# FelixBronnhuber/RenderBaby

Hardware: AMD Instinct MI355X
Metric: Msamples/s (ray-segments/s) (higher is better)
Workload: dtype f32; 1 GPU; C2 Cornell box (12 tris, 8 spheres, 1 area light), 1920x1080, 1024 spp, 8 bounces; width=1920, height=1080, spp=1024, max_depth=8, parallelism=single GPU, stripe_rows=8, walk=library default, tree_builder=, device=AMD Radeon Graphics (gfx950:sramecc+:xnack-, 256 CUs)

## Files before the change

### include/rb_abi.h

```cpp
#ifndef RB_ABI_H
#define RB_ABI_H

#include <stddef.h>
#include <stdint.h>

#ifdef __cplusplus
extern "C" {
#endif


typedef struct rb_camera {
    float pane_distance;
    float pane_width;
    float _pad0[2];
    float pos[3];
    float _pad1;
    float dir[3];
    float _pad2;
} rb_camera;

typedef struct rb_uniforms {
    uint32_t width;
    uint32_t height;
    uint32_t total_samples;
// ... 249 lines not shown
int rb_reset_stats(rb_engine* e);
int rb_last_dispatch_ms(rb_engine* e, float* ms);

int rb_bvh_build(const rb_gpu_triangle* tris, size_t n_tris,
                 rb_bvh_node* nodes_out, size_t nodes_capacity, size_t* n_nodes,
                 uint32_t* indices_out);

int rb_bvh_build_canonical(const rb_gpu_triangle* tris, size_t n_tris,
                           rb_bvh_node* nodes_out, size_t nodes_capacity, size_t* n_nodes,
                           uint32_t* indices_out);
int rb_bvh_build_device(int32_t device, const rb_gpu_triangle* tris, size_t n_tris,
                        rb_bvh_node* nodes_out, size_t nodes_capacity, size_t* n_nodes,
                        uint32_t* indices_out);
int rb_engine_tree(rb_engine* e, rb_bvh_node* nodes_out, size_t nodes_capacity, size_t* n_nodes,
                   uint32_t* indices_out, size_t indices_capacity, size_t* n_indices);
const char* rb_tree_builder(const rb_engine* e, float* build_ms);

int rb_debug_chunk_tree(const rb_gpu_triangle* tris, size_t n_tris, const rb_bvh_node* nodes, size_t n_nodes, const uint32_t* indices,
                        size_t n_indices, uint64_t out6[6]);
int rb_debug_engine_chunk_tree(rb_engine* e, uint64_t out6[6]);
typedef struct rb_debug_own_node {
    float lmin[3];
    uint32_t left;
    float lmax[3];
    uint32_t right;
    float rmin[3];
    float left_fa;
    float rmax[3];
    float right_fa;
} rb_debug_own_node;
typedef struct rb_debug_sphere_node {
    float cx[4], cy[4], cz[4], hx[4], hy[4], hz[4];
    uint32_t ref[4];
    uint32_t axes;
    uint32_t _pad[3];
} rb_debug_sphere_node;
int rb_debug_own_tree(const rb_gpu_triangle* tris, size_t n_tris, const rb_bvh_node* nodes, size_t n_nodes, const uint32_t* indices,
                      size_t n_indices, rb_debug_own_node* nodes_out, size_t nodes_capacity, uint32_t* slots_out, size_t slots_capacity,
                      uint32_t* slot_meta_out, size_t slot_meta_capacity, uint64_t counts3[3], uint32_t root_depth[2], float bounds6[6]);
int rb_debug_engine_own_tree(rb_engine* e, rb_debug_own_node* nodes_out, size_t nodes_capacity, uint32_t* slots_out, size_t slots_capacity,
                             uint32_t* slot_meta_out, size_t slot_meta_capacity, uint64_t counts3[3], uint32_t root_depth[2], float bounds6[6]);
int rb_debug_sphere_tree(const rb_sphere* spheres, size_t n, rb_debug_sphere_node* nodes_out, size_t nodes_capacity, float* leaf_out,
                         uint32_t* id_out, size_t spheres_capacity, uint64_t counts2[2], uint32_t root_depth[2]);
int rb_debug_engine_sphere_tree(rb_engine* e, rb_debug_sphere_node* nodes_out, size_t nodes_capacity, float* leaf_out, uint32_t* id_out,
                                size_t spheres_capacity, uint64_t counts2[2], uint32_t root_depth[2]);
const char* rb_chunk_tree_builder(const rb_engine* e, float* build_ms);
int rb_measure_l1_gather(int32_t device, uint64_t table_bytes, double* accesses_per_s);
int rb_debug_math(const float* a, const float* b, float* out8n, uint32_t n);
int rb_debug_walk_profile(uint64_t out64[64], int reset);
int rb_debug_rcp_exhaustive(uint32_t biased_exponent, uint32_t* out16);
int rb_debug_rcp_det_exhaustive(uint32_t biased_exponent, uint32_t* out16);
int rb_debug_triangle_trip(uint32_t n, uint32_t seed, uint32_t* out32);
int rb_debug_triangle_trip_flat(uint32_t n, uint32_t seed, uint32_t* out32);
int rb_debug_root_box(const float* rays, uint32_t n, const float* box6, uint32_t* out);
int rb_debug_normalize_sites(const float* xyz, uint32_t n, uint32_t n_unit, uint32_t seed0, uint32_t n_seeds, uint32_t* out16);
int rb_measure_salu_mix(int32_t device, uint32_t scalar_per_16, uint32_t branch, double* out3);
int rb_debug_rnd_pm1_exhaustive(uint32_t* out16);
int rb_debug_div_exhaustive(uint32_t b_begin, uint32_t b_count, uint32_t ea, uint32_t eb, uint32_t a_begin,
                            uint32_t a_count, unsigned long long* out16);

const char* rb_last_kernel_name(const rb_engine* e);
enum {
    RB_TRACE_FORM_FLAT = 1u,
    RB_TRACE_FORM_BIG = 4u,
    RB_TRACE_FORM_STAGED = 8u,
    RB_TRACE_FORM_MULTI = 16u
};
uint32_t rb_debug_trace_form(const rb_engine* e);

typedef struct rb_ray { float origin[3]; float _pad0; float dir[3]; float _pad1; } rb_ray;
enum { RB_HIT_NONE = 0, RB_HIT_GROUND = 1, RB_HIT_TRIANGLE = 2, RB_HIT_SPHERE = 3, RB_HIT_LIGHT = 4,
       RB_HIT_INVALID = 0xFFFFFFFFu };
typedef struct rb_hit {
    float t;
    uint32_t kind;
    uint32_t prim;
    uint32_t mesh;
    float u, v;
    uint32_t _pad[2];
    float normal[3];
    float _pad1;
} rb_hit;
typedef struct rb_surface {
    float albedo[3];
    uint32_t flags;
    float emissive[3];
    int32_t texture_index;
    float uv[2];
    float _pad[2];
} rb_surface;
int rb_cast_rays(rb_engine* e, const rb_ray* rays, size_t n, rb_hit* hits_out, rb_surface* surf_out);
int rb_render_hits(rb_engine* e, rb_hit* hits_out, rb_surface* surf_out);
int rb_pick(rb_engine* e, uint32_t px, uint32_t py, rb_hit* hit_out, rb_surface* surf_out);
const char* rb_last_query_kernel_name(const rb_engine* e);
int rb_last_query_ms(rb_engine* e, float* ms);

enum { RB_OCCL_VISIBLE = 0, RB_OCCL_OCCLUDED = 1, RB_OCCL_INVALID = 255 };
enum { RB_MASK_GROUND = 1, RB_MASK_TRIANGLES = 2, RB_MASK_SPHERES = 4, RB_MASK_LIGHTS = 8, RB_MASK_ALL = 15 };
int rb_occluded(rb_engine* e, const rb_ray* rays, const float* tmax, size_t n, uint32_t mask, uint8_t* out);
int rb_occluded_device(rb_engine* e, const rb_ray* d_rays, const float* d_tmax, size_t n, uint32_t mask, uint8_t* d_out);
int rb_cast_rays_device(rb_engine* e, const rb_ray* d_rays, size_t n, rb_hit* d_hits, rb_surface* d_surf);

typedef struct rb_radiance { float sum[3]; float weight; } rb_radiance;
#define RB_TRACE_PIECE_ITEMS (1u << 24)
int rb_trace_rays(rb_engine* e, const rb_ray* rays, const uint32_t* seeds, size_t n, uint32_t first_sample, uint32_t samples,
                  rb_radiance* out);
int rb_trace_rays_device(rb_engine* e, const rb_ray* d_rays, const uint32_t* d_seeds, size_t n, uint32_t first_sample,
                         uint32_t samples, rb_radiance* d_out);

enum { RB_CAM_PERSPECTIVE = 1, RB_CAM_ORTHO = 2, RB_CAM_EQUIRECT = 3 };
enum { RB_CAM_NO_JITTER = 1u };
typedef struct rb_camera_ex {
    uint32_t kind, width, height, flags;
    float pos[3];     float tan_half_fov;
    float right[3];   float half_width;
    float up[3];      float half_height;
// ... 304 lines not shown
```

### renderbaby_amd/_lib.py

```python
import ctypes as C
import os

from . import abi

_HERE = os.path.dirname(os.path.abspath(__file__))
LIB_PATH = os.environ.get("RB_LIBRARY_PATH") or os.path.join(_HERE, "librenderbaby_hip.so")
_lib = None


P = C.POINTER
vp, u32, i32, sz = C.c_void_p, C.c_uint32, C.c_int, C.c_size_t
SIGNATURES = {
    "rb_create": (vp, [P(abi.Config)]),
    "rb_create_ex": (vp, [P(abi.Config), P(abi.Options)]),
    "rb_create_multi": (vp, [P(abi.Config), P(abi.Options), P(C.c_int32), u32]),
    "rb_comm_unique_id": (i32, [vp]),
    "rb_comm_available": (i32, []),
    "rb_comm_init_rank": (i32, [vp, vp, u32, u32]),
    "rb_comm_info": (i32, [vp, P(u32), P(u32), P(C.c_float)]),
    "rb_destroy": (None, [vp]),
    "rb_update": (i32, [vp, P(abi.Config)]),
    "rb_render": (i32, [vp, vp]),
    "rb_render_config": (i32, [vp, P(abi.Config), vp]),
    "rb_iter_begin": (i32, [vp, P(abi.Config)]),
    "rb_iter_has_next": (i32, [vp]),
    "rb_iter_next": (i32, [vp, vp]),
    "rb_iter_destroy": (None, [vp]),
    "rb_iter_set_passes_per_frame": (i32, [vp, u32]),
    "rb_last_error": (C.c_char_p, [vp]),
    "rb_get_size": (i32, [vp, P(u32), P(u32)]),
    "rb_clear": (i32, [vp]),
    "rb_dispatch": (i32, [vp, u32, u32]),
    "rb_reserve": (i32, [vp, u32]),
    "rb_sync": (i32, [vp]),
    "rb_read_rgba": (i32, [vp, vp]),
    "rb_read_accumulation": (i32, [vp, vp]),
    "rb_device_rgba": (i32, [vp, P(vp), P(sz)]),
    "rb_host_alloc": (vp, [sz]),
    "rb_host_free": (None, [vp]),
    "rb_local_rows": (i32, [vp, P(u32), P(u32)]),
    "rb_global_row": (i32, [vp, u32, P(u32)]),
    "rb_shard_layout": (i32, [u32, u32, u32, u32, P(u32), P(u32)]),
    "rb_shard_global_row": (u32, [u32, u32, u32, u32]),
    "rb_get_stats": (i32, [vp, P(abi.Stats)]),
    "rb_reset_stats": (i32, [vp]),
    "rb_last_dispatch_ms": (i32, [vp, P(C.c_float)]),
    "rb_bvh_build": (i32, [vp, sz, vp, sz, P(sz), vp]),
    "rb_bvh_build_canonical": (i32, [vp, sz, vp, sz, P(sz), vp]),
    "rb_bvh_build_device": (i32, [i32, vp, sz, vp, sz, P(sz), vp]),
    "rb_engine_tree": (i32, [vp, vp, sz, P(sz), vp, sz, P(sz)]),
    "rb_tree_builder": (C.c_char_p, [vp, vp]),
    "rb_debug_chunk_tree": (i32, [vp, sz, vp, sz, vp, sz, vp]),
    "rb_measure_l1_gather": (i32, [i32, C.c_uint64, P(C.c_double)]),
    "rb_debug_math": (i32, [vp, vp, vp, u32]),
    "rb_debug_walk_profile": (i32, [vp, i32]),
    "rb_debug_rcp_exhaustive": (i32, [u32, vp]),
    "rb_debug_rcp_det_exhaustive": (i32, [u32, vp]),
    "rb_debug_rnd_pm1_exhaustive": (i32, [vp]),
    "rb_debug_triangle_trip": (i32, [u32, u32, vp]),
    "rb_debug_triangle_trip_flat": (i32, [u32, u32, vp]),
    "rb_debug_trace_form": (u32, [vp]),
    "rb_debug_root_box": (i32, [vp, u32, vp, vp]),
    "rb_debug_normalize_sites": (i32, [vp, u32, u32, u32, u32, vp]),
    "rb_measure_salu_mix": (i32, [i32, u32, u32, P(C.c_double)]),
    "rb_debug_div_exhaustive": (i32, [u32, u32, u32, u32, u32, u32, vp]),
    "rb_last_kernel_name": (C.c_char_p, [vp]),
    "rb_cast_rays": (i32, [vp, vp, sz, vp, vp]),
    "rb_render_hits": (i32, [vp, vp, vp]),
    "rb_pick": (i32, [vp, u32, u32, vp, vp]),
    "rb_occluded": (i32, [vp, vp, vp, sz, u32, vp]),
    "rb_occluded_device": (i32, [vp, vp, vp, sz, u32, vp]),
    "rb_cast_rays_device": (i32, [vp, vp, sz, vp, vp]),
    "rb_trace_rays": (i32, [vp, vp, vp, sz, u32, u32, vp]),
    "rb_trace_rays_device": (i32, [vp, vp, vp, sz, u32, u32, vp]),
    "rb_camera_rays": (i32, [i32, vp, C.c_uint64, sz, u32, u32, vp, vp]),
    "rb_trace_camera": (i32, [vp, vp, C.c_uint64, sz, u32, u32, vp]),
    "rb_trace_camera_device": (i32, [vp, vp, C.c_uint64, sz, u32, u32, vp]),
    "rb_last_camera_rays_ms": (i32, [vp, P(C.c_float)]),
    "rb_hemisphere_rays": (i32, [i32, vp, vp, sz, vp, u32, u32, vp, vp]),
    "rb_trace_hemisphere": (i32, [vp, vp, vp, sz, vp, u32, u32, vp]),
    "rb_trace_hemisphere_device": (i32, [vp, vp, vp, sz, vp, u32, u32, vp]),
    "rb_openness_hemisphere": (i32, [vp, vp, vp, sz, vp, u32, u32, vp]),
    "rb_openness_hemisphere_device": (i32, [vp, vp, vp, sz, vp, u32, u32, vp]),
    "rb_scene_emitters": (i32, [vp, vp, sz, P(sz)]),
    "rb_scene_emitters_device": (i32, [vp, vp, sz, vp]),
    "rb_light_rays": (i32, [i32, vp, sz, vp, vp, sz, vp, u32, u32, vp, vp, vp]),
    "rb_direct_light": (i32, [vp, vp, sz, vp, vp, sz, vp, u32, u32, vp]),
    "rb_direct_light_device": (i32, [vp, vp, sz, vp, vp, sz, vp, u32, u32, vp]),
    "rb_lightmap_surfels": (i32, [i32, vp, sz, vp, sz, vp, vp, vp]),
    "rb_lightmap_surfels_device": (i32, [vp, vp, vp, vp]),
    "rb_lightmap_resolve": (i32, [i32, u32, u32, vp, u32, vp]),
    "rb_bake_lightmap": (i32, [vp, vp, u32, u32, vp, vp]),
    "rb_bake_lightmap_device": (i32, [vp, vp, u32, u32, vp, vp]),
    "rb_last_lightmap_ms": (i32, [vp, P(C.c_float), P(C.c_float)]),
    "rb_probe_rays": (i32, [i32, vp, vp, sz, u32, u32, vp, vp]),
    "rb_bake_probes": (i32, [vp, vp, vp, sz, u32, u32, vp]),
    "rb_bake_probes_device": (i32, [vp, vp, vp, sz, u32, u32, vp]),
    "rb_last_probe_project_ms": (i32, [vp, P(C.c_float)]),
    "rb_probe_coefficients": (i32, [i32, vp, sz, vp]),
    "rb_probe_coefficients_device": (i32, [vp, vp, sz, vp]),
    "rb_light_points": (i32, [i32, vp, vp, vp, sz, vp]),
    "rb_light_points_device": (i32, [vp, vp, vp, vp, sz, vp]),
    "rb_bake_probe_depth": (i32, [vp, vp, vp, sz, u32, u32, C.c_float, vp]),
    "rb_bake_probe_depth_device": (i32, [vp, vp, vp, sz, u32, u32, C.c_float, vp]),
    "rb_last_probe_depth_project_ms": (i32, [vp, P(C.c_float)]),
    "rb_probe_moments": (i32, [i32, vp, sz, vp, vp]),
    "rb_probe_moments_device": (i32, [vp, vp, sz, vp, vp]),
    "rb_light_points_visible": (i32, [i32, vp, vp, vp, vp, sz, vp, vp]),
    "rb_light_points_visible_device": (i32, [vp, vp, vp, vp, vp, sz, vp, vp]),
    "rb_last_query_kernel_name": (C.c_char_p, [vp]),
    "rb_last_query_ms": (i32, [vp, P(C.c_float)]),
    "rb_denoise_default_params": (i32, [vp]),
    "rb_denoise_buffers": (i32, [i32, vp, u32, u32, vp, vp, vp, vp]),
# ... 63 lines not shown
```

### renderbaby_amd/abi.py

```python
import ctypes as C

import numpy as np

f4, u4, i4 = np.float32, np.uint32, np.int32

CAMERA = np.dtype([
    ("pane_distance", f4), ("pane_width", f4), ("_pad0", f4, (2,)),
    ("pos", f4, (3,)), ("_pad1", f4), ("dir", f4, (3,)), ("_pad2", f4)])

UNIFORMS = np.dtype([
    ("width", u4), ("height", u4), ("total_samples", u4), ("color_hash_enabled", u4),
    ("camera", CAMERA),
    ("spheres_count", u4), ("triangles_count", u4), ("bvh_node_count", u4),
    ("bvh_triangle_count", u4), ("bvh_root", u4), ("ground_height", f4),
    ("ground_enabled", u4), ("checkerboard_enabled", u4),
    ("sky_color", f4, (3,)), ("max_depth", u4),
    ("checkerboard_color_1", f4, (3,)), ("_pad1", u4),
    ("checkerboard_color_2", f4, (3,)), ("_pad2", u4)])

MATERIAL = np.dtype([
    ("ambient", f4, (3,)), ("_pad0", f4), ("diffuse", f4, (3,)), ("_pad1", f4),
    ("specular", f4, (3,)), ("shininess", f4), ("emissive", f4, (3,)), ("ior", f4),
    ("opacity", f4), ("illum", u4), ("texture_index", i4), ("_pad2", u4)])

# ... 38 lines not shown
PROBE_GRID = np.dtype([("origin", f4, (3,)), ("_pad0", u4), ("step", f4, (3,)), ("_pad1", u4), ("counts", u4, (3,)), ("flags", u4)])
LIT = np.dtype([("value", f4, (3,)), ("weight", f4)])
LIGHT_PIECE_POINTS = 1 << 22
PROBE_DEPTH = np.dtype([("texel", f4, (64, 4))])
LIGHT_VISIBILITY = np.dtype([("normal_bias", f4), ("min_visibility", f4), ("flags", u4), ("_pad", u4)])
VIS_NO_WRAP, VIS_NO_DEPTH = 1, 2
EMITTER = np.dtype([("a", f4, (3,)), ("kind", u4), ("b", f4, (3,)), ("prim", u4), ("c", f4, (3,)), ("area", f4),
                    ("emissive", f4, (3,)), ("_pad", f4)])
LIGHT_PARAMS = np.dtype([("offset", f4), ("shorten", f4), ("mask", u4), ("flags", u4), ("_reserved", u4, (4,))])
MAX_EMITTERS = 1 << 24
OCCL_VISIBLE, OCCL_OCCLUDED, OCCL_INVALID = 0, 1, 255
MASK_GROUND, MASK_TRIANGLES, MASK_SPHERES, MASK_LIGHTS, MASK_ALL = 1, 2, 4, 8, 15
GUIDE = np.dtype([("normal", f4, (3,)), ("t", f4), ("pos", f4, (3,)), ("cls", u4), ("albedo", f4, (3,)), ("_pad", f4)])
DENOISE_PARAMS = np.dtype([("iterations", u4), ("normal_power_log2", u4), ("sigma_depth", f4), ("sigma_color", f4),
                           ("albedo_floor", f4), ("flags", u4), ("_reserved", u4, (2,))])
VIEW = np.dtype([("pos", f4, (3,)), ("cx", f4), ("right", f4, (3,)), ("cy", f4), ("up", f4, (3,)), ("sx", f4), ("fwd", f4, (3,)), ("sy", f4)])
REPROJECT_PARAMS = np.dtype([("sigma_depth", f4), ("normal_min", f4), ("albedo_floor", f4), ("max_history", f4), ("flags", u4),
                             ("_reserved", u4, (3,))])
FRAME_RECORD = np.dtype([("mean", f4, (3,)), ("count", f4)])
OWN_NODE = np.dtype([("lmin", f4, (3,)), ("left", u4), ("lmax", f4, (3,)), ("right", u4),
                     ("rmin", f4, (3,)), ("left_fa", f4), ("rmax", f4, (3,)), ("right_fa", f4)])
SPHERE_NODE = np.dtype([("cx", f4, (4,)), ("cy", f4, (4,)), ("cz", f4, (4,)), ("hx", f4, (4,)), ("hy", f4, (4,)), ("hz", f4, (4,)),
                        ("ref", u4, (4,)), ("axes", u4), ("_pad", u4, (3,))])

SIZES = {"camera": (CAMERA, 48), "uniforms": (UNIFORMS, 144), "material": (MATERIAL, 80),
         "sphere": (SPHERE, 96), "point_light": (POINT_LIGHT, 96), "mesh": (MESH, 96),
         "bvh_node": (BVH_NODE, 48), "gpu_triangle": (GPU_TRIANGLE, 64),
         "ray": (RAY, 32), "hit": (HIT, 48), "surface": (SURFACE, 48),
         "guide": (GUIDE, 48), "denoise_params": (DENOISE_PARAMS, 32), "view": (VIEW, 64),
         "reproject_params": (REPROJECT_PARAMS, 32), "frame_record": (FRAME_RECORD, 16), "camera_ex": (CAMERA_EX, 96),
         "surfel": (SURFEL, 32), "hemi_params": (HEMI_PARAMS, 32), "openness": (OPENNESS, 8),
         "lightmap_params": (LIGHTMAP_PARAMS, 32), "probe": (PROBE, 16), "sh9": (SH9, 112),
         "probe_grid": (PROBE_GRID, 48), "lit": (LIT, 16),
         "probe_depth": (PROBE_DEPTH, 1024), "light_visibility": (LIGHT_VISIBILITY, 16),
         "emitter": (EMITTER, 64), "light_params": (LIGHT_PARAMS, 32),
         "own_node": (OWN_NODE, 64), "sphere_node": (SPHERE_NODE, 128)}
for _n, (_dt, _sz) in SIZES.items():
    assert _dt.itemsize == _sz, (_n, _dt.itemsize, _sz)

KEEP, CREATE, UPDATE, DELETE = 0, 1, 2, 3

RB_OK = 0
ERR = {
    1: "PaneDistanceOutOfBounds", 2: "PaneWidthOutOfBounds", 3: "InvalidCameraDirection",
    4: "InvalidUniforms", 5: "InvalidSpheres", 6: "InvalidUVs", 7: "InvalidMeshes",
    8: "InvalidLights", 9: "InvalidTextures", 10: "CannotDeleteNonexistent",
    11: "UniformsNotInitialized", 12: "NoMoreFrames", 13: "InvalidBVH", 14: "UnsupportedDelete",
    15: "NullArgument", 16: "Device", 17: "NotInitialized", 18: "InvalidOptions"}
RB_ERR_NO_MORE_FRAMES = 12
RB_ERR_DEVICE = 16

KERNEL_DEFAULT, KERNEL_PIXEL, KERNEL_QUEUE, KERNEL_STREAM = 0, 1, 2, 3
TRACE_FORM_FLAT, TRACE_FORM_BIG, TRACE_FORM_STAGED, TRACE_FORM_MULTI = 1, 4, 8, 16
FLAG_STATS = 1
FLAG_NO_SPHERE_BVH = 2
FLAG_FAST_BVH = 4
FLAG_DEVICE_BVH = 8
FLAG_DEVICE_LBVH = 16
FLAG_REFERENCE_WALK = 32
FLAG_HOST_BVH = 64
FLAG_GATHER_PEER_COPY = 128
FLAG_NO_RUN_AHEAD = 256
FLAG_SKIP_NEAR_DEGENERATE = 512
FLAG_CHUNK_WALK = 1024
FLAG_SPHERE_TREE_HOST = 2048
FLAG_SPHERE_TREE_DEVICE = 4096
FLAG_CHUNK_TREE_HOST = 8192
FLAG_CHUNK_TREE_DEVICE = 16384
FLAG_BUILD_TREE = 32768
FLAG_BUILD_TREE_HOST = 65536
COMM_ID_BYTES = 128


class Field(C.Structure):
    _fields_ = [("change", C.c_uint32), ("ptr", C.c_void_p), ("count", C.c_size_t)]


class Config(C.Structure):
    _fields_ = [(n, Field) for n in ("uniforms", "spheres", "uvs", "meshes", "lights", "bvh_nodes",
                                      "bvh_indices", "bvh_triangles", "textures")]


class Texture(C.Structure):
    _fields_ = [("width", C.c_uint32), ("height", C.c_uint32), ("rgba_data", C.c_void_p)]


class Options(C.Structure):
    _fields_ = [("device", C.c_int32), ("shard_rank", C.c_uint32), ("shard_count", C.c_uint32),
                ("stripe_rows", C.c_uint32), ("passes_per_launch", C.c_uint32), ("kernel", C.c_uint32),
                ("flags", C.c_uint32), ("_reserved", C.c_uint32 * 5)]


class Ray(C.Structure):
    _fields_ = [("origin", C.c_float * 3), ("_pad0", C.c_float), ("dir", C.c_float * 3), ("_pad1", C.c_float)]


class Hit(C.Structure):
    _fields_ = [("t", C.c_float), ("kind", C.c_uint32), ("prim", C.c_uint32), ("mesh", C.c_uint32), ("u", C.c_float),
                ("v", C.c_float), ("_pad", C.c_uint32 * 2), ("normal", C.c_float * 3), ("_pad1", C.c_float)]


class Surface(C.Structure):
    _fields_ = [("albedo", C.c_float * 3), ("flags", C.c_uint32), ("emissive", C.c_float * 3),
                ("texture_index", C.c_int32), ("uv", C.c_float * 2), ("_pad", C.c_float * 2)]


# ... 17 lines not shown
```

### renderbaby_amd/csrc/rb_debug.hip

```cpp
#include <algorithm>

#include "rb_device_shade.hpp"

#pragma clang fp contract(off)

namespace rb {
namespace {

__global__ void k_rcp_exhaustive(uint32_t expo, uint32_t* mismatch) {
    const uint32_t m = blockIdx.x * blockDim.x + threadIdx.x;
    if (m >= (1u << 23)) return;
    for (uint32_t sign = 0; sign < 2; sign++) {
        const uint32_t bits = (sign << 31) | ((expo & 0xFFu) << 23) | m;
        const float b = __uint_as_float(bits);
        float want, got;
        if (expo & 0x100u) {
            if (sign) continue;
            want = sqrtf(b);
            got = sqrt_exact(b);
        } else {
            if (!rcp_safe(b)) continue;
            want = 1.0f / b;
            got = rcp_newton(b);
        }
// ... 60 lines not shown
DEV void trip_case(uint32_t k, f3& o, f3& d, f3& v0, f3& e1, f3& e2) {
    o = mk(0.25f, 0.25f, -1.0f);
    d = mk(0.0f, 0.0f, 1.0f);
    v0 = mk(0.0f, 0.0f, 0.0f);
    e1 = mk(0.0f, 1.0f, 0.0f);
    e2 = mk(1.0f, 0.0f, 0.0f);
    const uint32_t eps = 0x358637BDu, big = 0x71800000u, one = 0x3F800000u, tmin = 0x3A83126Fu;
    const float nan = __uint_as_float(0x7FC00000u), inf = __uint_as_float(0x7F800000u);
    switch (k) {
        case 0: case 1: case 2: e1.y = __uint_as_float(eps - 1u + k); break;
        case 3: case 4: case 5: e1.y = -__uint_as_float(eps - 1u + (k - 3u)); break;
        case 6: case 7: case 8: e1.y = __uint_as_float(big - 1u + (k - 6u)); break;
        case 9: e1.y = -0x1p100f; break;
        case 10: e1.y = 0x1p120f; break;
        case 11: e1.y = __uint_as_float(0x3F80FFFFu); break;
        case 12: e1.y = __uint_as_float(0xC123FFFFu); break;
        case 13: e1.y = __uint_as_float(0x3FFFFFFFu); break;
        case 14: o.y = 0.0f; break;
        case 15: o.y = -0.0f; break;
        case 16: o.y = -0x1p-149f; break;
        case 17: o.y = 1.0f; o.x = 0.0f; break;
        case 18: o.y = __uint_as_float(one + 1u); o.x = 0.0f; break;
        case 19: o.x = 0.0f; break;
        case 20: o.x = -0.0f; break;
        case 21: o.x = -0x1p-149f; break;
        case 22: o.x = 0.75f; break;
        case 23: o.x = 0.75f; o.y = __uint_as_float(0x3E800001u); break;
        case 24: o.z = -__uint_as_float(tmin); break;
        case 25: o.z = -__uint_as_float(tmin + 1u); break;
        case 26: o.z = -__uint_as_float(tmin - 1u); break;
        case 27: o.z = 0.0f; break;
        case 28: o.z = 1.0f; break;
        case 29: o.x = nan; break;
        case 30: o.y = nan; break;
        case 31: o.z = nan; break;
        case 32: d.x = nan; break;
        case 33: d.y = nan; break;
        case 34: d.z = nan; break;
        case 35: o.x = inf; break;
        case 36: o.y = -inf; break;
        case 37: o.z = -inf; break;
        case 38: d.x = inf; break;
        case 39: d.y = -inf; break;
        case 40: d.z = inf; break;
        case 41: e1.y = 0.0f; break;
        case 42: e1.y = nan; break;
        default: e2.x = inf; break;
    }
}
DEV float trip_unit(uint32_t& s) {
    s = pcg(s);
    return (float)(int32_t)s * 0x1p-31f;
}
template <bool FLAT>
__global__ void __launch_bounds__(256) k_triangle_trip(uint32_t n_waves, uint32_t seed, uint32_t* mismatch) {
    const uint32_t wave = (blockIdx.x * 256u + threadIdx.x) >> 6, lane = threadIdx.x & 63u;
    if (wave >= n_waves + kTripCases) return;
    f3 o, d, v0, e1, e2;
    float hit_t = 1e20f;
    bool on = true;
    if (wave < n_waves) {
        uint32_t sw = pcg(seed ^ (wave * 0x9E3779B9u)), sl = pcg(sw + lane * 0x85EBCA6Bu + 1u);
        const uint32_t kind = pcg(sw) & 15u;
        const float scale = kind == 0u ? 0x1p-10f : kind == 1u ? 0x1p52f : 1.0f;
        v0 = mk(trip_unit(sw), trip_unit(sw), trip_unit(sw));
        e1 = scale * mk(trip_unit(sw), trip_unit(sw), trip_unit(sw));
        e2 = scale * mk(trip_unit(sw), trip_unit(sw), trip_unit(sw));
        o = 2.0f * mk(trip_unit(sl), trip_unit(sl), trip_unit(sl));
        const float a = 0.7f * trip_unit(sl) + 0.5f, b = 0.7f * trip_unit(sl) + 0.5f;
        const f3 to = (v0 + a * e1 + b * e2) - o;
        d = __builtin_amdgcn_rsqf(dot(to, to) + 1e-30f) * to;
        const uint32_t r = pcg(sl);
        if (r & 1u) hit_t = 2.0f * (float)(r >> 8) * 0x1p-24f;
        on = (r & 6u) != 0u;
    } else {
        trip_case(wave - n_waves, o, d, v0, e1, e2);
        on = (lane & 8u) == 0u;
    }
    auto uni = [](float x) { return __uint_as_float((uint32_t)__builtin_amdgcn_readfirstlane((int)__float_as_uint(x))); };
    const v4f ra = {uni(v0.x), uni(v0.y), uni(v0.z), 0.0f}, rb_ = {uni(e1.x), uni(e1.y), uni(e1.z), 0.0f},
              rc = {uni(e2.x), uni(e2.y), uni(e2.z), 1.0f};
    const uint32_t slot = (uint32_t)__builtin_amdgcn_readfirstlane((int)(wave + 1u));
    if (wave >= n_waves) {
        TriHit own;
        own.t = 1e20f, own.u = 0.0f, own.v = 0.0f, own.slot = 0u, own.hit = false;
        accept_slot<true>(ra, rb_, rc, slot, o, d, own);
        const uint32_t v = lane & 3u;
        hit_t = v == 0u ? 1e20f : v == 1u ? 0.5f : v == 2u ? own.t : __uint_as_float(__float_as_uint(own.t) + 1u);
    }
    TriHit want, got;
    want.t = hit_t, want.u = -2.0f, want.v = -3.0f, want.slot = 0xABCDu, want.hit = false;
    got = want;
    float big = 0x1p100f;
    if constexpr (RB_TRIP_BLOCK) asm("s_mov_b32 %0, 0x71800000" : "=s"(big));
    if (on) {
        accept_slot<true>(ra, rb_, rc, slot, o, d, want);
        if constexpr (FLAT && RB_TRIP_BLOCK) {
            TriHitT<false> flat;
            flat.t = got.t, flat.slot = got.slot, flat.hit = false;
            accept_trip<RB_TRIP_ASM - 1, false>(ra, rb_, rc, slot, o, d, big, flat);
            got.t = flat.t, got.slot = flat.slot, got.u = want.u, got.v = want.v;
        } else if constexpr (RB_TRIP_BLOCK) accept_trip<RB_TRIP_ASM - 1>(ra, rb_, rc, slot, o, d, big, got);
        else accept_slot<true>(ra, rb_, rc, slot, o, d, got);
    }
    if (__float_as_uint(want.t) != __float_as_uint(got.t) || __float_as_uint(want.u) != __float_as_uint(got.u) ||
        __float_as_uint(want.v) != __float_as_uint(got.v) || want.slot != got.slot) {
        if (atomicAdd(&mismatch[0], 1u) == 0u) {
            mismatch[1] = wave * 64u + lane;
            const float in[16] = {o.x, o.y, o.z, d.x, d.y, d.z, ra.x, ra.y, ra.z, rb_.x, rb_.y, rb_.z, rc.x, rc.y, rc.z, hit_t};
            for (int k = 0; k < 16; k++) mismatch[2 + k] = __float_as_uint(in[k]);
            mismatch[18] = __float_as_uint(got.t), mismatch[19] = __float_as_uint(got.u), mismatch[20] = __float_as_uint(got.v);
            mismatch[21] = got.slot;
            mismatch[22] = __float_as_uint(want.t), mismatch[23] = __float_as_uint(want.u), mismatch[24] = __float_as_uint(want.v);
            mismatch[25] = want.slot;
        }
    }
}

template <int SALU, bool BRANCH>
__global__ void __launch_bounds__(256, 8) k_salu_mix(uint32_t rounds, float c, float* sink, unsigned long long* stamp) {
    float v[16];
#pragma unroll
    for (int k = 0; k < 16; k++) v[k] = (float)(threadIdx.x + k) * 0x1p-20f;
    const float c2 = c * 0x1p-20f;
    uint32_t s0 = rounds, s1 = rounds + 1u, s2 = rounds + 2u, s3 = rounds + 3u;
    const unsigned long long t0 = __builtin_amdgcn_s_memtime(), r0 = __builtin_amdgcn_s_memrealtime();
#define RB_MIX_F(k) "v_fmac_f32_e32 %" #k ", %[c], %[c2]\n\t"
#define RB_MIX_S(j) "s_add_u32 %[s" #j "], %[s" #j "], 1\n\t"
#define RB_MIX_Q0(a, b, c, d) RB_MIX_F(a) RB_MIX_F(b) RB_MIX_F(c) RB_MIX_F(d)
#define RB_MIX_Q1(a, b, c, d) RB_MIX_F(a) RB_MIX_F(b) RB_MIX_S(0) RB_MIX_F(c) RB_MIX_F(d)
#define RB_MIX_Q2(a, b, c, d) RB_MIX_F(a) RB_MIX_S(0) RB_MIX_F(b) RB_MIX_F(c) RB_MIX_S(1) RB_MIX_F(d)
#define RB_MIX_Q3(a, b, c, d) RB_MIX_F(a) RB_MIX_S(0) RB_MIX_F(b) RB_MIX_S(1) RB_MIX_F(c) RB_MIX_S(2) RB_MIX_F(d)
#define RB_MIX_Q4(a, b, c, d) RB_MIX_F(a) RB_MIX_S(0) RB_MIX_F(b) RB_MIX_S(1) RB_MIX_F(c) RB_MIX_S(2) RB_MIX_F(d) RB_MIX_S(3)
#define RB_MIX_BR "s_cbranch_execz .Lmix_out_%=\n\t"
#define RB_MIX_GROUP(Q, BR) Q(0, 1, 2, 3) Q(4, 5, 6, 7) Q(8, 9, 10, 11) Q(12, 13, 14, 15) BR
#define RB_MIX_ASM(Q, BR)                                                                                                 \
    asm volatile(RB_MIX_GROUP(Q, BR) RB_MIX_GROUP(Q, BR) RB_MIX_GROUP(Q, BR) RB_MIX_GROUP(Q, BR) ".Lmix_out_%=:"          \
                 : "+v"(v[0]), "+v"(v[1]), "+v"(v[2]), "+v"(v[3]), "+v"(v[4]), "+v"(v[5]), "+v"(v[6]), "+v"(v[7]), "+v"(v[8]), \
                   "+v"(v[9]), "+v"(v[10]), "+v"(v[11]), "+v"(v[12]), "+v"(v[13]), "+v"(v[14]), "+v"(v[15]), [s0] "+s"(s0), \
                   [s1] "+s"(s1), [s2] "+s"(s2), [s3] "+s"(s3)                                                            \
                 : [c] "v"(c), [c2] "v"(c2)                                                                                             \
                 : "scc")
    for (uint32_t r = rounds; r != 0u; r--) {
        if constexpr (BRANCH) {
            if constexpr (SALU == 0) RB_MIX_ASM(RB_MIX_Q0, RB_MIX_BR);
            else if constexpr (SALU == 4) RB_MIX_ASM(RB_MIX_Q1, RB_MIX_BR);
            else if constexpr (SALU == 8) RB_MIX_ASM(RB_MIX_Q2, RB_MIX_BR);
            else if constexpr (SALU == 12) RB_MIX_ASM(RB_MIX_Q3, RB_MIX_BR);
            else RB_MIX_ASM(RB_MIX_Q4, RB_MIX_BR);
        } else {
            if constexpr (SALU == 0) RB_MIX_ASM(RB_MIX_Q0, "");
            else if constexpr (SALU == 4) RB_MIX_ASM(RB_MIX_Q1, "");
            else if constexpr (SALU == 8) RB_MIX_ASM(RB_MIX_Q2, "");
            else if constexpr (SALU == 12) RB_MIX_ASM(RB_MIX_Q3, "");
            else RB_MIX_ASM(RB_MIX_Q4, "");
        }
    }
#undef RB_MIX_F
#undef RB_MIX_S
#undef RB_MIX_Q0
#undef RB_MIX_Q1
#undef RB_MIX_Q2
#undef RB_MIX_Q3
#undef RB_MIX_Q4
#undef RB_MIX_BR
#undef RB_MIX_GROUP
#undef RB_MIX_ASM
    const unsigned long long t1 = __builtin_amdgcn_s_memtime(), r1 = __builtin_amdgcn_s_memrealtime();
    float acc = (float)(s0 ^ s1 ^ s2 ^ s3);
// ... 127 lines not shown
#undef RB_MIX_LAUNCH
        (void)hipEventRecord(t1, nullptr);
        if (!ok || hipGetLastError() != hipSuccess || hipEventSynchronize(t1) != hipSuccess) { ok = false; break; }
        float ms = 0.0f;
        (void)hipEventElapsedTime(&ms, t0, t1);
        if (rep > 0 && ms > 0.0f && (best == 0.0f || ms < best)) {
            best = ms;
            (void)hipMemcpy(st, stamp, 16, hipMemcpyDeviceToHost);
        }
    }
    (void)hipEventDestroy(t0);
    (void)hipEventDestroy(t1);
    (void)hipFree(sink);
    (void)hipFree(stamp);
    if (!ok || best <= 0.0f || st[1] == 0ull) return false;
    const double ghz = (double)st[0] / (double)st[1] * 0.1;
    out[0] = (best * 1e-3) * (ghz * 1e9) / ((double)rounds * 64.0 * 8.0);
    out[1] = ghz;
    out[2] = best;
    return true;
}

double measure_l1_gather(size_t table_bytes, uint32_t rounds) {
    size_t lines = 64;
    while (lines * 2 * 128 <= table_bytes) lines *= 2;
    float4 *table = nullptr, *sink = nullptr;
    if (hipMalloc(reinterpret_cast<void**>(&table), lines * 128) != hipSuccess) return 0.0;
    if (hipMalloc(reinterpret_cast<void**>(&sink), 16) != hipSuccess) { (void)hipFree(table); return 0.0; }
    (void)hipMemset(table, 0, lines * 128);
    hipEvent_t t0, t1;
    (void)hipEventCreate(&t0);
    (void)hipEventCreate(&t1);
    double best = 0.0;
    for (int shape = 0; shape < 4; shape++) {
        const uint32_t inflight = (shape & 1) ? 16u : 8u, blocks = device_cu_count_cached() * ((shape & 2) ? 8u : 4u);
        for (int rep = 0; rep < 2; rep++) {
            (void)hipEventRecord(t0, nullptr);
            if (inflight == 16u) hipLaunchKernelGGL(k_l1_gather<16>, dim3(blocks), dim3(256), 0, nullptr, table, (uint32_t)(lines - 1), rounds, sink);
            else hipLaunchKernelGGL(k_l1_gather<8>, dim3(blocks), dim3(256), 0, nullptr, table, (uint32_t)(lines - 1), rounds, sink);
            (void)hipEventRecord(t1, nullptr);
            if (hipEventSynchronize(t1) != hipSuccess) break;
            float ms = 0.0f;
            (void)hipEventElapsedTime(&ms, t0, t1);
            if (ms > 0.0f) best = std::max(best, (double)blocks * 256.0 * rounds * inflight / (ms * 1e-3));
        }
    }
    (void)hipEventDestroy(t0);
    (void)hipEventDestroy(t1);
    (void)hipFree(table);
    (void)hipFree(sink);
    return best;
}
}
}

extern "C" {

int rb_debug_rcp_exhaustive(uint32_t biased_exponent, uint32_t* out16) {
    if (!out16) return RB_ERR_NULL_ARGUMENT;
    return rb::round_trip(out16, 64, 64, [&](uint32_t* d) {
        hipLaunchKernelGGL(rb::k_rcp_exhaustive, dim3((1u << 23) / 256), dim3(256), 0, nullptr, biased_exponent, d);
    });
}

int rb_debug_rcp_det_exhaustive(uint32_t biased_exponent, uint32_t* out16) {
    if (!out16) return RB_ERR_NULL_ARGUMENT;
    if (biased_exponent > 255u) return RB_ERR_INVALID_OPTIONS;
    return rb::round_trip(out16, 64, 64, [&](uint32_t* d) {
        hipLaunchKernelGGL(rb::k_rcp_det_exhaustive, dim3((1u << 23) / 256), dim3(256), 0, nullptr, biased_exponent, d);
    });
}

int rb_debug_triangle_trip(uint32_t n, uint32_t seed, uint32_t* out32) {
    if (!out32) return RB_ERR_NULL_ARGUMENT;
    if (n > (1u << 26)) return RB_ERR_INVALID_OPTIONS;
    return rb::round_trip(out32, 128, 128, [&](uint32_t* d) {
        const uint32_t n_waves = (n + 63u) / 64u, waves = n_waves + rb::kTripCases;
        hipLaunchKernelGGL(rb::k_triangle_trip<false>, dim3((waves + 3u) / 4u), dim3(256), 0, nullptr, n_waves, seed, d);
    });
}

int rb_debug_triangle_trip_flat(uint32_t n, uint32_t seed, uint32_t* out32) {
    if (!out32) return RB_ERR_NULL_ARGUMENT;
    if (n > (1u << 26)) return RB_ERR_INVALID_OPTIONS;
    return rb::round_trip(out32, 128, 128, [&](uint32_t* d) {
        const uint32_t n_waves = (n + 63u) / 64u, waves = n_waves + rb::kTripCases;
        hipLaunchKernelGGL(rb::k_triangle_trip<true>, dim3((waves + 3u) / 4u), dim3(256), 0, nullptr, n_waves, seed, d);
    });
}

int rb_debug_root_box(const float* rays, uint32_t n, const float* box6, uint32_t* out) {
    if (!rays || !box6 || !out) return RB_ERR_NULL_ARGUMENT;
    if (n == 0u) return RB_OK;
    if (n > (1u << 24)) return RB_ERR_INVALID_OPTIONS;
    const size_t out_bytes = (size_t)n * 4u, in_bytes = (size_t)n * 24u;
    const rb::f3 bmin = {box6[0], box6[1], box6[2]}, bmax = {box6[3], box6[4], box6[5]};
    return rb::round_trip(out, out_bytes, out_bytes + in_bytes, [&](uint32_t* d) {
        float* dr = reinterpret_cast<float*>(d + n);
        (void)hipMemcpy(dr, rays, in_bytes, hipMemcpyHostToDevice);
        hipLaunchKernelGGL(rb::k_root_box, dim3((n + 255u) / 256u), dim3(256), 0, nullptr, dr, n, bmin, bmax, d);
    });
}

int rb_debug_normalize_sites(const float* xyz, uint32_t n, uint32_t n_unit, uint32_t seed0, uint32_t n_seeds, uint32_t* out16) {
    if (!out16 || (!xyz && n + n_unit != 0u)) return RB_ERR_NULL_ARGUMENT;
    if (n > (1u << 26) || n_unit > (1u << 26) || n_seeds > (1u << 26)) return RB_ERR_INVALID_OPTIONS;
    const size_t total = (size_t)n + n_unit + n_seeds, in_bytes = ((size_t)n + n_unit) * 12u;
    if (total == 0u) {
        std::fill(out16, out16 + 16, 0u);
        return RB_OK;
    }
    return rb::round_trip(out16, 64, 64 + in_bytes, [&](uint32_t* d) {
        float* dv = reinterpret_cast<float*>(d + 16);
        if (in_bytes) (void)hipMemcpy(dv, xyz, in_bytes, hipMemcpyHostToDevice);
        hipLaunchKernelGGL(rb::k_normalize_sites, dim3((uint32_t)((total + 255u) / 256u)), dim3(256), 0, nullptr, dv, n, n_unit, seed0, n_seeds, d);
    });
}

int rb_measure_salu_mix(int32_t device, uint32_t scalar_per_16, uint32_t branch, double* out3) {
    if (!out3) return RB_ERR_NULL_ARGUMENT;
    if (scalar_per_16 > 16u || (scalar_per_16 & 3u) != 0u) return RB_ERR_INVALID_OPTIONS;
    int before = -1;
    if (device >= 0 && (hipGetDevice(&before) != hipSuccess || hipSetDevice(device) != hipSuccess)) return RB_ERR_DEVICE;
    const bool ok = rb::measure_salu_mix(scalar_per_16, branch != 0u, 4096u, out3);
    if (before >= 0) (void)hipSetDevice(before);
    return ok ? RB_OK : RB_ERR_DEVICE;
}

int rb_debug_rnd_pm1_exhaustive(uint32_t* out16) {
    if (!out16) return RB_ERR_NULL_ARGUMENT;
    return rb::round_trip(out16, 64, 64, [&](uint32_t* d) {
        hipLaunchKernelGGL(rb::k_rnd_pm1_exhaustive, dim3(1u << 16), dim3(256), 0, nullptr, d);
    });
}

int rb_debug_div_exhaustive(uint32_t b_begin, uint32_t b_count, uint32_t ea, uint32_t eb, uint32_t a_begin,
                            uint32_t a_count, unsigned long long* out16) {
    if (!out16) return RB_ERR_NULL_ARGUMENT;
    return rb::round_trip(out16, 128, 128, [&](unsigned long long* d) {
        hipLaunchKernelGGL(rb::k_div_exhaustive, dim3((b_count + 255) / 256), dim3(256), 0, nullptr, b_begin, ea, eb, a_begin, a_count, d);
// ... 24 lines not shown
```

### renderbaby_amd/csrc/rb_device_intersect.hpp

```cpp
#pragma once
#include "rb_device_math.hpp"

#pragma clang fp contract(off)

namespace rb {
namespace {

template <bool TEXEL = true>
DEV f3 sample_texture(const KParams& p, int32_t index, float uvx, float uvy) {
    if (!TEXEL || index < 0) {
        if (p.u.checkerboard_enabled > 0u) {
            int32_t u2 = f2i(floorf(uvx * 10.0f));
            int32_t v2 = f2i(floorf(uvy * 10.0f));
            int32_t sum = (int32_t)((uint32_t)u2 + (uint32_t)v2);
            return (sum % 2 == 0) ? ld3(p.u.checkerboard_color_1) : ld3(p.u.checkerboard_color_2);
        }
        return mk(1.0f, 1.0f, 1.0f);
    }
    if ((uint32_t)index >= p.n_tex) return mk(0.0f, 0.0f, 0.0f);
    const v4u iw = ((cu4p)p.tex_info)[index];
    rb_texture_info info;
    info.offset = iw.x;
    info.width = iw.y;
    info.height = iw.z;
// ... 128 lines not shown
    uint32_t slot;
    bool hit;
};
using TriHit = TriHitT<true>;

template <bool UV>
DEV void test_slot(const v4f a, const v4f b, const v4f c, uint32_t slot, f3 o, f3 d, TriHitT<UV>& h) {
    float u, v;
    const float t = isect_triangle(o, d, mk(a.x, a.y, a.z), mk(b.x, b.y, b.z), mk(c.x, c.y, c.z), u, v);
    if (t > 0.001f && t < h.t) {
        h.hit = true;
        h.t = t;
        if constexpr (UV) {
            h.u = u;
            h.v = v;
        }
        h.slot = slot;
    }
}

template <bool DET = false>
DEV void accept_slot(const v4f a, const v4f b, const v4f c, uint32_t slot, f3 o, f3 d, TriHit& hit) {
    const f3 v0 = mk(a.x, a.y, a.z), edge1 = mk(b.x, b.y, b.z), edge2 = mk(c.x, c.y, c.z);
    const f3 h = cross(d, edge2);
    const float det = dot(edge1, h);
    if (!(fabsf(det) < 1e-6f)) {
        const float f = DET ? rcp_det(det) : rcp_tri(det);
        const f3 s = o - v0;
        const float u = f * dot(s, h);
        if (!(u < 0.0f || u > 1.0f)) {
            const f3 q = cross(s, edge1);
            const float v = f * dot(d, q);
            if (!(v < 0.0f || u + v > 1.0f)) {
                const float t = f * dot(edge2, q);
                if (t > 0.0f && t > 0.001f && t < hit.t) {
                    hit.t = t;
                    hit.u = u;
                    hit.v = v;
                    hit.slot = slot;
                }
            }
        }
    }
}

#ifndef RB_TRIP_PLAIN
#define RB_TRIP_PLAIN 1
#endif
#ifndef RB_TRIP_ASM
#define RB_TRIP_ASM 3
#endif
#define RB_TRIP_BLOCK (RB_TRIP_ASM != 0 && RB_FAST_RCP && RB_RCP_DET)

template <int SKIP, bool UV = true>
DEV void accept_trip(const v4f a, const v4f b, const v4f c, uint32_t slot, f3 o, f3 d, float big, TriHitT<UV>& hit) {
    float r8, r10, r11, r12, r13, r14, r15, r16, r17;
    uint64_t entry, keep, m, ds;
#define RB_TRIP_HEAD                                                                                                     \
    "s_mov_b64 %[entry], exec\n\t"                                                                                       \
    "v_mul_f32_e32 %[r8], %[cz], %[dy]\n\t"                                                                              \
    "v_mul_f32_e32 %[r10], %[cy], %[dz]\n\t"                                                                             \
    "v_sub_f32_e32 %[r10], %[r8], %[r10]\n\t"                                                                            \
    "v_mul_f32_e32 %[r8], %[cx], %[dz]\n\t"                                                                              \
    "v_mul_f32_e32 %[r11], %[cz], %[dx]\n\t"                                                                             \
    "v_sub_f32_e32 %[r11], %[r8], %[r11]\n\t"                                                                            \
    "v_mul_f32_e32 %[r8], %[cy], %[dx]\n\t"                                                                              \
    "v_mul_f32_e32 %[r12], %[cx], %[dy]\n\t"                                                                             \
    "v_sub_f32_e32 %[r12], %[r8], %[r12]\n\t"                                                                            \
    "v_mul_f32_e32 %[r8], %[bx], %[r10]\n\t"                                                                             \
    "v_mul_f32_e32 %[r13], %[by], %[r11]\n\t"                                                                            \
    "v_add_f32_e32 %[r8], %[r8], %[r13]\n\t"                                                                             \
    "v_mul_f32_e32 %[r13], %[bz], %[r12]\n\t"                                                                            \
    "v_add_f32_e32 %[r13], %[r13], %[r8]\n\t"                                                                            \
    "v_cmpx_nlt_f32_e64 vcc, |%[r13]|, %[eps]\n\t"                                                  \
    "v_cmp_eq_u16_e64 %[m], -1, %[r13]\n\t"                                     \
    "v_cmp_nlt_f32_e64 vcc, |%[r13]|, %[big]\n\t"                                               \
    "v_rcp_f32_e32 %[r8], %[r13]\n\t"                                                                                    \
    "s_or_b64 %[m], vcc, %[m]\n\t"                                                                                       \
    "v_fma_f32 %[r14], -%[r13], %[r8], 1.0\n\t"                                                                          \
    "v_fmac_f32_e32 %[r8], %[r14], %[r8]\n\t"                                                                            \
    "s_and_saveexec_b64 %[keep], %[m]\n\t"                                                                               \
    "s_cbranch_execz .Ltrip_rcp_%=\n\t"                                                                                  \
    "v_div_scale_f32 %[r8], %[ds], %[r13], %[r13], 1.0\n\t"                   \
    "v_rcp_f32_e32 %[r14], %[r8]\n\t"                                                                                    \
    "v_div_scale_f32 %[r15], vcc, 1.0, %[r13], 1.0\n\t"                                                                  \
    "v_fma_f32 %[r16], -%[r8], %[r14], 1.0\n\t"                                                                          \
    "v_fmac_f32_e32 %[r14], %[r16], %[r14]\n\t"                                                                          \
    "v_mul_f32_e32 %[r16], %[r15], %[r14]\n\t"                                                                           \
    "v_fma_f32 %[r17], -%[r8], %[r16], %[r15]\n\t"                                                                       \
    "v_fmac_f32_e32 %[r16], %[r17], %[r14]\n\t"                                                                          \
    "v_fma_f32 %[r8], -%[r8], %[r16], %[r15]\n\t"                                                                        \
    "v_div_fmas_f32 %[r8], %[r8], %[r14], %[r16]\n\t"                                                                    \
    "v_div_fixup_f32 %[r8], %[r8], %[r13], 1.0\n"                                                                        \
    ".Ltrip_rcp_%=:\n\t"                                                                                                 \
    "s_mov_b64 exec, %[keep]\n\t"                                                                                        \
    "v_subrev_f32_e32 %[r13], %[ax], %[ox]\n\t"                                                                          \
    "v_subrev_f32_e32 %[r14], %[ay], %[oy]\n\t"                                                                          \
    "v_subrev_f32_e32 %[r15], %[az], %[oz]\n\t"                                                                          \
    "v_mul_f32_e32 %[r10], %[r13], %[r10]\n\t"                                                                           \
    "v_mul_f32_e32 %[r11], %[r14], %[r11]\n\t"                                                                           \
    "v_add_f32_e32 %[r10], %[r10], %[r11]\n\t"                                                                           \
    "v_mul_f32_e32 %[r11], %[r15], %[r12]\n\t"                                                                           \
    "v_add_f32_e32 %[r10], %[r11], %[r10]\n\t"                                                                           \
    "v_mul_f32_e32 %[r10], %[r10], %[r8]\n\t"                                                                     \
    "v_cmpx_ngt_f32_e32 vcc, 0, %[r10]\n\t"                                                                \
    "v_cmpx_nlt_f32_e32 vcc, 1.0, %[r10]\n\t"
#define RB_TRIP_TAIL                                                                                                     \
    "v_mul_f32_e32 %[r11], %[bz], %[r14]\n\t"                                                                            \
    "v_mul_f32_e32 %[r12], %[by], %[r15]\n\t"                                                                            \
    "v_sub_f32_e32 %[r12], %[r11], %[r12]\n\t"                                                                           \
    "v_mul_f32_e32 %[r11], %[bx], %[r15]\n\t"                                                                            \
    "v_mul_f32_e32 %[r15], %[bz], %[r13]\n\t"                                                                            \
    "v_sub_f32_e32 %[r15], %[r11], %[r15]\n\t"                                                                           \
    "v_mul_f32_e32 %[r11], %[by], %[r13]\n\t"                                                                            \
    "v_mul_f32_e32 %[r13], %[bx], %[r14]\n\t"                                                                            \
    "v_sub_f32_e32 %[r13], %[r11], %[r13]\n\t"                                                                           \
    "v_mul_f32_e32 %[r11], %[dx], %[r12]\n\t"                                                                            \
    "v_mul_f32_e32 %[r14], %[dy], %[r15]\n\t"                                                                            \
    "v_add_f32_e32 %[r11], %[r11], %[r14]\n\t"                                                                           \
    "v_mul_f32_e32 %[r14], %[dz], %[r13]\n\t"                                                                            \
    "v_add_f32_e32 %[r11], %[r14], %[r11]\n\t"                                                                           \
    "v_mul_f32_e32 %[r11], %[r11], %[r8]\n\t"                                                                     \
    "v_add_f32_e32 %[r14], %[r10], %[r11]\n\t"                                                                           \
    "v_cmpx_ngt_f32_e32 vcc, 0, %[r11]\n\t"                                                                \
    "v_cmpx_nlt_f32_e32 vcc, 1.0, %[r14]\n\t"
#define RB_TRIP_LAST                                                                                                     \
    "v_mul_f32_e32 %[r12], %[cx], %[r12]\n\t"                                                                            \
    "v_mul_f32_e32 %[r14], %[cy], %[r15]\n\t"                                                                            \
    "v_add_f32_e32 %[r12], %[r12], %[r14]\n\t"                                                                           \
    "v_mul_f32_e32 %[r13], %[cz], %[r13]\n\t"                                                                            \
    "v_add_f32_e32 %[r12], %[r13], %[r12]\n\t"                                                                           \
    "v_mul_f32_e32 %[r8], %[r12], %[r8]\n\t"                                                                      \
    "v_cmpx_lt_f32_e32 vcc, %[tmin], %[r8]\n\t"                                                           \
    "v_cmpx_lt_f32_e32 vcc, %[r8], %[ht]\n\t"                                                             \
    "v_mov_b32_e32 %[hs], %[slot]\n\t"
#define RB_TRIP_MOVES_UV                                                                                                 \
    "v_mov_b32_e32 %[hv], %[r11]\n\t"                                                                                    \
    "v_mov_b32_e32 %[ht], %[r8]\n\t"                                                                                     \
    "v_mov_b32_e32 %[hu], %[r10]\n"
#define RB_TRIP_MOVES_T                                                                                                  \
    "v_mov_b32_e32 %[ht], %[r8]\n"
#define RB_TRIP_OUT_UV [ht] "+v"(hit.t), [hu] "+v"(hit.u), [hv] "+v"(hit.v), [hs] "+v"(hit.slot)
#define RB_TRIP_OUT_T [ht] "+v"(hit.t), [hs] "+v"(hit.slot)
#define RB_TRIP_TEMPS                                                                                                    \
    [r8] "=&v"(r8), [r10] "=&v"(r10),                                                                                     \
      [r11] "=&v"(r11), [r12] "=&v"(r12), [r13] "=&v"(r13), [r14] "=&v"(r14), [r15] "=&v"(r15), [r16] "=&v"(r16),         \
      [r17] "=&v"(r17), [entry] "=&s"(entry), [keep] "=&s"(keep), [m] "=&s"(m), [ds] "=&s"(ds)
#define RB_TRIP_IN                                                                                                       \
    [ax] "s"(a.x), [ay] "s"(a.y), [az] "s"(a.z), [bx] "s"(b.x), [by] "s"(b.y), [bz] "s"(b.z), [cx] "s"(c.x),              \
      [cy] "s"(c.y), [cz] "s"(c.z), [slot] "s"(slot), [ox] "v"(o.x), [oy] "v"(o.y), [oz] "v"(o.z), [dx] "v"(d.x),         \
      [dy] "v"(d.y), [dz] "v"(d.z), [eps] "s"(1e-6f)
#define RB_TRIP_CLOBBERS "vcc", "scc"
#define RB_TRIP_OPS_UV : RB_TRIP_OUT_UV, RB_TRIP_TEMPS : RB_TRIP_IN, [big] "s"(big), [tmin] "s"(0.001f) : RB_TRIP_CLOBBERS
#define RB_TRIP_OPS_T : RB_TRIP_OUT_T, RB_TRIP_TEMPS : RB_TRIP_IN, [big] "s"(big), [tmin] "s"(0.001f) : RB_TRIP_CLOBBERS
#define RB_TRIP_SKIP "s_cbranch_execz .Ltrip_end_%=\n\t"
#define RB_TRIP_EMIT(MOVES, OPS)                                                                                         \
    if constexpr (SKIP == 2) {                                                                                           \
        asm volatile(RB_TRIP_HEAD RB_TRIP_SKIP RB_TRIP_TAIL RB_TRIP_SKIP RB_TRIP_LAST MOVES ".Ltrip_end_%=:\n\t"         \
                     "s_mov_b64 exec, %[entry]" OPS);                                                                    \
    } else if constexpr (SKIP == 1) {                                                                                    \
        asm volatile(RB_TRIP_HEAD RB_TRIP_SKIP RB_TRIP_TAIL RB_TRIP_LAST MOVES ".Ltrip_end_%=:\n\t"                      \
                     "s_mov_b64 exec, %[entry]" OPS);                                                                    \
    } else {                                                                                                             \
        asm volatile(RB_TRIP_HEAD RB_TRIP_TAIL RB_TRIP_LAST MOVES "\ts_mov_b64 exec, %[entry]" OPS);                     \
    }
    if constexpr (UV) {
        RB_TRIP_EMIT(RB_TRIP_MOVES_UV, RB_TRIP_OPS_UV)
    } else {
        RB_TRIP_EMIT(RB_TRIP_MOVES_T, RB_TRIP_OPS_T)
    }
#undef RB_TRIP_EMIT
#undef RB_TRIP_SKIP
#undef RB_TRIP_HEAD
#undef RB_TRIP_MOVES_UV
#undef RB_TRIP_MOVES_T
#undef RB_TRIP_OUT_UV
#undef RB_TRIP_OUT_T
#undef RB_TRIP_TEMPS
#undef RB_TRIP_IN
#undef RB_TRIP_CLOBBERS
#undef RB_TRIP_OPS_UV
#undef RB_TRIP_OPS_T
#undef RB_TRIP_TAIL
#undef RB_TRIP_LAST
}


DEV float cone_cos_bound(f3 d, v4f cone) {
    const float y = fabsf(__builtin_fmaf(d.z, cone.z, __builtin_fmaf(d.y, cone.y, d.x * cone.x)));
    const float k2 = __builtin_fmaf(cone.z, cone.z, __builtin_fmaf(cone.y, cone.y, cone.x * cone.x));
    const float root = 1.000001f * __builtin_amdgcn_sqrtf(fmaxf(__builtin_fmaf(-y, y, k2), 0.0f) + 4e-6f * k2);
    return __builtin_fmaf(-cone.w, root, y - 1e-6f);
}
DEV bool cone_admits_grazing(f3 d, v4f cone) {
    if (cone.w < 0.0f) return false;
    return !(cone_cos_bound(d, cone) >= kFastGrazeCos);
}
constexpr float kFastKF = 27.0f * 5.9604645e-8f * 1.01f;
constexpr float kFastKS = 20.0f * 5.9604645e-8f * 1.01f;
template <bool STATS>
struct FastWalk {
    f3 o, d, inv;
    float m_ref;
    TriHit h;
    uint32_t best_rank;
    uint32_t cur;
    uint32_t gend;
    bool graze;
    int sp;

    DEV void begin(const KParams& p, f3 o_, f3 d_) {
        o = o_;
        d = d_;
        h.hit = false;
        h.t = 1e20f;
        h.u = 0.0f;
        h.v = 0.0f;
        h.slot = 0u;
        best_rank = 0xFFFFFFFFu;
        inv = mk(rcp_exact(d.x), rcp_exact(d.y), rcp_exact(d.z));
        const f3 fb0 = ld3(p.fast_bmin), fb1 = ld3(p.fast_bmax);
        const float sx_ = fmaxf(fabsf(o.x - fb0.x), fabsf(o.x - fb1.x)), sy_ = fmaxf(fabsf(o.y - fb0.y), fabsf(o.y - fb1.y)),
// ... 156 lines not shown
        const cf4p rnodes = (cf4p)p.nodes;
        const RB_CONST uint32_t* parent = cptr(p.ref_parent);
        const float m = m_ref;
        {
            const v4f n0 = rnodes[leaf_node * 3u], n1 = rnodes[leaf_node * 3u + 1u];
            if constexpr (STATS) tl.nodes++;
            const bool thick = (n1.x - n0.x >= 2.0f * m) && (n1.y - n0.y >= 2.0f * m) && (n1.z - n0.z >= 2.0f * m);
            const f3 t0 = (mk(n0.x + m, n0.y + m, n0.z + m) - o) * inv;
            const f3 t1 = (mk(n1.x - m, n1.y - m, n1.z - m) - o) * inv;
            const float tn = fmaxf(fmaxf(fminf(t0.x, t1.x), fminf(t0.y, t1.y)), fminf(t0.z, t1.z));
            const float tf = fminf(fminf(fmaxf(t0.x, t1.x), fmaxf(t0.y, t1.y)), fmaxf(t0.z, t1.z));
            const bool finite = (t0.x == t0.x) && (t0.y == t0.y) && (t0.z == t0.z) && (t1.x == t1.x) && (t1.y == t1.y) &&
                                (t1.z == t1.z);
            if (thick && finite && tf >= fmaxf(tn, 0.0f)) return true;
        }
        uint32_t n = leaf_node;
        for (;;) {
            const v4f n0 = rnodes[n * 3u], n1 = rnodes[n * 3u + 1u];
            if constexpr (STATS) tl.nodes++;
            if (!isect_aabb(o, inv, mk(n0.x, n0.y, n0.z), mk(n1.x, n1.y, n1.z))) return false;
            if (n == 0u) return true;
            n = parent[n];
        }
    }

    DEV bool leaf_step(const KParams& p, uint32_t* stack, uint32_t stride, Tally<STATS>& tl) {
        const cf4p ftris = (cf4p)p.fast_tris;
        const RB_CONST uint32_t* fslots = cptr(p.fast_slots);
        const RB_CONST uint32_t* meta = cptr(p.slot_meta);
        const uint32_t first = cur & 0x0FFFFFFFu, count = ((cur >> 28) & 3u) + 1u;
        for (uint32_t j = first; j < first + count; j++) {
            const v4f a = ftris[j * 4u], b = ftris[j * 4u + 1u], c = ftris[j * 4u + 2u];
            if constexpr (STATS) tl.tris++;
            float u, v;
            const float t = isect_triangle(o, d, mk(a.x, a.y, a.z), mk(b.x, b.y, b.z), mk(c.x, c.y, c.z), u, v);
            if (t > 0.001f && !(t > h.t)) {
                const uint32_t slot = fslots[j];
                const uint32_t leaf_node = meta[slot * 2u], rank = meta[slot * 2u + 1u] & ~kSlotLarge;
                if ((t < h.t || rank < best_rank) && reference_would_test(p, leaf_node, tl)) {
                    h.hit = true;
                    h.t = t;
                    h.u = u;
                    h.v = v;
                    h.slot = slot;
                    best_rank = rank;
                    if constexpr (STATS) tl.mesh_hits++;
                }
            }
        }
        return pop(p, stack, stride);
    }
};

template <bool STATS>
DEV TriHit intersect_bvh_fast(const KParams& p, f3 o, f3 d, uint32_t* stack, uint32_t stride, Tally<STATS>& tl) {
    FastWalk<STATS> w;
    w.begin(p, o, d);
    while (w.step(p, stack, stride, tl)) {
    }
    return w.h;
}

template <bool STATS, bool MULTI = true, bool TRIP = false, bool UV = true>
DEV TriHitT<UV> intersect_bvh(const KParams& p, f3 o, f3 d, uint32_t* stack, uint32_t stride, Tally<STATS>& tl, uint32_t box = kBoxUnknown) {
    static_assert(UV || (TRIP && !MULTI && RB_TRIP_BLOCK && RB_TRIP_PLAIN != 0), "the flat forms exist for the hand-laid trip only");
    TriHitT<UV> h;
    h.hit = false;
    h.t = 1e20f;
    if constexpr (UV) {
        h.u = 0.0f;
        h.v = 0.0f;
    }
    h.slot = 0u;
    const uint32_t node_count = p.u.bvh_node_count;
    if (node_count == 0u) return h;
    if constexpr (MULTI) {
        if (p.fast_nodes != nullptr) return intersect_bvh_fast<STATS>(p, o, d, stack, stride, tl);
    }
    constexpr bool skip_box = TRIP && !MULTI && RB_ROOT_INSIDE != 0;
    const f3 inv = skip_box ? d : mk(rcp_exact(d.x), rcp_exact(d.y), rcp_exact(d.z));
    const cf4p nodes = (cf4p)p.nodes;
    const cf4p ptris = (cf4p)p.ptris;

    if (node_count == 1u) {
        const v4f n0 = nodes[0], n1 = nodes[1];
        const v4u n2 = ((cu4p)p.nodes)[2];
        if constexpr (STATS) tl.nodes++;
        const uint32_t first = n2.z, count = n2.w;
        const uint32_t end = (first + count < p.index_len) ? first + count : p.index_len;
        auto in_box = [&]() {
            const f3 b0 = mk(n0.x, n0.y, n0.z), b1 = mk(n1.x, n1.y, n1.z);
            if constexpr (skip_box) {
                const uint64_t unknown = __builtin_amdgcn_uicmp(box, kBoxUnknown, 32) & ~root_inside_mask(o, d, b0, b1);
                if (__builtin_expect(unknown == 0ull && box_finite(b0, b1), 1)) return box != kBoxMiss;
                return isect_aabb(o, mk(rcp_exact(d.x), rcp_exact(d.y), rcp_exact(d.z)), b0, b1);
            } else {
                return isect_aabb(o, inv, b0, b1);
            }
        };
        if (first < end && in_box()) {
            constexpr bool trip = TRIP && !MULTI;
            float big = 0x1p100f;
            if constexpr (trip && RB_TRIP_BLOCK) asm("s_mov_b32 %0, 0x71800000" : "=s"(big));
            auto test = [&](const v4f a, const v4f b, const v4f c, uint32_t slot) {
                if constexpr (STATS) tl.tris++;
                const float before = h.t;
                if constexpr (trip && RB_TRIP_BLOCK) accept_trip<RB_TRIP_ASM - 1, UV>(a, b, c, slot, o, d, big, h);
                else accept_slot<!MULTI>(a, b, c, slot, o, d, h);
                if constexpr (STATS) tl.mesh_hits += (h.t != before) ? 1u : 0u;
            };
            if constexpr (trip && RB_TRIP_PLAIN != 0) {
                cf4p rec = ptris + (size_t)first * 4u;
                for (uint32_t slot = first; slot != end; slot++, rec += 4) {
                    v4f a = rec[0], b = rec[1], c = rec[2];
                    uint32_t live = __float_as_uint(c.w);
                    asm volatile("" : "+s"(a.x), "+s"(b.x), "+s"(live));
                    if (live != 0u) test(a, b, c, slot);
                }
            } else {
                const uint32_t last = end - 1u;
                cf4p rec = ptris + (size_t)first * 4u;
                v4f a = rec[0], b = rec[1], c = rec[2];
                bool live = __float_as_uint(c.w) != 0u;
                for (uint32_t slot = first;; slot++) {
                    if (slot < last) rec += 4;
                    const v4f na = rec[0], nb = rec[1], nc = rec[2];
                    if (live) test(a, b, c, slot);
                    if (slot == last) break;
                    a = na;
                    b = nb;
                    c = nc;
                    live = __float_as_uint(nc.w) != 0u;
                }
            }
            h.hit = h.t < 1e20f;
        }
        return h;
    }
    if constexpr (!MULTI) return h;

    int sp = 0;
    stack[0] = 0u;
    sp = 1;
    while (sp > 0) {
        sp--;
        const uint32_t node_idx = stack[sp * stride];
        if (node_idx >= node_count) continue;
        const v4f n0 = nodes[node_idx * 3u], n1 = nodes[node_idx * 3u + 1u];
        const v4u n2 = ((cu4p)p.nodes)[node_idx * 3u + 2u];
        if constexpr (STATS) tl.nodes++;
        if (!isect_aabb(o, inv, mk(n0.x, n0.y, n0.z), mk(n1.x, n1.y, n1.z))) continue;
        const uint32_t left = n2.x, right = n2.y, first = n2.z, count = n2.w;
        if (count > 0u) {
            for (uint32_t i = 0; i < count; i++) {
                const uint32_t slot = first + i;
                if (slot >= p.index_len) continue;
                const v4f a = ptris[slot * 4u], b = ptris[slot * 4u + 1u], c = ptris[slot * 4u + 2u];
                if (__float_as_uint(c.w) == 0u) continue;
                if constexpr (STATS) tl.tris++;
                const float before = h.t;
                test_slot(a, b, c, slot, o, d, h);
                if constexpr (STATS) tl.mesh_hits += (h.t != before) ? 1u : 0u;
            }
        } else {
// ... 29 lines not shown
```

### renderbaby_amd/csrc/rb_device_shade.hpp

```cpp
#pragma once
#include "rb_device_intersect.hpp"

#pragma clang fp contract(off)

namespace rb {
namespace {

DEV const KParams& fresh_params(const KParams&) {
    const RB_CONST char* k = (const RB_CONST char*)__builtin_amdgcn_kernarg_segment_ptr();
    asm volatile("" : "+s"(k));
    return *(const KParams*)k;
}

struct Mat {
    f3 diffuse, specular, emissive;
    float fuzz;
    bool metal;
    int32_t tex;
};
DEV Mat load_mat(const rb_material* m) {
    const cf4p q = (cf4p)m;
    const v4f d = q[1], s = q[2], e = q[3];
    const v4u t = ((cu4p)m)[4];
    Mat r;
// ... 437 lines not shown
            } else {
                use_tex = load_tex_index(mm) >= 0;
            }
        }
        if (kind == K_TRI) {
            prim = p0.w;
            mesh = p1.w;
            bu = th.u;
            bv = th.v;
            const v4f s = ((cf4p)p.ptris)[th.slot * 4u + 3u];
            normal = mk(s.x, s.y, s.z);
        }
    }
    if (kind == K_GROUND) m.diffuse = mk(0.5f, 0.5f, 0.5f);
    if (sphere_idx != 0xFFFFFFFFu) {
        const rb_sphere* s = p.spheres + sphere_idx;
        if (kind == K_SPHERE) {
            m = load_mat(&s->material);
            use_tex = m.tex >= 0;
            const v4f cr = ((cf4p)s)[0];
            normal = normalize(pos - mk(cr.x, cr.y, cr.z));
            prim = sphere_idx;
        } else {
            use_tex = load_tex_index(&s->material) >= 0;
        }
    }
    if (kind == K_LIGHT) {
        const rb_point_light* l = p.lights + light_idx;
        m = load_mat(&l->material);
        const v4f cr = ((cf4p)l)[0];
        normal = normalize(pos - mk(cr.x, cr.y, cr.z));
        prim = light_idx;
    }
    f3 albedo = m.metal ? m.specular : m.diffuse;
    if (!m.metal && use_tex) albedo = albedo * sample_texture(p, m.tex, uvx, uvy);
    out.h0 = v4f{closest_t, __uint_as_float(kind), __uint_as_float(prim), __uint_as_float(mesh)};
    out.h1 = v4f{bu, bv, 0.0f, 0.0f};
    out.h2 = v4f{normal.x, normal.y, normal.z, 0.0f};
    out.s0 = v4f{albedo.x, albedo.y, albedo.z, __uint_as_float((m.metal ? 1u : 0u) | (use_tex ? 2u : 0u))};
    out.s1 = v4f{m.emissive.x, m.emissive.y, m.emissive.z, __uint_as_float((uint32_t)m.tex)};
    out.s2 = v4f{uvx, uvy, 0.0f, 0.0f};
}

template <bool STATS, bool SPHTREE = true, bool PARK = true, bool JOINED = true, bool LEAN = false, bool TRIM = false, bool UV = true>
DEV bool segment_finish(const KParams& p, Path& pt, const TriHitT<UV> th, uint32_t* stack, uint32_t stride,
                        Tally<STATS>& tl) {
    const SegState st = segment_pre<STATS, UV>(fresh_params(p), pt, th, tl);
    float closest_t = st.closest_t;
    uint32_t sphere_idx = 0xFFFFFFFFu;
    segment_spheres<STATS, SPHTREE, LEAN>(fresh_params(p), pt.o, pt.d, dot(pt.d, pt.d), closest_t, sphere_idx, stack, stride, tl);
    return segment_post<STATS, PARK, JOINED, TRIM, UV>(fresh_params(p), pt, th, st, closest_t, sphere_idx, tl);
}

template <bool STATS, bool MULTI = true, bool JOINED = true, bool TRIP = false, bool UV = true>
DEV bool segment(const KParams& p, Path& pt, uint32_t* stack, uint32_t stride, Tally<STATS>& tl, uint32_t box = kBoxUnknown) {
    const TriHitT<UV> th = intersect_bvh<STATS, MULTI, TRIP, UV>(fresh_params(p), pt.o, pt.d, stack, stride, tl, box);
    return segment_finish<STATS, MULTI, true, JOINED, !MULTI, TRIP && !MULTI, UV>(p, pt, th, stack, stride, tl);
}

DEV void start_path_hashed(const KParams& p, uint32_t x, uint32_t y, uint32_t pixel_index, uint32_t sample_hash, Path& pt) {
    const Cam& c = p.cam;
    uint32_t seed = pcg(pixel_index + sample_hash);
    const float off_x = rnd(seed) - 0.5f;
    const float off_y = rnd(seed) - 0.5f;
    const float ax = (float)x + off_x, ay = (float)y + off_y;
    float qx, qy;
    if (c.fast_wh) {
        qx = __builtin_copysignf(div_newton(ax, c.wm1, c.inv_wm1), ax);
        qy = __builtin_copysignf(div_newton(ay, c.hm1, c.inv_hm1), ay);
    } else {
        qx = ax / c.wm1;
        qy = ay / c.hm1;
    }
    const float u = ((qx * 2.0f) - 1.0f) * c.aspect;
    const float v = 1.0f - qy * 2.0f;
    pt.o = ld3(c.pos);
    pt.d = normalize(((c.fov * u) * ld3(c.right) + (c.fov * v) * ld3(c.up)) + ld3(c.fwd));
    pt.seed = seed;
    pt.color = mk(0, 0, 0);
    pt.att = mk(1, 1, 1);
    pt.depth = 0;
}

DEV void start_ray_hashed(const KParams& p, uint32_t x, uint32_t y, uint32_t pixel_index, uint32_t sample_hash, f3& d, uint32_t& seed_out) {
    const Cam& c = p.cam;
    uint32_t seed = pcg(pixel_index + sample_hash);
    const float off_x = rnd(seed) - 0.5f;
    const float off_y = rnd(seed) - 0.5f;
    const float ax = (float)x + off_x, ay = (float)y + off_y;
    float qx, qy;
    if (c.fast_wh) {
        qx = __builtin_copysignf(div_newton(ax, c.wm1, c.inv_wm1), ax);
        qy = __builtin_copysignf(div_newton(ay, c.hm1, c.inv_hm1), ay);
    } else {
        qx = ax / c.wm1;
        qy = ay / c.hm1;
    }
    const float u = ((qx * 2.0f) - 1.0f) * c.aspect;
    const float v = 1.0f - qy * 2.0f;
    d = normalize(((c.fov * u) * ld3(c.right) + (c.fov * v) * ld3(c.up)) + ld3(c.fwd));
    seed_out = seed;
}

DEV void start_path(const KParams& p, uint32_t x, uint32_t y, uint32_t pixel_index, uint32_t sample_offset, Path& pt) {
    start_path_hashed(p, x, y, pixel_index, pcg(sample_offset), pt);
}

DEV uint32_t global_row(const KParams& p, uint32_t ly) {
    if (p.shard_count <= 1u) return ly;
// ... 66 lines not shown
```

### renderbaby_amd/csrc/rb_engine.hpp

```cpp
#pragma once
#include <hip/hip_runtime_api.h>

#include <algorithm>
#include <memory>
#include <mutex>
#include <string>
#include <vector>

#include "rb_color_plan.hpp"
#include "rb_internal.hpp"
#include "rb_rccl.hpp"
#include "rb_stage_timer.hpp"
#include "rb_update_plan.hpp"

namespace rb {

template <typename T>
struct DevBuf {
    T* ptr = nullptr;
    size_t count = 0;
    ~DevBuf() { release(); }
    void release() {
        if (ptr) (void)hipFree(ptr);
        ptr = nullptr;
        count = 0;
    }
    hipError_t resize(size_t n) {
        if (n == count && ptr) return hipSuccess;
        release();
        if (n == 0) return hipSuccess;
        hipError_t e = hipMalloc(reinterpret_cast<void**>(&ptr), n * sizeof(T));
        if (e == hipSuccess) count = n;
        return e;
    }
    void adopt(T* p, size_t n) {
        release();
        ptr = p;
        count = n;
    }
    bool serves(size_t n) const { return ptr && n <= count && count <= 4 * std::max<size_t>(n, 1); }
    hipError_t reserve(size_t n) { return serves(n) ? hipSuccess : resize(n); }
};

struct FrameSlot {
    DevBuf<float> accum;
    DevBuf<uint32_t> rgba;
    hipEvent_t done = nullptr;
};

struct BuildRecord {
    const char* builder = "";
    float ms = 0.0f;
    bool built() const { return builder[0] != '\0'; }
};

struct SphereAccel {
    DevBuf<SphereNode4> nodes;
    DevBuf<float> leaf;
    DevBuf<uint32_t> id;
    uint32_t root = 0, depth = 0;
    BuildRecord rec;
};

struct ChunkAccel {
    DevBuf<ChunkNode> nodes;
    DevBuf<float> a, b, c;
    DevBuf<uint32_t> rank_slot;
    DevBuf<uint32_t> pos_slot, pos_rank;
    size_t n_nodes = 0;
    uint32_t root = 0, depth = 0;
    BuildRecord rec;
};

struct OwnAccel {
    DevBuf<SphereNode> nodes;
    DevBuf<PrepTri> tris;
    DevBuf<uint32_t> slots, slot_meta, ref_parent, stack_overflow;
    DevBuf<GrazeNode> gnodes;
    DevBuf<uint32_t> gslots;
    DeviceTreeInfo info{};
    BuildRecord rec;
};

struct MeshWalks {
    bool host_mesh = false;
    bool chunk = false;
    bool own_named = false;
    bool own(uint32_t n_tris) const { return host_mesh && (own_named || n_tris >= kOwnTreeDefaultMinTriangles); }
};

}

struct rb_engine {
    std::mutex mu;
    mutable std::mutex err_mu;
    mutable std::string error;
    int device = 0;
    hipStream_t stream = nullptr;
    hipStream_t copy_stream = nullptr;
    hipStream_t accum_stream = nullptr;
    hipStream_t trace_stream = nullptr;
    hipEvent_t ev_begin = nullptr, ev_end = nullptr;
    hipEvent_t ev_top = nullptr;
    hipEvent_t ev_traced[2] = {nullptr, nullptr};
    hipEvent_t ev_accumulated[2] = {nullptr, nullptr};
    std::vector<hipEvent_t> ev_pool;
    uint32_t ev_used = 0;
    const char* last_kernel_name = "";
    rb_options opt{};

    rb::SceneFacts sc;
    bool scene_valid = false;
    bool trace_uv = false;
    uint32_t last_trace_form = 0;
    rb_progressive prh{};
    bool iter_initialized = false;
    uint32_t iter_passes_per_frame = 1;

    bool prep_dirty = true;
    uint32_t prep_tri_count = 0xFFFFFFFFu;

    rb::DevBuf<rb_sphere> spheres;
    rb::DevBuf<float> sph_scan;
    rb::DevBuf<rb_point_light> lights;
    rb::DevBuf<rb_mesh> meshes;
    rb::DevBuf<rb_bvh_node> nodes;
    rb::DevBuf<uint32_t> indices;
    rb::DevBuf<rb_gpu_triangle> tris;
    rb::DevBuf<rb::PrepTri> ptris;
    rb::DevBuf<rb::PrepTriShade> pshade;
    rb::DevBuf<float> uvs;
    rb::DevBuf<uint32_t> tex_data;
    rb::DevBuf<rb_texture_info> tex_info;
    rb::DevBuf<float> srgb_lut;
    rb::FrameSlot slot[2];
    int cur = 0;
    bool spec_valid = false;
    uint32_t spec_first = 0, spec_n = 0;
    rb::DevBuf<unsigned long long> counters;
    rb::DevBuf<uint32_t> queue;
    rb::SphereAccel sph;
    rb::ChunkAccel chunk;
    rb::OwnAccel own;
    rb::BuildRecord tree;
    std::vector<rb_gpu_triangle> host_tris;
    std::vector<uint32_t> host_indices;
    size_t host_tri_len = 0, host_index_len = 0;
    bool host_tris_stale = false, host_indices_stale = false;
    bool stack_depth_covers = true;
    rb::DevBuf<float> colors;
    size_t color_part_floats = 0;
    uint64_t color_budget = 0;

    rb::DevBuf<rb_ray> q_rays;
    rb::DevBuf<rb_hit> q_hits;
    rb::DevBuf<rb_surface> q_surf;
    rb::DevBuf<float> q_tmax;
    rb::DevBuf<uint8_t> q_occl;
    rb::DevBuf<float> rad_colors;
    rb::DevBuf<uint32_t> rad_seeds, rad_queue;
    rb::DevBuf<rb_radiance> rad_out;
    rb::DevBuf<rb_surfel> hemi_surfels;
    rb::DevBuf<rb_openness> hemi_open;
    rb::DevBuf<rb_probe> probe_pos;
    rb::DevBuf<rb_sh9> probe_out;
    rb::DevBuf<rb_probe_depth> depth_out;
    rb::DevBuf<rb_emitter> emit_table, emit_given;
// ... 89 lines not shown
```

### renderbaby_amd/csrc/rb_internal.hpp

```cpp
#pragma once

#include <cstddef>
#include <cstdint>
#include <string>
#include <vector>

#include "../../include/rb_abi.h"

#if defined(__HIPCC__) || defined(__HIP__)
#define RB_HD __host__ __device__
#else
#define RB_HD
#endif

namespace rb {

constexpr uint32_t kStackDepth = 32;
constexpr uint32_t kStackEntryBytes = 4;
constexpr uint32_t kDefaultStripeRows = 8;

void bvh_build(const rb_gpu_triangle* tris, size_t n_tris, std::vector<rb_bvh_node>& nodes,
               std::vector<uint32_t>& indices);
bool bvh_validate(const rb_bvh_node* nodes, uint32_t node_count, uint32_t max_stack, std::string& why,
                  uint32_t* depth_out);
// ... 203 lines not shown
    const rb_texture_info* tex_info;
    const float* srgb_lut;
    const SphereNode* fast_nodes;
    const GrazeNode* gnodes;
    const uint32_t* gslots;
    uint32_t fast_skip_second_pass;
    const float* fast_tris;
    const uint32_t* fast_slots;
    const uint32_t* slot_meta;
    const uint32_t* ref_parent;
    uint32_t fast_root;
    float fast_margin;
    float fast_bmin[3];
    float fast_root_amax;
    float fast_bmax[3];
    uint32_t _pad_fast;
    const ChunkNode* chunk_nodes;
    const float* chunk_a;
    const float* chunk_b;
    const float* chunk_c;
    const uint32_t* chunk_rank_slot;
    uint32_t chunk_root;
    uint32_t chunk_n;
    const SphereNode4* sph_nodes;
    const float* sph_leaf;
    const uint32_t* sph_id;
    uint32_t sph_root;
    uint32_t _pad_sph;
    const float* accum_in;
    float* accum_out;
    uint32_t* out_rgba;
    unsigned long long* counters;
    uint32_t* queue;
    float* colors;
    uint32_t n_lights;
    uint32_t n_meshes;
    uint32_t index_len;
    uint32_t n_uvs;
    uint32_t n_tex;
    uint32_t first_pass, n_passes, samples_per_pass;
    uint32_t shard_rank, shard_count, stripe_rows, local_rows;
    uint32_t stack_depth;
    uint32_t blocks_per_cu;
    uint32_t queue_batch;
    uint32_t queue_groups;
    uint32_t queue_region;
    uint32_t no_leaf_stepping;
    uint32_t lds_mode;
    uint32_t magic_S, magic_tiles_x;
    uint32_t* stack_overflow;
    Cam cam;
    const float* sph_scan;
    uint32_t no_uv;
};

struct LaunchInfo {
    uint32_t grid, block;
    size_t lds_bytes;
    const char* kernel_name;
    uint32_t trace_form;
};

enum QueryWalk : uint32_t { kWalkPlain, kWalkBvh, kWalkChunk };
inline QueryWalk query_walk(KParams& p) {
    if (p.u.bvh_node_count > 1u && !p.no_leaf_stepping && p.chunk_nodes != nullptr) return kWalkChunk;
    p.fast_nodes = nullptr;
    return (p.u.bvh_node_count > 1u || p.sph_nodes != nullptr) ? kWalkBvh : kWalkPlain;
}

struct QueryArgs {
    const rb_ray* rays;
    rb_hit* hits;
    rb_surface* surf;
    uint32_t n;
    uint32_t win_x, win_y, win_w, win_h;
    uint32_t win_global;
};
#ifndef RB_QUERY_PIECE_LOG2
#define RB_QUERY_PIECE_LOG2 22
#endif
constexpr uint32_t kQueryPiece = 1u << RB_QUERY_PIECE_LOG2;
int launch_query(const KParams& p, const QueryArgs& q, void* stream, LaunchInfo* info);
struct OcclArgs {
    QueryArgs q;
    const float* tmax;
    uint8_t* out;
    uint32_t mask;
};
int launch_occluded(const KParams& p, const OcclArgs& a, void* stream, LaunchInfo* info);
struct RadArgs {
    const rb_ray* rays;
    const uint32_t* seeds;
    float* colors;
    rb_radiance* out;
    uint32_t* queue;
    uint32_t n;
    uint32_t seed_base;
    uint32_t first_sample, samples;
    uint32_t batch, magic_S;
};
int launch_radiance(const KParams& p, const RadArgs& a, void* stream, LaunchInfo* info, bool records = false);
struct CamGenArgs {
    rb_camera_ex cam;
    rb_ray* recs;
    uint32_t* seeds;
    uint32_t first_pixel;
// ... 89 lines not shown
size_t lightmap_work_bytes(uint32_t n_tris);
int lightmap_surfels(const LmArgs& g, rb_surfel* surfels, uint32_t* owners, void* work, uint64_t piece_units, void* stream);
int launch_lightmap_resolve(const rb_radiance* sums, uint32_t width, uint32_t height, uint32_t dilate, float* out, float* tmp, void* stream);
Cam host_cam(const rb_uniforms& u);

struct GuidePlanes {
    float* nt;
    float* pc;
    float* al;
};
enum : uint32_t { kDenoisePlain = 1, kDenoiseLds = 2 };
struct DenoiseArgs {
    uint32_t w, h;
    const float* accum;
    const float* color4;
    GuidePlanes g;
    float* r[2];
    float* linear_out;
    uint32_t* rgba_out;
    uint32_t variant;
};
bool denoise_params_valid(const rb_denoise_params& p, const char** why);
int launch_denoise(const rb_denoise_params& prm, const DenoiseArgs& a, void* stream);
int launch_guide_pack(const rb_uniforms& u, const rb_hit* hits, const rb_surface* surf, uint32_t w, uint32_t h, const GuidePlanes& g, void* stream);
int launch_guide_split(const rb_guide* guides, size_t n, const GuidePlanes& g, void* stream);
int launch_guide_join(const GuidePlanes& g, size_t n, rb_guide* guides, void* stream);

struct ReprojectArgs {
    uint32_t w, h;
    rb_view view;
    const float* prev4;
    GuidePlanes prev;
    GuidePlanes cur;
    const float* cur4;
    float* out4;
};
bool reproject_params_valid(const rb_reproject_params& p, const char** why);
bool view_finite(const rb_view& v);
int launch_reproject(const rb_reproject_params& prm, const ReprojectArgs& a, void* stream);
int launch_history_merge(uint32_t w, uint32_t h, const float* accum, const float* base, const GuidePlanes& g, float* out4, void* stream);

int launch_render(const KParams& p, uint32_t kernel, bool stats, void* stream, LaunchInfo* info);
int launch_accumulate(const KParams& p, void* stream);
int launch_prep_tris(const rb_gpu_triangle* tris, uint32_t tri_count, const uint32_t* indices,
                     uint32_t index_len, PrepTri* out, PrepTriShade* shade, void* stream);
int launch_prep_materials(void* first_material, uint32_t stride, uint32_t n, void* stream);
int launch_prep_sphere_scan(const rb_sphere* spheres, uint32_t n, float* out, void* stream);
int launch_gather_tris(const PrepTri* ptris, const uint32_t* slots, uint32_t n, PrepTri* out, void* stream);
int launch_chunk_gather(const PrepTri* ptris, const uint32_t* pos_slot, const uint32_t* pos_rank, uint32_t n, float* a,
                        float* b, float* c, void* stream);
int launch_deinterleave(const uint32_t* gathered, uint32_t* frame, uint32_t width, uint32_t height, uint32_t padded_rows,
                        uint32_t stripe_rows, uint32_t shard_count, void* stream);
size_t max_dynamic_lds(int device);
int debug_walk_profile(unsigned long long* out64, int reset);
int device_cu_count(int device);
uint32_t device_cu_count_cached();
uint32_t stream_kernel_max_threads(uint32_t blocks_per_cu);

}
```

### renderbaby_amd/csrc/rb_kernels.hip

```cpp
#include "rb_device_shade.hpp"

namespace rb {
namespace {
constexpr float kChunkFMax = 1.5e5f;
constexpr float kChunkKS = 24.0f * 5.9604645e-8f * 1.01f;
constexpr float kChunkKP = 12.0f * 5.9604645e-8f * 1.01f;
constexpr float kChunkKT = 11.0f * 5.9604645e-8f * 1.01f;
constexpr float kChunkKD = 16.0f * 5.9604645e-8f * 1.01f;
}
}
#define RB_CHUNK_MARGINS_DEFINED
#include "rb_device_chunk.hpp"
#include "rb_launch_plan.hpp"
#include "rb_host_cam.hpp"

#pragma clang fp contract(off)

namespace rb {
namespace {

constexpr uint32_t kPixelBlock = 256;

template <bool STATS>
__global__ void __launch_bounds__(kPixelBlock) k_pixel(const KParams p) {
    extern __shared__ __attribute__((aligned(16))) uint32_t s_stack[];
    const uint32_t tid = threadIdx.x;
    const uint32_t wave = tid >> 6, lane = tid & 63u;
    const uint32_t tiles_x = (p.u.width + 15u) / 16u;
    const uint32_t bx = blockIdx.x % tiles_x, by = blockIdx.x / tiles_x;
    const uint32_t x = bx * 16u + (wave & 1u) * 8u + (lane & 7u);
    const uint32_t ly = by * 16u + (wave >> 1) * 8u + (lane >> 3);
    Tally<STATS> tl;
    bool active = (x < p.u.width) && (ly < p.local_rows);
    uint32_t y = 0;
    if (active) {
        y = global_row(p, ly);
        active = y < p.u.height;
    }
    if (active) {
        const uint32_t pixel_index = y * p.u.width + x;
        const float4 a4 = reinterpret_cast<const float4*>(p.accum_in)[(size_t)ly * p.u.width + x];
        f3 acc = mk(a4.x, a4.y, a4.z);
        uint32_t total = f2u(a4.w);
        for (uint32_t pass = p.first_pass; pass < p.first_pass + p.n_passes; pass++) {
            for (uint32_t s = 0; s < p.samples_per_pass; s++) {
                Path pt;
                start_path(fresh_params(p), x, y, pixel_index, pass * p.samples_per_pass + s, pt);
                if (p.u.max_depth > 0u) {
                    while (segment<STATS>(p, pt, &s_stack[tid], kPixelBlock, tl)) {
                    }
                }
                tl.paths++;
                acc = acc + pt.color;
                total = total + 1u;
            }
        }
        store_pixel(p, x, ly, acc, total);
    }
    flush_tally<STATS>(tl, p.counters);
}

constexpr uint32_t kQueueBlock = 256;

template <bool STATS>
__global__ void __launch_bounds__(kQueueBlock) k_queue(const KParams p) {
    extern __shared__ __attribute__((aligned(16))) uint32_t s_stack[];
// ... 222 lines not shown
            uint32_t b = 0;
            if (lane == 0u) b = atomicAdd(p.queue, batch);
            b = (uint32_t)__builtin_amdgcn_readfirstlane((int)b);
            if (b >= total_items) return false;
            loc_next = b;
            loc_end = (total_items - b < batch) ? total_items : b + batch;
            return true;
        }
        while (tried < p.queue_groups) {
            uint32_t b = 0;
            if (lane == 0u) b = atomicAdd(p.queue + grp * kQueueStride, batch);
            b = (uint32_t)__builtin_amdgcn_readfirstlane((int)b);
            uint32_t it = 0;
            if (band_item(p, grp, b, total_items, it)) {
                loc_next = it;
                loc_end = (total_items - it < batch) ? total_items : it + batch;
                return true;
            }
            grp = (grp + 1u == p.queue_groups) ? 0u : grp + 1u;
            tried++;
        }
        return false;
    }

    template <class IsIdle, class OnItem>
    DEV void refill(const KParams& p, uint32_t lane, uint32_t total_items, uint32_t S, uint32_t tiles_x,
                    uint32_t sample_base, IsIdle&& is_idle, OnItem&& on_item) {
        unsigned long long idle = __ballot(is_idle());
        for (int round = 0; round < 2 && idle != 0ull; round++) {
            if (loc_next == loc_end) {
                if (exhausted) break;
                if (!reserve(p, lane, total_items)) {
                    exhausted = true;
                    break;
                }
            }
            const ItemRows rows = item_rows(p, loc_next, S, tiles_x, sample_base);
            const uint32_t avail = loc_end - loc_next;
            const uint32_t rank = (uint32_t)__popcll(idle & ((1ull << lane) - 1ull));
            const bool take = ((idle >> lane) & 1ull) != 0ull && rank < avail;
            const uint32_t n_idle = (uint32_t)__popcll(idle);
            const uint32_t taken = n_idle < avail ? n_idle : avail;
            if (take) {
                uint32_t x = 0, y = 0, sample_hash = 0;
                if (item_pixel(p, rows, rank, x, y, sample_hash)) on_item(loc_next + rank, x, y, sample_hash);
            }
            loc_next += taken;
            idle = __ballot(is_idle());
            if (taken == n_idle) break;
        }
    }
};

template <bool STATS, bool MULTI, bool STAGED, bool JOINED, bool UV = true>
DEV void trace_body(const KParams& p, v4f* s_ring) {
    extern __shared__ __attribute__((aligned(16))) uint32_t s_stack[];
    const uint32_t tid = threadIdx.x;
    const uint32_t lane = tid & 63u;
    const uint32_t tiles_x = (p.u.width + 7u) / 8u;
    const uint32_t tiles_y = (p.local_rows + 7u) / 8u;
    const uint32_t S = p.n_passes * p.samples_per_pass;
    const uint32_t total_items = tiles_x * tiles_y * S * 64u;
    float4* __restrict__ colors = reinterpret_cast<float4*>(p.colors);
    Tally<STATS> tl;
    ColorRing cring(s_ring, tid >> 6, lane, STAGED ? kRingWaveStaged : kRingWave);
    bool active = false, exhausted = false;
    uint32_t item = 0;
    uint32_t loc_next = 0, loc_end = 0;
    const uint32_t batch = p.queue_batch;
    {
        const uint64_t first = (uint64_t)(blockIdx.x * (kTraceBlock / 64u) + (tid >> 6)) * batch;
        if (first < total_items) {
            loc_next = (uint32_t)__builtin_amdgcn_readfirstlane((int)(uint32_t)first);
            loc_end = (total_items - loc_next < batch) ? total_items : loc_next + batch;
        }
    }
    Path pt;
    pt.depth = 0;

    for (;;) {
        unsigned long long idle = __ballot(!active);
        uint32_t box = kBoxUnknown;
        for (int round = 0; round < 2 && idle != 0ull; round++) {
            if (loc_next == loc_end) {
                if (exhausted) break;
                uint32_t b = 0;
                if (lane == 0u) b = atomicAdd(p.queue, batch);
                b = (uint32_t)__builtin_amdgcn_readfirstlane((int)b);
                if (b >= total_items) {
                    exhausted = true;
                    break;
                }
                loc_next = b;
                loc_end = (total_items - b < batch) ? total_items : b + batch;
            }
            const KParams& rp = fresh_params(p);
            const uint32_t rS = rp.n_passes * rp.samples_per_pass, r_tiles_x = (rp.u.width + 7u) / 8u;
            const uint32_t r_sample_base = rp.first_pass * rp.samples_per_pass, r_width = rp.u.width;
            const uint32_t direct_mask = (rp.queue_batch % (kRingRows * 64u)) ? kDirect : 0u;
            const ItemRows rows = item_rows(rp, loc_next, rS, r_tiles_x, r_sample_base);
            const uint32_t avail = loc_end - loc_next;
            const uint32_t rank = (uint32_t)__popcll(idle & ((1ull << lane) - 1ull));
            const bool take = !active && rank < avail;
            const uint32_t n_idle = (uint32_t)__popcll(idle);
            const uint32_t taken = n_idle < avail ? n_idle : avail;
            if constexpr (STAGED) {
                if (rows.in0 == 0u || rows.in0 + taken > 64u) {
                    const uint32_t nx = rows.in0 != 0u ? 1u : 0u, row = (loc_next >> 6) + nx;
                    cring.open_row(colors, lane, row, active, item);
                    cring.stage_row(rp, lane, row, rows.tx[nx], rows.ty[nx], rows.hs[nx]);
                    __builtin_amdgcn_fence(__ATOMIC_ACQ_REL, "wavefront");
                }
                if (take) {
                    const uint32_t it = loc_next + rank;
                    if (cring.take(it, pt.d, pt.seed, box)) {
                        pt.o = ld3(rp.cam.pos);
                        pt.color = mk(0, 0, 0);
                        pt.att = mk(1, 1, 1);
                        pt.depth = 0;
                        item = it;
                        if (rp.u.max_depth > 0u) {
                            active = true;
                        } else {
                            colors[it] = make_float4(0.0f, 0.0f, 0.0f, 0.0f);
                            tl.paths++;
                        }
                    }
                }
            } else {
                if (direct_mask == 0u) {
                    if (rows.in0 == 0u) cring.open_row(colors, lane, loc_next >> 6, active, item);
                    else if (rows.in0 + taken > 64u) cring.open_row(colors, lane, (loc_next >> 6) + 1u, active, item);
                }
                if (take) {
                    const uint32_t it = loc_next + rank;
                    uint32_t x = 0, y = 0, sample_hash = 0;
                    if (item_pixel(rp, rows, rank, x, y, sample_hash)) {
                        start_path_hashed(rp, x, y, y * r_width + x, sample_hash, pt);
                        item = it | direct_mask;
                        if (rp.u.max_depth > 0u) {
                            active = true;
                        } else {
                            colors[it] = make_float4(0.0f, 0.0f, 0.0f, 0.0f);
                            tl.paths++;
                        }
                    }
                }
            }
            loc_next += taken;
            idle = __ballot(!active) & ~0ull;
            if (taken == n_idle) break;
        }
        if (__ballot(active) == 0ull && exhausted && loc_next == loc_end) break;
        if (active) {
            const bool alive = segment<STATS, MULTI, JOINED, !MULTI, UV>(p, pt, &s_stack[tid], kTraceBlock, tl, box);
            if (!alive) {
                cring.finish(colors, item, pt.color);
                tl.paths++;
                active = false;
            }
        }
    }
    for (uint32_t k = 0; k < kRingRows; k++) cring.drain(colors, lane, k);
    flush_tally<STATS>(tl, fresh_params(p).counters);
}
template <bool STATS, bool MULTI, int WAVES = RB_TRACE_WAVES>
__global__ void __launch_bounds__(kTraceBlock, WAVES) k_trace(const KParams p) {
    __shared__ __attribute__((aligned(16))) v4f s_ring[(kTraceBlock / 64u) * (MULTI ? kRingWave : kRingWaveStaged)];
    trace_body<STATS, MULTI, !MULTI, !(STATS && MULTI)>(p, s_ring);
}
template <bool STATS, bool MULTI, int WAVES = RB_TRACE_WAVES>
__global__ void __launch_bounds__(kTraceBlock, WAVES) k_trace_direct(const KParams p) {
    __shared__ __attribute__((aligned(16))) v4f s_ring[(kTraceBlock / 64u) * kRingRows * 64u];
    trace_body<STATS, MULTI, false, STATS || MULTI>(p, s_ring);
}
#define RB_TRACE_FLAT (RB_TRIP_BLOCK && RB_TRIP_PLAIN != 0)
#if RB_TRACE_FLAT
template <int WAVES>
__global__ void __launch_bounds__(kTraceBlock, WAVES) k_trace_flat(const KParams p) {
    __shared__ __attribute__((aligned(16))) v4f s_ring[(kTraceBlock / 64u) * kRingWaveStaged];
    trace_body<false, false, true, true, false>(p, s_ring);
}
template <int WAVES>
__global__ void __launch_bounds__(kTraceBlock, WAVES) k_trace_flat_direct(const KParams p) {
    __shared__ __attribute__((aligned(16))) v4f s_ring[(kTraceBlock / 64u) * kRingRows * 64u];
    trace_body<false, false, false, false, false>(p, s_ring);
}
#endif

#ifndef RB_BVH_WAVES
#define RB_BVH_WAVES 1
#endif
template <bool STATS, bool LDS, uint32_t BLOCK>
__global__ void __launch_bounds__(BLOCK, RB_BVH_WAVES) k_trace_bvh(const KParams p) {
    extern __shared__ __attribute__((aligned(16))) uint32_t s_stack[];
    const uint32_t tid = threadIdx.x;
    const uint32_t lane = tid & 63u;
    const uint32_t width = p.u.width;
    const uint32_t tiles_x = (width + 7u) / 8u;
    const uint32_t tiles_y = (p.local_rows + 7u) / 8u;
    const uint32_t S = p.n_passes * p.samples_per_pass;
    const uint32_t total_items = tiles_x * tiles_y * S * 64u;
    const uint32_t sample_base = p.first_pass * p.samples_per_pass;
    const uint32_t node_count = p.u.bvh_node_count;
    float4* __restrict__ colors = reinterpret_cast<float4*>(p.colors);
    const cf4p nodes = (cf4p)p.nodes;
    const cf4p ptris = (cf4p)p.ptris;
    uint32_t* const stack = stack_column(s_stack, tid);
    Tally<STATS> tl;

    v4f* const lds_nodes = reinterpret_cast<v4f*>(s_stack + p.stack_depth * BLOCK);
    v4f* const lds_tris = lds_nodes + node_count * 3u;
    if constexpr (LDS) {
        const v4f* gn = reinterpret_cast<const v4f*>(p.nodes);
        const v4f* gt = reinterpret_cast<const v4f*>(p.ptris);
        for (uint32_t i = tid; i < node_count * 3u; i += BLOCK) lds_nodes[i] = gn[i];
        for (uint32_t i = tid; i < p.index_len * 3u; i += BLOCK) {
            const uint32_t slot = i / 3u, part = i - slot * 3u;
            lds_tris[i] = gt[slot * 4u + part];
        }
        __syncthreads();
    }
    auto node_q = [&](uint32_t idx, uint32_t part) -> v4f {
        if constexpr (LDS) return lds_nodes[idx * 3u + part];
        else return nodes[idx * 3u + part];
    };
    auto tri_q = [&](uint32_t slot, uint32_t part) -> v4f {
        if constexpr (LDS) return lds_tris[slot * 3u + part];
        else return ptris[slot * 4u + part];
    };

    enum : uint32_t { IDLE = 0, BEGIN = 1, TRAV = 2, FINISH = 3 };
    uint32_t state = IDLE;
    uint32_t item = 0;
    ItemQueue iq(p, total_items);
    Path pt;
    pt.depth = 0;
    TriHit th;
    th.hit = false;
    th.t = 1e20f;
// ... 774 lines not shown

uint32_t device_cu_count_cached() {
    static int cached[64] = {0};
    int dev = 0;
    (void)hipGetDevice(&dev);
    if (dev < 0 || dev >= 64) return (uint32_t)device_cu_count(dev);
    if (cached[dev] == 0) cached[dev] = device_cu_count(dev);
    return (uint32_t)cached[dev];
}

uint32_t stream_kernel_max_threads(uint32_t blocks_per_cu) {
    return device_cu_count_cached() * (blocks_per_cu ? blocks_per_cu : 8u) * 256u;
}

Cam host_cam(const rb_uniforms& u) {
    auto fast_den = [](float b) {
        uint32_t x;
        __builtin_memcpy(&x, &b, 4);
        x &= 0x7FFFFFFFu;
        return (x - 0x0D800000u) < 0x64000000u && (x - 0x21800000u) < 0x3C000000u && (x & 0x007FFFFFu) != 0x007FFFFFu;
    };
    Cam c{};
    const CamBasis b = host_cam_basis(u.camera, u.width, u.height);
    c.aspect = b.aspect;
    for (int i = 0; i < 3; i++) c.pos[i] = u.camera.pos[i], c.fwd[i] = b.fwd[i], c.right[i] = b.right[i], c.up[i] = b.up[i];
    c.fov = b.fov;
    c.wm1 = b.wm1;
    c.hm1 = b.hm1;
    c.fast_wh = (RB_FAST_DIV && fast_den(c.wm1) && fast_den(c.hm1)) ? 1u : 0u;
    c.inv_wm1 = c.fast_wh ? 1.0f / c.wm1 : 0.0f;
    c.inv_hm1 = c.fast_wh ? 1.0f / c.hm1 : 0.0f;
    return c;
}

using TraceKernel = void (*)(const KParams);
constexpr LaunchConsts kLaunchConsts = {kTraceBlock, kRingRows, kTraceManyItems, kChunkWaveLds, kSphWaveLds, RB_SPH_WAVES, RB_CHUNK_WAVES, RB_XCD_BANDS != 0,
                                        RB_TRACE_FLAT != 0};
template <bool STATS>
static TraceKernel trace_kernel(const LaunchPlan& pl) {
    switch (pl.variant) {
        case kTraceSph: return k_trace_sph<STATS>;
        case kTraceChunk: return pl.sph_tree ? k_trace_chunk<STATS, true> : k_trace_chunk<STATS, false>;
        case kTraceFast: return k_trace_fast<STATS>;
        case kTraceBvhLds: return k_trace_bvh<STATS, true, 1024u>;
        case kTraceBvh: return k_trace_bvh<STATS, false, kTraceBlock>;
        case kTracePlain: break;
    }
    if (pl.plain == kPlainMulti) return k_trace<STATS, true>;
#if RB_TRACE_FLAT
    if constexpr (!STATS)
        if (pl.flat) {
            constexpr int W6 = RB_TRACE_WAVES, W8 = RB_TRACE_WAVES_BIG;
            const bool staged = pl.plain == kPlainStaged;
            return pl.big ? (staged ? k_trace_flat<W8> : k_trace_flat_direct<W8>) : (staged ? k_trace_flat<W6> : k_trace_flat_direct<W6>);
        }
#endif
    if constexpr (!STATS)
        if (pl.big) return pl.plain == kPlainStaged ? k_trace<false, false, RB_TRACE_WAVES_BIG> : k_trace_direct<false, false, RB_TRACE_WAVES_BIG>;
    return pl.plain == kPlainStaged ? k_trace<STATS, false> : k_trace_direct<STATS, false>;
}

int launch_render(const KParams& p_, uint32_t kernel, bool stats, void* stream_, LaunchInfo* info) {
    KParams p = p_;
    p.cam = host_cam(p.u);
    hipStream_t stream = static_cast<hipStream_t>(stream_);
    LaunchInfo li{};
    const size_t lds = (size_t)kStackEntryBytes * p.stack_depth * 256u;
    li.lds_bytes = lds;
    if (kernel == RB_KERNEL_PIXEL) {
        const uint32_t tiles_x = (p.u.width + 15u) / 16u, tiles_y = (p.local_rows + 15u) / 16u;
        li.grid = tiles_x * tiles_y;
        li.block = kPixelBlock;
        li.kernel_name = "k_pixel";
        if (li.grid == 0) return 0;
        if (stats)
            hipLaunchKernelGGL(k_pixel<true>, dim3(li.grid), dim3(li.block), lds, stream, p);
        else
            hipLaunchKernelGGL(k_pixel<false>, dim3(li.grid), dim3(li.block), lds, stream, p);
    } else if (kernel == RB_KERNEL_QUEUE) {
        const uint64_t items = (uint64_t)((p.u.width + 7u) / 8u) * ((p.local_rows + 7u) / 8u) * 64u;
        li.grid = persistent_blocks(items, kQueueBlock, device_cu_count_cached(), p.blocks_per_cu ? p.blocks_per_cu : 8u);
        li.block = kQueueBlock;
        li.kernel_name = "k_queue";
        if (li.grid == 0) return 0;
        hipError_t e = hipMemsetAsync(p.queue, 0, sizeof(uint32_t), stream);
        if (e != hipSuccess) return (int)e;
        if (stats)
            hipLaunchKernelGGL(k_queue<true>, dim3(li.grid), dim3(li.block), lds, stream, p);
        else
            hipLaunchKernelGGL(k_queue<false>, dim3(li.grid), dim3(li.block), lds, stream, p);
    } else {
        int dev = 0;
        (void)hipGetDevice(&dev);
        const LaunchPlan pl = plan_launch(p, stats, device_cu_count_cached(), max_dynamic_lds(dev), kLaunchConsts);
        li = pl.li;
        if (li.grid == 0) return 0;
        if (pl.variant == kTracePlain)
            li.trace_form = (pl.flat ? RB_TRACE_FORM_FLAT : 0u) | (pl.big ? RB_TRACE_FORM_BIG : 0u) | (pl.plain == kPlainStaged ? RB_TRACE_FORM_STAGED : 0u) |
                            (pl.plain == kPlainMulti ? RB_TRACE_FORM_MULTI : 0u);
        KParams q = p;
        q.queue_batch = pl.queue_batch, q.queue_groups = pl.queue_groups, q.queue_region = pl.queue_region;
        q.magic_S = pl.magic_S, q.magic_tiles_x = pl.magic_tiles_x;
        hipError_t e = hipSuccess;
        if (pl.queue_groups > 1u) {
            QueueInit qi;
            for (uint32_t g = 0; g < kQueueGroups; g++) qi.start[g] = pl.queue_start[g];
            hipLaunchKernelGGL(k_queue_init, dim3(1), dim3(64), 0, stream, p.queue, qi);
            e = hipGetLastError();
        } else {
            e = hipMemsetD32Async(reinterpret_cast<hipDeviceptr_t>(p.queue), (int)pl.queue_start[0], 1, stream);
        }
        if (e != hipSuccess) return (int)e;
        const TraceKernel fn = stats ? trace_kernel<true>(pl) : trace_kernel<false>(pl);
        if (pl.variant == kTraceBvhLds) {
            e = hipFuncSetAttribute(reinterpret_cast<const void*>(fn), hipFuncAttributeMaxDynamicSharedMemorySize, (int)li.lds_bytes);
            if (e != hipSuccess) return (int)e;
        }
        hipLaunchKernelGGL(fn, dim3(li.grid), dim3(li.block), li.lds_bytes, stream, q);
    }
    if (info) *info = li;
    return (int)hipGetLastError();
}

int launch_accumulate(const KParams& p, void* stream_) {
    const uint64_t tiles = (uint64_t)((p.u.width + 7u) / 8u) * ((p.local_rows + 7u) / 8u);
    if (tiles == 0 || p.n_passes * p.samples_per_pass == 0) return 0;
    hipLaunchKernelGGL(k_accumulate, dim3((uint32_t)((tiles + 3u) / 4u)), dim3(256), 0, static_cast<hipStream_t>(stream_), p);
    return (int)hipGetLastError();
}

int launch_prep_tris(const rb_gpu_triangle* tris, uint32_t tri_count, const uint32_t* indices,
                     uint32_t index_len, PrepTri* out, PrepTriShade* shade, void* stream_) {
    if (index_len == 0) return 0;
    hipStream_t stream = static_cast<hipStream_t>(stream_);
    const uint32_t block = 256, grid = (index_len + block - 1) / block;
    hipLaunchKernelGGL(k_prep_tris, dim3(grid), dim3(block), 0, stream, tris, tri_count, indices, index_len, out,
                       shade);
    return (int)hipGetLastError();
}

int launch_prep_materials(void* first_material, uint32_t stride, uint32_t n, void* stream_) {
    if (n == 0) return 0;
    hipStream_t stream = static_cast<hipStream_t>(stream_);
    hipLaunchKernelGGL(k_prep_materials, dim3((n + 255) / 256), dim3(256), 0, stream,
                       static_cast<unsigned char*>(first_material), stride, n);
    return (int)hipGetLastError();
}

int launch_prep_sphere_scan(const rb_sphere* spheres, uint32_t n, float* out, void* stream_) {
    if (n == 0) return 0;
    hipStream_t stream = static_cast<hipStream_t>(stream_);
// ... 41 lines not shown
```

### renderbaby_amd/csrc/rb_launch_plan.hpp

```cpp
#pragma once
#include <algorithm>
#include <cstdint>

#include "rb_internal.hpp"

namespace rb {

struct LaunchConsts {
    uint32_t trace_block, ring_rows;
    uint64_t many_items;
    uint32_t chunk_wave_lds, sph_wave_lds;
    uint32_t sph_waves, chunk_waves;
    bool xcd_bands;
    bool flat = false;
};

enum TraceVariant : uint32_t { kTracePlain, kTraceBvh, kTraceBvhLds, kTraceFast, kTraceSph, kTraceChunk };
enum PlainKind : uint32_t { kPlainMulti, kPlainStaged, kPlainDirect };

struct LaunchPlan {
    TraceVariant variant = kTracePlain;
    LaunchInfo li{};
    PlainKind plain = kPlainDirect;
    bool big = false;
    bool flat = false;
    bool sph_tree = false;
    uint32_t queue_batch = 0, queue_groups = 1, queue_region = 0, magic_S = 0, magic_tiles_x = 0;
    uint32_t queue_start[kQueueGroups] = {};
};

inline uint32_t dense_blocks_per_cu(uint64_t items, uint32_t cus) { return (items >= (uint64_t)cus * 8u * 4u * 1024u) ? 8u : 4u; }

inline uint32_t persistent_blocks(uint64_t items, uint32_t block, uint32_t cus, uint32_t blocks_per_cu) {
    uint32_t blocks = cus * blocks_per_cu;
    const uint64_t needed = (items + block - 1) / block;
    if (needed < blocks) blocks = (uint32_t)needed;
    return blocks;
}

inline uint64_t reservation(uint64_t items, uint64_t waves, bool plain) {
    uint64_t batch = items / (waves * (plain ? 8u : 64u));
    batch = (batch / 64u) * 64u;
    if (batch < 64u) batch = 64u;
    if (batch > (plain ? 512u : 4096u)) batch = (plain ? 512u : 4096u);
    return batch;
}

inline uint32_t magic_of(uint64_t d) { return d > 1u ? (uint32_t)((1ull << 32) / d) : 0xFFFFFFFFu; }

inline LaunchPlan plan_launch(const KParams& p, bool stats, uint32_t cus, size_t max_lds, const LaunchConsts& k) {
    LaunchPlan pl;
    const size_t lds = (size_t)kStackEntryBytes * p.stack_depth * 256u;
    const uint64_t tiles = (uint64_t)((p.u.width + 7u) / 8u) * ((p.local_rows + 7u) / 8u);
    const uint64_t items = tiles * 64u * p.n_passes * p.samples_per_pass;
    const bool multi = p.u.bvh_node_count > 1u && !p.no_leaf_stepping;
    const size_t scene_lds = (size_t)p.u.bvh_node_count * 48u + (size_t)p.index_len * 48u;
    TraceVariant v = kTracePlain;
    if (multi && p.chunk_nodes != nullptr) v = kTraceChunk;
    else if (multi && p.fast_nodes != nullptr) v = kTraceFast;
    else if (multi) v = (p.lds_mode != 1u && lds * 4u + scene_lds <= max_lds) ? kTraceBvhLds : kTraceBvh;
    else if (p.sph_nodes != nullptr && !p.no_leaf_stepping) v = kTraceSph;
    static const char* const names[] = {"k_trace", "k_trace_bvh", "k_trace_bvh_lds", "k_trace_fast", "k_trace_sph", "k_trace_chunk"};
    pl.variant = v;
    pl.sph_tree = p.sph_nodes != nullptr;
    pl.li.kernel_name = names[v];
    pl.li.block = v == kTraceBvhLds ? 1024u : k.trace_block;
    pl.li.lds_bytes = v == kTraceBvhLds ? lds * 4u + scene_lds : v == kTraceChunk ? lds + (k.trace_block / 64u) * k.chunk_wave_lds
                                        : v == kTraceSph ? lds + (k.trace_block / 64u) * k.sph_wave_lds : lds;
    const uint32_t blocks_per_cu = v == kTraceBvhLds ? 1u : p.blocks_per_cu ? p.blocks_per_cu : v == kTraceFast ? 4u : v == kTraceSph ? k.sph_waves
                                                                                                   : v == kTraceChunk ? k.chunk_waves : dense_blocks_per_cu(items, cus);
    pl.li.grid = persistent_blocks(items, pl.li.block, cus, blocks_per_cu);
    if (pl.li.grid == 0) return pl;
    const uint64_t waves = (uint64_t)pl.li.grid * (pl.li.block / 64u);
    uint64_t batch = reservation(items, waves, v == kTracePlain);
    if (v == kTracePlain && batch >= 256u) batch = (batch / 256u) * 256u;
    if (p.queue_batch) batch = p.queue_batch;
    pl.queue_batch = (uint32_t)batch;
    pl.magic_S = magic_of((uint64_t)p.n_passes * p.samples_per_pass);
    pl.magic_tiles_x = magic_of((p.u.width + 7u) / 8u);
    const uint64_t row_items = (uint64_t)((p.u.width + 7u) / 8u) * 64u * p.n_passes * p.samples_per_pass;
    const uint64_t stripe = std::max<uint64_t>(((4u * row_items + batch - 1u) / batch) * batch, 8u * batch);
    const bool banded = v != kTracePlain && k.xcd_bands && pl.li.grid >= kQueueGroups && items >= 4u * kQueueGroups * stripe && stripe < (1ull << 30);
    if (banded) {
        pl.queue_groups = kQueueGroups;
        pl.queue_region = (uint32_t)stripe;
        for (uint32_t g = 0; g < kQueueGroups; g++) {
            const uint64_t blocks_g = (pl.li.grid + kQueueGroups - 1u - g) / kQueueGroups;
            pl.queue_start[g] = (uint32_t)std::min<uint64_t>(blocks_g * (pl.li.block / 64u) * batch, 0x7FFFFFFFull);
        }
    } else {
        pl.queue_start[0] = (uint32_t)(waves * batch);
    }
    if (v == kTracePlain) {
        pl.plain = (p.u.bvh_node_count > 1u || p.sph_nodes != nullptr) ? kPlainMulti
                   : pl.queue_batch % (k.ring_rows * 64u) == 0u        ? kPlainStaged : kPlainDirect;
        pl.big = pl.plain != kPlainMulti && !stats && items >= k.many_items;
        pl.flat = k.flat && pl.plain != kPlainMulti && !stats && p.no_uv != 0u;
    }
    return pl;
}

}
```

### renderbaby_amd/csrc/rb_runtime.cpp

```cpp
#include <cmath>
#include <cstdarg>
#include <cstdio>
#include <cstdlib>
#include <cstring>

#include "rb_engine.hpp"

static thread_local std::string g_create_error;

int rb::fail(const rb_engine* e, int code, const char* fmt, ...) {
    char buf[512];
    va_list ap;
    va_start(ap, fmt);
    vsnprintf(buf, sizeof buf, fmt, ap);
    va_end(ap);
    if (e) {
        std::lock_guard<std::mutex> g(e->err_mu);
        e->error = buf;
    } else {
        g_create_error = buf;
    }
    return code;
}

namespace {

using rb::copy_error, rb::ensure_prepared, rb::make_params, rb::require_ready;

int resize_frame(rb_engine* e, uint32_t w, uint32_t h, const rb::ShardLayout& rows) {
    const uint64_t px = static_cast<uint64_t>(w) * rows.padded;
    if (px >= (1ull << 31)) return rb::fail(e, RB_ERR_INVALID_UNIFORMS, "frame of %u x %u pixels is too large", w, h);
    HIP_TRY(e, hipStreamSynchronize(e->stream));
    e->spec_valid = false;
    e->cur = 0;
    e->slot[1].accum.release();
    e->slot[1].rgba.release();
    rb::FrameSlot& s = e->slot[0];
    HIP_TRY(e, s.accum.resize(px * 4));
    HIP_TRY(e, s.rgba.resize(px));
    if (px) {
        HIP_TRY(e, hipMemsetAsync(s.accum.ptr, 0, px * 16, e->stream));
        HIP_TRY(e, hipMemsetAsync(s.rgba.ptr, 0, px * 4, e->stream));
    }
    return RB_OK;
}

int upload_textures(rb_engine* e, const rb_texture* t, size_t count) {
    std::vector<uint32_t> data;
    std::vector<rb_texture_info> info;
    uint32_t offset = 0;
    for (size_t i = 0; i < count; ++i) {
        const size_t n = static_cast<size_t>(t[i].width) * t[i].height;
        info.push_back(rb_texture_info{offset, t[i].width, t[i].height, 0});
        data.insert(data.end(), t[i].rgba_data, t[i].rgba_data + n);
        offset += t[i].width * t[i].height;
    }
    int rc = rb::upload(e, e->tex_data, data.data(), data.size(), true);
    if (rc) return rc;
    rc = rb::upload(e, e->tex_info, info.data(), info.size(), true);
    if (rc) return rc;
    HIP_TRY(e, hipStreamSynchronize(e->stream));
    return RB_OK;
}

int prep_sphere_scan(rb_engine* e) {
    const size_t n = e->spheres.count;
    HIP_TRY(e, e->sph_scan.resize(n * 4));
    int rc = rb::launch_prep_sphere_scan(e->spheres.ptr, static_cast<uint32_t>(n), e->sph_scan.ptr, e->stream);
    if (rc) return rb::fail(e, RB_ERR_DEVICE, "sphere scan prep launch failed: %s", hipGetErrorString(static_cast<hipError_t>(rc)));
    return RB_OK;
}

int prep_materials(rb_engine* e, rb_material* first, size_t stride, size_t n) {
    if (!first || n == 0) return RB_OK;
    int rc = rb::launch_prep_materials(first, static_cast<uint32_t>(stride), static_cast<uint32_t>(n), e->stream);
    if (rc) return rb::fail(e, RB_ERR_DEVICE, "material prep launch failed: %s", hipGetErrorString(static_cast<hipError_t>(rc)));
    return RB_OK;
}

template <typename T>
void keep_host_copy(rb_engine* e, const void* src, size_t n, std::vector<T>& copy, size_t& len, bool& stale) {
    if (!rb::mesh_walks(e->opt).host_mesh) return;
    len = n;
    stale = rb::host_copy_can_wait(e, n);
    if (stale) std::vector<T>().swap(copy);
    else copy.assign(static_cast<const T*>(src), static_cast<const T*>(src) + n);
}

int apply_field(rb_engine* e, rb::Field f, const rb::UpdatePlan& pl, const rb_config* cfg) {
    using namespace rb;
    if (f == kUniforms) {
        if (pl.act[f] == Act::Take) {
            const rb_uniforms* u = static_cast<const rb_uniforms*>(cfg->uniforms.ptr);
            if (pl.resize || e->slot[0].accum.ptr == nullptr)
                if (const int rc = resize_frame(e, u->width, u->height, pl.frame)) return rc;
            e->prh.total_samples = u->total_samples;
            e->prh.total_passes = (u->total_samples + e->prh.samples_per_pass - 1) / e->prh.samples_per_pass;
        }
        commit_field(e->sc, pl, cfg, f);
        return RB_OK;
    }
    if (pl.act[f] == Act::None) return RB_OK;
    const bool del = pl.act[f] == Act::Delete;
    const void* src = del ? nullptr : field_of(cfg, f).ptr;
    const size_t n = del ? 0 : field_of(cfg, f).count;
    int rc = RB_OK;
    switch (f) {
        case kSpheres: rc = upload(e, e->spheres, src, n, true); break;
        case kUvs: rc = upload(e, e->uvs, src, n, true); break;
        case kMeshes: rc = upload(e, e->meshes, src, n, true); break;
        case kLights: rc = upload(e, e->lights, src, n, !del); break;
        case kNodes: rc = upload(e, e->nodes, src, n, true); break;
        case kIndices: rc = upload(e, e->indices, src, n, true); break;
        case kTriangles: rc = upload(e, e->tris, src, n, true); break;
        case kTextures: rc = upload_textures(e, static_cast<const rb_texture*>(src), n); break;
        default: break;
    }
    if (rc) return rc;
    commit_field(e->sc, pl, cfg, f);
    switch (f) {
        case kSpheres:
            rc = prep_materials(e, &e->spheres.ptr->material, sizeof(rb_sphere), n);
            if (!rc) rc = prep_sphere_scan(e);
            if (!rc) rc = build_sphere_bvh(e, static_cast<const rb_sphere*>(src), n);
            break;
        case kMeshes: rc = prep_materials(e, &e->meshes.ptr->material, sizeof(rb_mesh), n); break;
        case kLights: rc = prep_materials(e, e->lights.ptr ? &e->lights.ptr->material : nullptr, sizeof(rb_point_light), e->sc.n_lights); break;
        case kNodes:
            e->prep_dirty = true;
            e->tree = {n ? "caller" : "", 0.0f};
            break;
        case kIndices:
            e->prep_dirty = true;
            keep_host_copy(e, src, n, e->host_indices, e->host_index_len, e->host_indices_stale);
            break;
        case kTriangles:
            e->prep_dirty = true;
            keep_host_copy(e, src, n, e->host_tris, e->host_tri_len, e->host_tris_stale);
            break;
        default: break;
    }
    return rc;
}

}

int rb::ensure_prepared(rb_engine* e) {
    const uint32_t tri_count = rb::triangle_count(e->sc);
    if (!e->prep_dirty && e->prep_tri_count == tri_count) return RB_OK;
    const uint32_t len = e->sc.n_indices;
    HIP_TRY(e, e->ptris.resize(len));
    HIP_TRY(e, e->pshade.resize(len));
    int rc = rb::launch_prep_tris(e->tris.ptr, tri_count, e->indices.ptr, len, e->ptris.ptr, e->pshade.ptr, e->stream);
    if (rc) return rb::fail(e, RB_ERR_DEVICE, "prep kernel launch failed: %s", hipGetErrorString(static_cast<hipError_t>(rc)));
    e->prep_dirty = false;
    e->prep_tri_count = tri_count;
    e->chunk.rec = e->own.rec = {};
    rc = rb::build_chunk_tree(e, tri_count);
    return (rc || e->chunk.rec.built()) ? rc : rb::build_own_tree(e, tri_count);
}

rb::KParams rb::make_params(rb_engine* e, uint32_t first_pass, uint32_t n_passes, int src, int dst) {
    rb::KParams p{};
    p.u = e->sc.uniforms;
    p.u.spheres_count = rb::spheres_count(e->sc);
    p.u.bvh_node_count = rb::node_count(e->sc);
    p.u.bvh_triangle_count = rb::triangle_count(e->sc);
    p.spheres = e->spheres.ptr;
    p.sph_scan = e->sph_scan.ptr;
    p.lights = e->lights.ptr;
    p.meshes = e->meshes.ptr;
    p.nodes = e->nodes.ptr;
    p.indices = e->indices.ptr;
    p.tris = e->tris.ptr;
    p.ptris = e->ptris.ptr;
    p.pshade = e->pshade.ptr;
    p.uvs = e->uvs.ptr;
    p.tex_data = e->tex_data.ptr;
    p.tex_info = e->tex_info.ptr;
    p.srgb_lut = e->srgb_lut.ptr;
    p.accum_in = e->slot[src].accum.ptr;
    p.accum_out = e->slot[dst].accum.ptr;
    p.out_rgba = e->slot[dst].rgba.ptr;
    p.counters = e->counters.ptr;
    p.queue = e->queue.ptr;
    p.n_lights = e->sc.n_lights;
    p.n_meshes = e->sc.n_meshes;
    p.index_len = e->sc.n_indices;
    p.n_uvs = e->sc.n_uvs;
    p.n_tex = e->sc.n_tex;
    p.first_pass = first_pass;
    p.n_passes = n_passes;
    p.samples_per_pass = e->prh.samples_per_pass;
    const rb::ShardLayout rows = e->sc.layout(e->sc.height);
    p.shard_rank = rows.rank;
    p.shard_count = rows.count;
    p.stripe_rows = rows.stripe;
    p.local_rows = e->sc.local_rows;
    p.colors = e->colors.ptr;
    p.stack_depth = rb::accel_params(e, p);
    e->stack_depth_covers = p.stack_depth <= rb::kStackDepth;
    p.blocks_per_cu = e->opt._reserved[0];
    p.queue_batch = e->opt._reserved[2] ? std::min<uint32_t>(((std::min<uint32_t>(e->opt._reserved[2], 4096u) + 63u) / 64u) * 64u, 4096u) : 0u;
    p.no_leaf_stepping = e->opt._reserved[3];
    p.lds_mode = e->opt._reserved[4];
    const bool single = p.u.bvh_node_count <= 1u && p.sph_nodes == nullptr && !e->trace_uv;
    p.no_uv = (single && e->sc.no_uv && (e->sc.untex_lights || p.u.ground_enabled == 0u)) ? 1u : 0u;
    return p;
}

int rb::require_ready(rb_engine* e) {
    if (!e->sc.initialized) return rb::fail(e, RB_ERR_NOT_INITIALIZED, "engine has not received its first update");
    if (!e->scene_valid) return rb::fail(e, RB_ERR_DEVICE, "the last update failed half-way on the device; send the scene again");
    if (!e->sc.have_uniforms) return rb::fail(e, RB_ERR_UNIFORMS_NOT_INITIALIZED, "Uniforms must be initialized");
    return RB_OK;
}

void rb::copy_error(rb_engine* g, const rb_engine* part) {
    std::string msg;
    {
        std::lock_guard<std::mutex> l(part->err_mu);
        msg = part->error;
    }
    std::lock_guard<std::mutex> l(g->err_mu);
    g->error = "device " + std::to_string(part->device) + ": " + msg;
}

namespace {

int clear_accum(rb_engine* e) {
    const size_t px = static_cast<size_t>(e->sc.width) * e->sc.padded_rows;
    e->spec_valid = false;
    if (px) HIP_TRY(e, hipMemsetAsync(e->slot[e->cur].accum.ptr, 0, px * 16, e->stream));
    return RB_OK;
}

int accumulate_timing(rb_engine* e) {
    float ms = 0.0f;
    if (e->last_launches > 0) {
        HIP_TRY(e, hipEventSynchronize(e->ev_end));
        HIP_TRY(e, hipEventElapsedTime(&ms, e->ev_begin, e->ev_end));
    }
    e->last_dispatch_ms = ms;
    if (e->timing_pending) {
        e->stats.kernel_ms += ms;
        for (uint32_t i = 0; i + 4 <= e->ev_used; i += 4) {
            float t = 0.0f, a = 0.0f;
            HIP_TRY(e, hipEventElapsedTime(&t, e->ev_pool[i], e->ev_pool[i + 1]));
            HIP_TRY(e, hipEventElapsedTime(&a, e->ev_pool[i + 2], e->ev_pool[i + 3]));
            e->stats.trace_ms += t;
            e->stats.accumulate_ms += a;
        }
        e->timing_pending = false;
    }
    return RB_OK;
}

uint64_t color_budget_bytes(rb_engine* e) {
    if (e->opt._reserved[1]) return static_cast<uint64_t>(e->opt._reserved[1]) << 20;
    if (e->color_budget == 0) {
// ... 231 lines not shown
        }
        const uint32_t n2 = std::min(per, e->prh.total_passes - e->prh.current_pass);
        rc = dispatch(e, e->prh.current_pass, n2, e->cur, 1 - e->cur);
        if (rc) return rc;
        e->spec_valid = true;
        e->spec_first = e->prh.current_pass;
        e->spec_n = n2;
    }
    return RB_OK;
}

int iter_next_locked(rb_engine* e, uint8_t* rgba_out) {
    if (!(e->prh.current_pass < e->prh.total_passes))
        return rb::fail(e, RB_ERR_NO_MORE_FRAMES, "No more frames available");
    const bool multiproc = e->net.nranks > 1;
    if (!rgba_out && !(multiproc && e->net.rank != 0)) return rb::fail(e, RB_ERR_NULL_ARGUMENT, "rgba_out is NULL");
    int rc = iter_advance(e, e->iter_passes_per_frame);
    if (rc) return rc;
    if (multiproc) {
        std::string why;
        if (rb::gather_process(e->net, e->slot[e->cur].rgba.ptr, e->sc.width, e->sc.height, e->sc.padded_rows,
                               e->sc.layout(e->sc.height).stripe, e->copy_stream, e->slot[e->cur].done,
                               rgba_out, why))
            return rb::fail(e, RB_ERR_DEVICE, "%s", why.c_str());
        return RB_OK;
    }
    return read_slot_rgba(e, e->cur, rgba_out);
}

rb_engine* create_single(const rb_config* cfg, const rb_options& opt) {
    if (opt.shard_count > 1 && opt.shard_rank >= opt.shard_count) {
        rb::fail(nullptr, RB_ERR_INVALID_OPTIONS, "shard_rank %u >= shard_count %u", opt.shard_rank, opt.shard_count);
        return nullptr;
    }
    if (opt.kernel > RB_KERNEL_STREAM) { rb::fail(nullptr, RB_ERR_INVALID_OPTIONS, "unknown kernel %u", opt.kernel); return nullptr; }
    if ((opt.flags & rb::kBuildTreeFlags) == rb::kBuildTreeFlags) {
        rb::fail(nullptr, RB_ERR_INVALID_OPTIONS, "RB_FLAG_BUILD_TREE and RB_FLAG_BUILD_TREE_HOST exclude each other");
        return nullptr;
    }
    int dev = opt.device;
    if (dev < 0) {
        if (hipGetDevice(&dev) != hipSuccess) { rb::fail(nullptr, RB_ERR_DEVICE, "no HIP device available"); return nullptr; }
    }
    if (hipSetDevice(dev) != hipSuccess) { rb::fail(nullptr, RB_ERR_DEVICE, "hipSetDevice(%d) failed", dev); return nullptr; }
    rb_engine* e = new rb_engine();
    e->device = dev;
    e->opt = opt;
    e->sc.own_tree = rb::builds_tree(opt);
    e->sc.shard_rank = opt.shard_rank, e->sc.shard_count = opt.shard_count, e->sc.stripe_rows = opt.stripe_rows;
    if (const char* rw = std::getenv("RB_REFERENCE_WALK"); rw && rw[0] == '1')
        e->opt.flags = (e->opt.flags & ~(rb::kOwnTreeFlags | RB_FLAG_DEVICE_LBVH | RB_FLAG_CHUNK_WALK | RB_FLAG_SKIP_NEAR_DEGENERATE)) |
                       RB_FLAG_REFERENCE_WALK;
    if (const char* uv = std::getenv("RB_TRACE_UV"); uv && uv[0] == '1') e->trace_uv = true;
    auto bail = [&](const char* what, hipError_t st) -> rb_engine* {
        rb::fail(nullptr, RB_ERR_DEVICE, "%s failed: %s", what, hipGetErrorString(st));
        rb_destroy(e);
        return nullptr;
    };
    hipError_t st;
    if ((st = hipStreamCreateWithFlags(&e->stream, hipStreamNonBlocking)) != hipSuccess) return bail("hipStreamCreate", st);
    if ((st = hipStreamCreateWithFlags(&e->copy_stream, hipStreamNonBlocking)) != hipSuccess) return bail("hipStreamCreate", st);
    if ((st = hipStreamCreateWithFlags(&e->accum_stream, hipStreamNonBlocking)) != hipSuccess) return bail("hipStreamCreate", st);
    if ((st = hipStreamCreateWithFlags(&e->trace_stream, hipStreamNonBlocking)) != hipSuccess) return bail("hipStreamCreate", st);
    for (hipEvent_t* x : {&e->ev_top, &e->ev_traced[0], &e->ev_traced[1], &e->ev_accumulated[0], &e->ev_accumulated[1]})
        if ((st = hipEventCreateWithFlags(x, hipEventDisableTiming)) != hipSuccess) return bail("hipEventCreate", st);
    if ((st = hipEventCreate(&e->ev_begin)) != hipSuccess) return bail("hipEventCreate", st);
    if ((st = hipEventCreate(&e->ev_end)) != hipSuccess) return bail("hipEventCreate", st);
    for (rb::FrameSlot& s : e->slot)
        if ((st = hipEventCreateWithFlags(&s.done, hipEventDisableTiming)) != hipSuccess) return bail("hipEventCreate", st);
    if ((st = e->counters.resize(rb::C_COUNT)) != hipSuccess) return bail("hipMalloc(counters)", st);
    if ((st = e->queue.resize(2 * rb::kQueueWords)) != hipSuccess) return bail("hipMalloc(queue)", st);
    if ((st = hipMemsetAsync(e->counters.ptr, 0, sizeof(unsigned long long) * rb::C_COUNT, e->stream)) != hipSuccess)
        return bail("hipMemset(counters)", st);
    float lut[256];
    for (int i = 0; i < 256; ++i) lut[i] = powf(static_cast<float>(i) / 255.0f, 2.2f);
    if ((st = e->srgb_lut.resize(256)) != hipSuccess) return bail("hipMalloc(lut)", st);
    if ((st = hipMemcpy(e->srgb_lut.ptr, lut, sizeof lut, hipMemcpyHostToDevice)) != hipSuccess) return bail("hipMemcpy(lut)", st);
    const rb_uniforms* u = static_cast<const rb_uniforms*>(cfg->uniforms.ptr);
    e->prh.samples_per_pass = 1;
    e->prh.total_samples = u->total_samples;
    e->prh.total_passes = u->total_samples;
    e->prh.current_pass = 0;
    return e;
}

bool check_create(const rb_config* cfg) {
    g_create_error.clear();
    int rc = rb::check_tags(cfg, g_create_error);
    if (!rc) rc = rb::check_first_config(cfg, g_create_error);
    return rc == RB_OK;
}

rb_engine* create_impl(const rb_config* cfg, const rb_options* opt_in) {
    if (!check_create(cfg)) return nullptr;
    rb_options opt{};
    opt.device = -1;
    if (opt_in) opt = *opt_in;
    return create_single(cfg, opt);
}

#define PART_TRY(g, part, call)            \
    do {                                   \
        rb::set_device(part);              \
        const int _rc = (call);            \
        if (_rc) {                         \
            copy_error((g), (part));       \
// ... 492 lines not shown
        if (rc) return rc;
    }
    HIP_TRY(e, hipMemsetAsync(e->counters.ptr, 0, sizeof(unsigned long long) * rb::C_COUNT, e->stream));
    e->stats = rb_stats{};
    return RB_OK;
}

int rb_last_dispatch_ms(rb_engine* e, float* ms) {
    if (!e || !ms) return RB_ERR_NULL_ARGUMENT;
    std::lock_guard<std::mutex> lock(e->mu);
    if (rb::is_group(e)) {
        *ms = 0.0f;
        for (auto& p : e->parts) {
            PART_TRY(e, p.get(), accumulate_timing(p.get()));
            *ms = std::max(*ms, p->last_dispatch_ms);
        }
        return RB_OK;
    }
    rb::set_device(e);
    int rc = accumulate_timing(e);
    if (rc) return rc;
    *ms = e->last_dispatch_ms;
    return RB_OK;
}

const char* rb_version(void) { return "renderbaby-hip 0.3 (gfx950)"; }

const char* rb_last_kernel_name(const rb_engine* e) {
    if (!e) return "";
    return rb::is_group(e) ? e->parts[0]->last_kernel_name : e->last_kernel_name;
}

uint32_t rb_debug_trace_form(const rb_engine* e) {
    if (!e) return 0u;
    return rb::is_group(e) ? e->parts[0]->last_trace_form : e->last_trace_form;
}

int rb_device_name(int device, char* buf, size_t buf_len) {
    if (!buf || buf_len == 0) return RB_ERR_NULL_ARGUMENT;
    hipDeviceProp_t prop;
    if (device < 0 && hipGetDevice(&device) != hipSuccess) return RB_ERR_DEVICE;
    if (hipGetDeviceProperties(&prop, device) != hipSuccess) return RB_ERR_DEVICE;
    snprintf(buf, buf_len, "%s (%s, %d CUs)", prop.name, prop.gcnArchName, prop.multiProcessorCount);
    return RB_OK;
}

int rb_debug_walk_profile(uint64_t out64[64], int reset) {
    if (!out64) return RB_ERR_NULL_ARGUMENT;
    static_assert(sizeof(unsigned long long) == sizeof(uint64_t), "counter width");
    if (hipDeviceSynchronize() != hipSuccess) return RB_ERR_DEVICE;
    return rb::debug_walk_profile(reinterpret_cast<unsigned long long*>(out64), reset) == 0 ? RB_OK : RB_ERR_DEVICE;
}

}
```

### renderbaby_amd/engine.py

```python
import ctypes as C
from dataclasses import dataclass
from functools import partial
from typing import Any, List, Optional

import numpy as np

from . import abi
from ._lib import load
from .bvh import own_tree_readback, sphere_tree_readback
from ._marshal import (SEEDS, Form, device_new, device_tensor, download, grid_records, host_in, host_out, host_ptr, is_tensor, probe_records,
                       ray_records, surfel_records, torch_device, upload)


class RenderError(RuntimeError):

    def __init__(self, code, message):
        super().__init__(f"[{abi.ERR.get(code, code)}] {message}")
        self.code = code
        self.message = message


@dataclass
class Change:
    tag: int
# ... 318 lines not shown
    def clear(self):
        self._check(self._lib.rb_clear(self._h))

    def dispatch(self, first_pass, n_passes):
        self._check(self._lib.rb_dispatch(self._h, first_pass, n_passes))

    def reserve(self, n_passes):
        self._check(self._lib.rb_reserve(self._h, n_passes))

    def sync(self):
        self._check(self._lib.rb_sync(self._h))

    def read_rgba(self):
        w, h = self._frame_shape()
        out = np.empty((h, w, 4), dtype=np.uint8)
        self._check(self._lib.rb_read_rgba(self._h, out.ctypes.data))
        return out

    def read_accumulation(self):
        w, h = self._frame_shape()
        out = np.empty((h, w, 4), dtype=np.float32)
        self._check(self._lib.rb_read_accumulation(self._h, out.ctypes.data))
        return out

    def device_rgba(self):
        p, n = C.c_void_p(), C.c_size_t()
        self._check(self._lib.rb_device_rgba(self._h, C.byref(p), C.byref(n)))
        return p.value, n.value

    def local_rows(self):
        r, pr = C.c_uint32(), C.c_uint32()
        self._check(self._lib.rb_local_rows(self._h, C.byref(r), C.byref(pr)))
        return r.value, pr.value

    def global_row(self, local_row):
        g = C.c_uint32()
        self._check(self._lib.rb_global_row(self._h, local_row, C.byref(g)))
        return g.value

    def stats(self):
        s = abi.Stats()
        self._check(self._lib.rb_get_stats(self._h, C.byref(s)))
        return s.as_dict()

    def reset_stats(self):
        self._check(self._lib.rb_reset_stats(self._h))

    def last_kernel_name(self):
        return (self._lib.rb_last_kernel_name(self._h) or b"").decode()

    def trace_form(self):
        return int(self._lib.rb_debug_trace_form(self._h))

    _ray_records = staticmethod(ray_records)

    def _device_call(self, fn, *args):
        import torch
        torch.cuda.current_stream(self.query_device).synchronize()
        self._check(fn(self._h, *args))
        self._check(self._lib.rb_sync(self._h))

    def _query(self, form, name, *args):
        if form.on_device:
            self._device_call(getattr(self._lib, name + "_device"), *args)
        else:
            self._check(getattr(self._lib, name)(self._h, *args))

    def _staged(self, *arrays):
        f = Form(self.query_device, *arrays, staged=True)
        return f, partial(self._query, f)

    def _last_ms(self, fn, count=1):
        ms = [C.c_float() for _ in range(count)]
        self._check(fn(self._h, *[C.byref(m) for m in ms]))
        return ms[0].value if count == 1 else tuple(m.value for m in ms)

    def _builder(self, fn):
        ms = C.c_float()
        name = (fn(self._h, C.byref(ms)) or b"").decode()
        return name, ms.value

    def cast_rays(self, origins, dirs, surfaces=False, hits_out=None, surfaces_out=None):
        return self.cast_ray_records(ray_records(origins, dirs), surfaces, hits_out, surfaces_out)

    def cast_ray_records(self, rays, surfaces=False, hits_out=None, surfaces_out=None):
        f = Form(self.query_device, rays, hits_out, surfaces_out)
        rays, rp = f.input("rays", rays, abi.RAY, flat=False)
        n = len(rays)
        hits, hp = f.output("hits_out", hits_out, abi.HIT, n)
        surf, sp = f.output("surfaces_out", surfaces_out, abi.SURFACE, n) if (surfaces or surfaces_out is not None) else (None, None)
        self._query(f, "rb_cast_rays", rp, n, hp, sp)
        return hits if surf is None else (hits, surf)

    def occluded(self, origins, dirs, tmax=None, mask=abi.MASK_ALL, out=None):
        return self.occluded_records(ray_records(origins, dirs), tmax, mask, out)

    def occluded_records(self, rays, tmax=None, mask=abi.MASK_ALL, out=None):
        f = Form(self.query_device, rays, tmax, out)
        rays, rp = f.input("rays", rays, abi.RAY, flat=False)
        n = len(rays)
        tmax, tp = f.optional("tmax", tmax, np.float32, n)
        res, op = f.output("out", out, np.uint8, n)
        self._query(f, "rb_occluded", rp, tp, n, int(mask), op)
        return res

    def trace_rays(self, origins, dirs, seeds=None, samples=1, first_sample=0, out=None):
# ... 514 lines not shown
```

Measured before the change: 40180 Msamples/s.

## Add conservative triangle sift prefilter that culls leaf triangles before the hand-laid test

```diff
diff --git a/include/rb_abi.h b/include/rb_abi.h
--- a/include/rb_abi.h
+++ b/include/rb_abi.h
@@ -325,6 +325,8 @@
 int rb_debug_rcp_det_exhaustive(uint32_t biased_exponent, uint32_t* out16);
 int rb_debug_triangle_trip(uint32_t n, uint32_t seed, uint32_t* out32);
 int rb_debug_triangle_trip_flat(uint32_t n, uint32_t seed, uint32_t* out32);
+int rb_debug_triangle_trip_vec(uint32_t n, uint32_t seed, uint32_t uv, uint32_t* out32);
+int rb_debug_tri_filter(rb_engine* e, const float* rays, uint32_t n, uint32_t* out, uint32_t* list2);
 int rb_debug_root_box(const float* rays, uint32_t n, const float* box6, uint32_t* out);
 int rb_debug_normalize_sites(const float* xyz, uint32_t n, uint32_t n_unit, uint32_t seed0, uint32_t n_seeds, uint32_t* out16);
 int rb_measure_salu_mix(int32_t device, uint32_t scalar_per_16, uint32_t branch, double* out3);
@@ -335,6 +337,7 @@
 const char* rb_last_kernel_name(const rb_engine* e);
 enum {
     RB_TRACE_FORM_FLAT = 1u,
+    RB_TRACE_FORM_SIFT = 2u,
     RB_TRACE_FORM_BIG = 4u,
     RB_TRACE_FORM_STAGED = 8u,
     RB_TRACE_FORM_MULTI = 16u
diff --git a/renderbaby_amd/_lib.py b/renderbaby_amd/_lib.py
--- a/renderbaby_amd/_lib.py
+++ b/renderbaby_amd/_lib.py
@@ -59,6 +59,8 @@
     "rb_debug_rnd_pm1_exhaustive": (i32, [vp]),
     "rb_debug_triangle_trip": (i32, [u32, u32, vp]),
     "rb_debug_triangle_trip_flat": (i32, [u32, u32, vp]),
+    "rb_debug_triangle_trip_vec": (i32, [u32, u32, u32, vp]),
+    "rb_debug_tri_filter": (i32, [vp, vp, u32, vp, vp]),
     "rb_debug_trace_form": (u32, [vp]),
     "rb_debug_root_box": (i32, [vp, u32, vp, vp]),
     "rb_debug_normalize_sites": (i32, [vp, u32, u32, u32, u32, vp]),
diff --git a/renderbaby_amd/abi.py b/renderbaby_amd/abi.py
--- a/renderbaby_amd/abi.py
+++ b/renderbaby_amd/abi.py
@@ -114,6 +114,7 @@
 
 KERNEL_DEFAULT, KERNEL_PIXEL, KERNEL_QUEUE, KERNEL_STREAM = 0, 1, 2, 3
 TRACE_FORM_FLAT, TRACE_FORM_BIG, TRACE_FORM_STAGED, TRACE_FORM_MULTI = 1, 4, 8, 16
+TRACE_FORM_SIFT = 2
 FLAG_STATS = 1
 FLAG_NO_SPHERE_BVH = 2
 FLAG_FAST_BVH = 4
diff --git a/renderbaby_amd/csrc/rb_debug.hip b/renderbaby_amd/csrc/rb_debug.hip
--- a/renderbaby_amd/csrc/rb_debug.hip
+++ b/renderbaby_amd/csrc/rb_debug.hip
@@ -136,8 +136,8 @@
     s = pcg(s);
     return (float)(int32_t)s * 0x1p-31f;
 }
-template <bool FLAT>
-__global__ void __launch_bounds__(256) k_triangle_trip(uint32_t n_waves, uint32_t seed, uint32_t* mismatch) {
+template <bool FLAT, bool VREC>
+DEV void trip_sweep(uint32_t n_waves, uint32_t seed, uint32_t* mismatch) {
     const uint32_t wave = (blockIdx.x * 256u + threadIdx.x) >> 6, lane = threadIdx.x & 63u;
     if (wave >= n_waves + kTripCases) return;
     f3 o, d, v0, e1, e2;
@@ -165,6 +165,9 @@
     const v4f ra = {uni(v0.x), uni(v0.y), uni(v0.z), 0.0f}, rb_ = {uni(e1.x), uni(e1.y), uni(e1.z), 0.0f},
               rc = {uni(e2.x), uni(e2.y), uni(e2.z), 1.0f};
     const uint32_t slot = (uint32_t)__builtin_amdgcn_readfirstlane((int)(wave + 1u));
+    v4f va = {v0.x, v0.y, v0.z, 0.0f}, vb = {e1.x, e1.y, e1.z, 0.0f}, vc = {e2.x, e2.y, e2.z, 1.0f};
+    uint32_t vslot = wave + 1u;
+    if constexpr (VREC) asm volatile("" : "+v"(va.x), "+v"(va.y), "+v"(va.z), "+v"(vb.x), "+v"(vb.y), "+v"(vb.z), "+v"(vc.x), "+v"(vc.y), "+v"(vc.z), "+v"(vslot));
     if (wave >= n_waves) {
         TriHit own;
         own.t = 1e20f, own.u = 0.0f, own.v = 0.0f, own.slot = 0u, own.hit = false;
@@ -182,9 +185,11 @@
         if constexpr (FLAT && RB_TRIP_BLOCK) {
             TriHitT<false> flat;
             flat.t = got.t, flat.slot = got.slot, flat.hit = false;
-            accept_trip<RB_TRIP_ASM - 1, false>(ra, rb_, rc, slot, o, d, big, flat);
+            if constexpr (VREC) accept_trip<RB_TRIP_ASM - 1, false, true>(va, vb, vc, vslot, o, d, big, flat);
+            else accept_trip<RB_TRIP_ASM - 1, false>(ra, rb_, rc, slot, o, d, big, flat);
             got.t = flat.t, got.slot = flat.slot, got.u = want.u, got.v = want.v;
-        } else if constexpr (RB_TRIP_BLOCK) accept_trip<RB_TRIP_ASM - 1>(ra, rb_, rc, slot, o, d, big, got);
+        } else if constexpr (RB_TRIP_BLOCK && VREC) accept_trip<RB_TRIP_ASM - 1, true, true>(va, vb, vc, vslot, o, d, big, got);
+        else if constexpr (RB_TRIP_BLOCK) accept_trip<RB_TRIP_ASM - 1>(ra, rb_, rc, slot, o, d, big, got);
         else accept_slot<true>(ra, rb_, rc, slot, o, d, got);
     }
     if (__float_as_uint(want.t) != __float_as_uint(got.t) || __float_as_uint(want.u) != __float_as_uint(got.u) ||
@@ -199,6 +204,29 @@
             mismatch[25] = want.slot;
         }
     }
+}
+
+template <bool FLAT>
+__global__ void __launch_bounds__(256) k_triangle_trip(uint32_t n_waves, uint32_t seed, uint32_t* mismatch) {
+    trip_sweep<FLAT, false>(n_waves, seed, mismatch);
+}
+template <bool FLAT>
+__global__ void __launch_bounds__(256) k_triangle_trip_vec(uint32_t n_waves, uint32_t seed, uint32_t* mismatch) {
+    trip_sweep<FLAT, true>(n_waves, seed, mismatch);
+}
+
+__global__ void __launch_bounds__(256) k_tri_filter(const KParams p, const float* rays, uint32_t n, uint32_t first, uint32_t end, uint32_t* out) {
+    const uint32_t i = blockIdx.x * 256u + threadIdx.x;
+    if (i >= n) return;
+    const f3 o = mk(rays[i * 6u], rays[i * 6u + 1u], rays[i * 6u + 2u]), d = mk(rays[i * 6u + 3u], rays[i * 6u + 4u], rays[i * 6u + 5u]);
+    const SiftRay r = sift_ray(p, o, d);
+    uint32_t ends = p.sift_block_ends, g0 = 0u, b = 0u;
+    for (uint32_t base = first; base < end && b < 4u; base += 32u, ends >>= 8, b++) {
+        const uint32_t g1 = ends & 0xFFu;
+        out[i * 4u + b] = sift_block(p, r, d, g0, g1, (end - base < 32u) ? end - base : 32u);
+        g0 = g1;
+    }
+    for (; b < 4u; b++) out[i * 4u + b] = 0u;
 }
 
 template <int SALU, bool BRANCH>
@@ -432,6 +460,15 @@
     return best;
 }
 }
+
+int debug_tri_filter(const KParams& p, const float* rays, uint32_t n, uint32_t first, uint32_t end, uint32_t* out) {
+    const size_t out_bytes = (size_t)n * 16u, in_bytes = (size_t)n * 24u;
+    return round_trip(out, out_bytes, out_bytes + in_bytes, [&](uint32_t* d) {
+        float* dr = reinterpret_cast<float*>(d + (size_t)n * 4u);
+        (void)hipMemcpy(dr, rays, in_bytes, hipMemcpyHostToDevice);
+        hipLaunchKernelGGL(k_tri_filter, dim3((n + 255u) / 256u), dim3(256), 0, nullptr, p, dr, n, first, end, d);
+    });
+}
 }
 
 extern "C" {
@@ -466,6 +503,16 @@
     return rb::round_trip(out32, 128, 128, [&](uint32_t* d) {
         const uint32_t n_waves = (n + 63u) / 64u, waves = n_waves + rb::kTripCases;
         hipLaunchKernelGGL(rb::k_triangle_trip<true>, dim3((waves + 3u) / 4u), dim3(256), 0, nullptr, n_waves, seed, d);
+    });
+}
+
+int rb_debug_triangle_trip_vec(uint32_t n, uint32_t seed, uint32_t uv, uint32_t* out32) {
+    if (!out32) return RB_ERR_NULL_ARGUMENT;
+    if (n > (1u << 26)) return RB_ERR_INVALID_OPTIONS;
+    return rb::round_trip(out32, 128, 128, [&](uint32_t* d) {
+        const uint32_t n_waves = (n + 63u) / 64u, waves = n_waves + rb::kTripCases;
+        if (uv) hipLaunchKernelGGL(rb::k_triangle_trip_vec<false>, dim3((waves + 3u) / 4u), dim3(256), 0, nullptr, n_waves, seed, d);
+        else hipLaunchKernelGGL(rb::k_triangle_trip_vec<true>, dim3((waves + 3u) / 4u), dim3(256), 0, nullptr, n_waves, seed, d);
     });
 }
 
diff --git a/renderbaby_amd/csrc/rb_device_intersect.hpp b/renderbaby_amd/csrc/rb_device_intersect.hpp
--- a/renderbaby_amd/csrc/rb_device_intersect.hpp
+++ b/renderbaby_amd/csrc/rb_device_intersect.hpp
@@ -204,7 +204,7 @@
 #endif
 #define RB_TRIP_BLOCK (RB_TRIP_ASM != 0 && RB_FAST_RCP && RB_RCP_DET)
 
-template <int SKIP, bool UV = true>
+template <int SKIP, bool UV = true, bool VREC = false>
 DEV void accept_trip(const v4f a, const v4f b, const v4f c, uint32_t slot, f3 o, f3 d, float big, TriHitT<UV>& hit) {
     float r8, r10, r11, r12, r13, r14, r15, r16, r17;
     uint64_t entry, keep, m, ds;
@@ -298,13 +298,13 @@
     [r8] "=&v"(r8), [r10] "=&v"(r10),                                                                                     \
       [r11] "=&v"(r11), [r12] "=&v"(r12), [r13] "=&v"(r13), [r14] "=&v"(r14), [r15] "=&v"(r15), [r16] "=&v"(r16),         \
       [r17] "=&v"(r17), [entry] "=&s"(entry), [keep] "=&s"(keep), [m] "=&s"(m), [ds] "=&s"(ds)
-#define RB_TRIP_IN                                                                                                       \
-    [ax] "s"(a.x), [ay] "s"(a.y), [az] "s"(a.z), [bx] "s"(b.x), [by] "s"(b.y), [bz] "s"(b.z), [cx] "s"(c.x),              \
-      [cy] "s"(c.y), [cz] "s"(c.z), [slot] "s"(slot), [ox] "v"(o.x), [oy] "v"(o.y), [oz] "v"(o.z), [dx] "v"(d.x),         \
+#define RB_TRIP_IN(K)                                                                                                    \
+    [ax] K(a.x), [ay] K(a.y), [az] K(a.z), [bx] K(b.x), [by] K(b.y), [bz] K(b.z), [cx] K(c.x),                            \
+      [cy] K(c.y), [cz] K(c.z), [slot] K(slot), [ox] "v"(o.x), [oy] "v"(o.y), [oz] "v"(o.z), [dx] "v"(d.x),               \
       [dy] "v"(d.y), [dz] "v"(d.z), [eps] "s"(1e-6f)
 #define RB_TRIP_CLOBBERS "vcc", "scc"
-#define RB_TRIP_OPS_UV : RB_TRIP_OUT_UV, RB_TRIP_TEMPS : RB_TRIP_IN, [big] "s"(big), [tmin] "s"(0.001f) : RB_TRIP_CLOBBERS
-#define RB_TRIP_OPS_T : RB_TRIP_OUT_T, RB_TRIP_TEMPS : RB_TRIP_IN, [big] "s"(big), [tmin] "s"(0.001f) : RB_TRIP_CLOBBERS
+#define RB_TRIP_OPS_UV(K) : RB_TRIP_OUT_UV, RB_TRIP_TEMPS : RB_TRIP_IN(K), [big] "s"(big), [tmin] "s"(0.001f) : RB_TRIP_CLOBBERS
+#define RB_TRIP_OPS_T(K) : RB_TRIP_OUT_T, RB_TRIP_TEMPS : RB_TRIP_IN(K), [big] "s"(big), [tmin] "s"(0.001f) : RB_TRIP_CLOBBERS
 #define RB_TRIP_SKIP "s_cbranch_execz .Ltrip_end_%=\n\t"
 #define RB_TRIP_EMIT(MOVES, OPS)                                                                                         \
     if constexpr (SKIP == 2) {                                                                                           \
@@ -316,10 +316,14 @@
     } else {                                                                                                             \
         asm volatile(RB_TRIP_HEAD RB_TRIP_TAIL RB_TRIP_LAST MOVES "\ts_mov_b64 exec, %[entry]" OPS);                     \
     }
-    if constexpr (UV) {
-        RB_TRIP_EMIT(RB_TRIP_MOVES_UV, RB_TRIP_OPS_UV)
+    if constexpr (UV && VREC) {
+        RB_TRIP_EMIT(RB_TRIP_MOVES_UV, RB_TRIP_OPS_UV("v"))
+    } else if constexpr (UV) {
+        RB_TRIP_EMIT(RB_TRIP_MOVES_UV, RB_TRIP_OPS_UV("s"))
+    } else if constexpr (VREC) {
+        RB_TRIP_EMIT(RB_TRIP_MOVES_T, RB_TRIP_OPS_T("v"))
     } else {
-        RB_TRIP_EMIT(RB_TRIP_MOVES_T, RB_TRIP_OPS_T)
+        RB_TRIP_EMIT(RB_TRIP_MOVES_T, RB_TRIP_OPS_T("s"))
     }
 #undef RB_TRIP_EMIT
 #undef RB_TRIP_SKIP
@@ -582,6 +586,72 @@
     }
 };
 
+constexpr float kSiftFMax = 1.5e5f;
+struct SiftRay {
+    f3 inv, oi;
+    bool inside;
+};
+DEV SiftRay sift_ray(const KParams& p, f3 o, f3 d) {
+    SiftRay r;
+    r.inv = mk(__builtin_amdgcn_rcpf(d.x), __builtin_amdgcn_rcpf(d.y), __builtin_amdgcn_rcpf(d.z));
+    r.oi = mk(o.x * r.inv.x, o.y * r.inv.y, o.z * r.inv.z);
+    const f3 lo = ld3(p.sift_lo), hi = ld3(p.sift_hi);
+    r.inside = ((__builtin_amdgcn_fcmpf(o.x, lo.x, 2) & __builtin_amdgcn_fcmpf(o.x, hi.x, 4) & __builtin_amdgcn_fcmpf(o.y, lo.y, 2) &
+                 __builtin_amdgcn_fcmpf(o.y, hi.y, 4) & __builtin_amdgcn_fcmpf(o.z, lo.z, 2) & __builtin_amdgcn_fcmpf(o.z, hi.z, 4) &
+                 __builtin_amdgcn_fcmpf(fabsf(r.inv.x), p.sift_rmax, 5) & __builtin_amdgcn_fcmpf(fabsf(r.inv.y), p.sift_rmax, 5) &
+                 __builtin_amdgcn_fcmpf(fabsf(r.inv.z), p.sift_rmax, 5)) >>
+                __lane_id()) & 1ull;
+    return r;
+}
+DEV uint32_t sift_block(const KParams& p, const SiftRay& r, f3 d, uint32_t g0, uint32_t g1, uint32_t n) {
+    const float kp = p.sift_kp, ks = p.sift_ks, kt = p.sift_kt, kd = p.sift_kd;
+    const cf4p groups = (cf4p)p.sift_groups;
+    const f3 inv = r.inv, oi = r.oi;
+    uint32_t cand = 0u;
+    for (uint32_t g = g1; g != g0; g--) {
+        const cf4p rec = groups + (size_t)(g - 1u) * 4u;
+        const v4f r0 = rec[0], r1 = rec[1], r2 = rec[2];
+        const uint32_t count = __float_as_uint(rec[3].y);
+        const float y = __builtin_fmaf(d.z, r2.z, __builtin_fmaf(d.y, r2.y, d.x * r2.x));
+        const float lb = fabsf(y) - r2.w;
+        const float fl = r0.w * __builtin_amdgcn_rcpf(lb);
+        const float f = (lb > 1e-6f && fl < r1.w) ? fl : r1.w;
+        const float mm = __builtin_fmaf(kp, f, ks), thr = 0.001f - __builtin_fmaf(kt, f, kd);
+        const float tcx = __builtin_fmaf(r0.x, inv.x, -oi.x), tcy = __builtin_fmaf(r0.y, inv.y, -oi.y), tcz = __builtin_fmaf(r0.z, inv.z, -oi.z);
+        const float hx = r1.x + mm, hy = r1.y + mm, hz = r1.z + mm;
+        const float ix = fabsf(inv.x), iy = fabsf(inv.y), iz = fabsf(inv.z);
+        const float tn = fmaxf(fmaxf(__builtin_fmaf(-hx, ix, tcx), __builtin_fmaf(-hy, iy, tcy)), __builtin_fmaf(-hz, iz, tcz));
+        const float tf = fminf(fminf(__builtin_fmaf(hx, ix, tcx), __builtin_fmaf(hy, iy, tcy)), __builtin_fmaf(hz, iz, tcz));
+        const uint64_t keep = (__builtin_amdgcn_fcmpf(tf, tn, 11) & __builtin_amdgcn_fcmpf(tf, thr, 11)) | __builtin_amdgcn_fcmpf(f, kSiftFMax, 10);
+        uint32_t ones;
+        asm("v_cndmask_b32_e64 %0, 0, -1, %1" : "=v"(ones) : "s"(keep));
+        cand = __builtin_amdgcn_alignbit(cand, ones, 32u - count);
+    }
+    if (!r.inside) cand = 0xFFFFFFFFu;
+    return cand & (0xFFFFFFFFu >> (32u - n));
+}
+template <bool UV>
+DEV void sift_triangles(const KParams& p, f3 o, f3 d, uint32_t first, uint32_t end, float big, TriHitT<UV>& h) {
+    const SiftRay r = sift_ray(p, o, d);
+    const cf4p ptris = (cf4p)p.ptris;
+    uint32_t ends = p.sift_block_ends, g0 = 0u;
+    for (uint32_t base = first; base < end; base += 32u, ends >>= 8) {
+        const uint32_t g1 = ends & 0xFFu;
+        uint32_t cand = sift_block(p, r, d, g0, g1, (end - base < 32u) ? end - base : 32u);
+        g0 = g1;
+        const cf4p block = ptris + (size_t)base * 4u;
+        while (cand != 0u) {
+            const uint32_t k = (uint32_t)__ffs((int)cand) - 1u;
+            cand &= cand - 1u;
+            const cf4p rec = block + __umul24(k, 4u);
+            v4f a = rec[0], b = rec[1], c = rec[2];
+            uint32_t live = __float_as_uint(c.w);
+            asm volatile("" : "+v"(a.x), "+v"(b.x), "+v"(live));
+            if (live != 0u) accept_trip<RB_TRIP_ASM - 1, UV, true>(a, b, c, base + k, o, d, big, h);
+        }
+    }
+}
+
 template <bool STATS>
 DEV TriHit intersect_bvh_fast(const KParams& p, f3 o, f3 d, uint32_t* stack, uint32_t stride, Tally<STATS>& tl) {
     FastWalk<STATS> w;
@@ -591,9 +661,10 @@
     return w.h;
 }
 
-template <bool STATS, bool MULTI = true, bool TRIP = false, bool UV = true>
+template <bool STATS, bool MULTI = true, bool TRIP = false, bool UV = true, bool SIFT = false>
 DEV TriHitT<UV> intersect_bvh(const KParams& p, f3 o, f3 d, uint32_t* stack, uint32_t stride, Tally<STATS>& tl, uint32_t box = kBoxUnknown) {
     static_assert(UV || (TRIP && !MULTI && RB_TRIP_BLOCK && RB_TRIP_PLAIN != 0), "the flat forms exist for the hand-laid trip only");
+    static_assert(!SIFT || (TRIP && !MULTI && !STATS && RB_TRIP_BLOCK), "the sift is written around the hand-laid trip; counting builds keep the plain loop");
     TriHitT<UV> h;
     h.hit = false;
     h.t = 1e20f;
@@ -639,7 +710,9 @@
                 else accept_slot<!MULTI>(a, b, c, slot, o, d, h);
                 if constexpr (STATS) tl.mesh_hits += (h.t != before) ? 1u : 0u;
             };
-            if constexpr (trip && RB_TRIP_PLAIN != 0) {
+            if constexpr (SIFT) {
+                sift_triangles<UV>(p, o, d, first, end, big, h);
+            } else if constexpr (trip && RB_TRIP_PLAIN != 0) {
                 cf4p rec = ptris + (size_t)first * 4u;
                 for (uint32_t slot = first; slot != end; slot++, rec += 4) {
                     v4f a = rec[0], b = rec[1], c = rec[2];
diff --git a/renderbaby_amd/csrc/rb_device_shade.hpp b/renderbaby_amd/csrc/rb_device_shade.hpp
--- a/renderbaby_amd/csrc/rb_device_shade.hpp
+++ b/renderbaby_amd/csrc/rb_device_shade.hpp
@@ -513,9 +513,9 @@
     return segment_post<STATS, PARK, JOINED, TRIM, UV>(fresh_params(p), pt, th, st, closest_t, sphere_idx, tl);
 }
 
-template <bool STATS, bool MULTI = true, bool JOINED = true, bool TRIP = false, bool UV = true>
+template <bool STATS, bool MULTI = true, bool JOINED = true, bool TRIP = false, bool UV = true, bool SIFT = false>
 DEV bool segment(const KParams& p, Path& pt, uint32_t* stack, uint32_t stride, Tally<STATS>& tl, uint32_t box = kBoxUnknown) {
-    const TriHitT<UV> th = intersect_bvh<STATS, MULTI, TRIP, UV>(fresh_params(p), pt.o, pt.d, stack, stride, tl, box);
+    const TriHitT<UV> th = intersect_bvh<STATS, MULTI, TRIP, UV, SIFT>(fresh_params(p), pt.o, pt.d, stack, stride, tl, box);
     return segment_finish<STATS, MULTI, true, JOINED, !MULTI, TRIP && !MULTI, UV>(p, pt, th, stack, stride, tl);
 }
 
diff --git a/renderbaby_amd/csrc/rb_engine.hpp b/renderbaby_amd/csrc/rb_engine.hpp
--- a/renderbaby_amd/csrc/rb_engine.hpp
+++ b/renderbaby_amd/csrc/rb_engine.hpp
@@ -11,6 +11,7 @@
 #include "rb_internal.hpp"
 #include "rb_rccl.hpp"
 #include "rb_stage_timer.hpp"
+#include "rb_tri_filter.hpp"
 #include "rb_update_plan.hpp"
 
 namespace rb {
@@ -113,6 +114,11 @@
     bool scene_valid = false;
     bool trace_uv = false;
     uint32_t last_trace_form = 0;
+    bool tri_filter = true;
+    rb::SiftTable sift_table;
+    rb::DevBuf<rb::SiftGroup> sift_groups;
+    float sph_box[6] = {0, 0, 0, 0, 0, 0};
+    bool sph_box_any = false;
     rb_progressive prh{};
     bool iter_initialized = false;
     uint32_t iter_passes_per_frame = 1;
diff --git a/renderbaby_amd/csrc/rb_internal.hpp b/renderbaby_amd/csrc/rb_internal.hpp
--- a/renderbaby_amd/csrc/rb_internal.hpp
+++ b/renderbaby_amd/csrc/rb_internal.hpp
@@ -279,6 +279,12 @@
     Cam cam;
     const float* sph_scan;
     uint32_t no_uv;
+    uint32_t sift;
+    const float* sift_groups;
+    uint32_t sift_block_ends;
+    float sift_lo[3], sift_hi[3];
+    float sift_kp, sift_ks, sift_kt, sift_kd;
+    float sift_rmax;
 };
 
 struct LaunchInfo {
@@ -474,6 +480,7 @@
 int launch_deinterleave(const uint32_t* gathered, uint32_t* frame, uint32_t width, uint32_t height, uint32_t padded_rows,
                         uint32_t stripe_rows, uint32_t shard_count, void* stream);
 size_t max_dynamic_lds(int device);
+int debug_tri_filter(const KParams& p, const float* rays, uint32_t n, uint32_t first, uint32_t end, uint32_t* out);
 int debug_walk_profile(unsigned long long* out64, int reset);
 int device_cu_count(int device);
 uint32_t device_cu_count_cached();
diff --git a/renderbaby_amd/csrc/rb_kernels.hip b/renderbaby_amd/csrc/rb_kernels.hip
--- a/renderbaby_amd/csrc/rb_kernels.hip
+++ b/renderbaby_amd/csrc/rb_kernels.hip
@@ -12,6 +12,7 @@
 #define RB_CHUNK_MARGINS_DEFINED
 #include "rb_device_chunk.hpp"
 #include "rb_launch_plan.hpp"
+#include "rb_tri_filter.hpp"
 #include "rb_host_cam.hpp"
 
 #pragma clang fp contract(off)
@@ -340,7 +341,7 @@
     }
 };
 
-template <bool STATS, bool MULTI, bool STAGED, bool JOINED, bool UV = true>
+template <bool STATS, bool MULTI, bool STAGED, bool JOINED, bool UV = true, bool SIFT = false>
 DEV void trace_body(const KParams& p, v4f* s_ring) {
     extern __shared__ __attribute__((aligned(16))) uint32_t s_stack[];
     const uint32_t tid = threadIdx.x;
@@ -441,7 +442,7 @@
         }
         if (__ballot(active) == 0ull && exhausted && loc_next == loc_end) break;
         if (active) {
-            const bool alive = segment<STATS, MULTI, JOINED, !MULTI, UV>(p, pt, &s_stack[tid], kTraceBlock, tl, box);
+            const bool alive = segment<STATS, MULTI, JOINED, !MULTI, UV, SIFT>(p, pt, &s_stack[tid], kTraceBlock, tl, box);
             if (!alive) {
                 cring.finish(colors, item, pt.color);
                 tl.paths++;
@@ -474,6 +475,13 @@
     __shared__ __attribute__((aligned(16))) v4f s_ring[(kTraceBlock / 64u) * kRingRows * 64u];
     trace_body<false, false, false, false, false>(p, s_ring);
 }
+template <int WAVES>
+__global__ void __launch_bounds__(kTraceBlock, WAVES) k_trace_sift(const KParams p) {
+    __shared__ __attribute__((aligned(16))) v4f s_ring[(kTraceBlock / 64u) * kRingWaveStaged];
+    trace_body<false, false, true, true, false, true>(p, s_ring);
+}
+static_assert(kSiftFMax == kChunkFMax && kSiftKS == kChunkKS && kSiftKP == kChunkKP && kSiftKT == kChunkKT && kSiftKD == kChunkKD,
+              "the sift's margins are the chunked walk's");
 #endif
 
 #ifndef RB_BVH_WAVES
@@ -1354,6 +1362,7 @@
         if (pl.flat) {
             constexpr int W6 = RB_TRACE_WAVES, W8 = RB_TRACE_WAVES_BIG;
             const bool staged = pl.plain == kPlainStaged;
+            if (pl.sift) return pl.big ? k_trace_sift<W8> : k_trace_sift<W6>;
             return pl.big ? (staged ? k_trace_flat<W8> : k_trace_flat_direct<W8>) : (staged ? k_trace_flat<W6> : k_trace_flat_direct<W6>);
         }
 #endif
@@ -1398,7 +1407,7 @@
         li = pl.li;
         if (li.grid == 0) return 0;
         if (pl.variant == kTracePlain)
-            li.trace_form = (pl.flat ? RB_TRACE_FORM_FLAT : 0u) | (pl.big ? RB_TRACE_FORM_BIG : 0u) | (pl.plain == kPlainStaged ? RB_TRACE_FORM_STAGED : 0u) |
+            li.trace_form = (pl.sift ? RB_TRACE_FORM_SIFT : 0u) | (pl.flat ? RB_TRACE_FORM_FLAT : 0u) | (pl.big ? RB_TRACE_FORM_BIG : 0u) | (pl.plain == kPlainStaged ? RB_TRACE_FORM_STAGED : 0u) |
                             (pl.plain == kPlainMulti ? RB_TRACE_FORM_MULTI : 0u);
         KParams q = p;
         q.queue_batch = pl.queue_batch, q.queue_groups = pl.queue_groups, q.queue_region = pl.queue_region;
diff --git a/renderbaby_amd/csrc/rb_launch_plan.hpp b/renderbaby_amd/csrc/rb_launch_plan.hpp
--- a/renderbaby_amd/csrc/rb_launch_plan.hpp
+++ b/renderbaby_amd/csrc/rb_launch_plan.hpp
@@ -24,6 +24,7 @@
     PlainKind plain = kPlainDirect;
     bool big = false;
     bool flat = false;
+    bool sift = false;
     bool sph_tree = false;
     uint32_t queue_batch = 0, queue_groups = 1, queue_region = 0, magic_S = 0, magic_tiles_x = 0;
     uint32_t queue_start[kQueueGroups] = {};
@@ -96,6 +97,7 @@
                    : pl.queue_batch % (k.ring_rows * 64u) == 0u        ? kPlainStaged : kPlainDirect;
         pl.big = pl.plain != kPlainMulti && !stats && items >= k.many_items;
         pl.flat = k.flat && pl.plain != kPlainMulti && !stats && p.no_uv != 0u;
+        pl.sift = pl.flat && pl.plain == kPlainStaged && p.sift != 0u && p.u.bvh_node_count == 1u;
     }
     return pl;
 }
diff --git a/renderbaby_amd/csrc/rb_runtime.cpp b/renderbaby_amd/csrc/rb_runtime.cpp
--- a/renderbaby_amd/csrc/rb_runtime.cpp
+++ b/renderbaby_amd/csrc/rb_runtime.cpp
@@ -69,6 +69,41 @@
     int rc = rb::launch_prep_sphere_scan(e->spheres.ptr, static_cast<uint32_t>(n), e->sph_scan.ptr, e->stream);
     if (rc) return rb::fail(e, RB_ERR_DEVICE, "sphere scan prep launch failed: %s", hipGetErrorString(static_cast<hipError_t>(rc)));
     return RB_OK;
+}
+
+int prep_tri_filter(rb_engine* e) {
+    e->sift_table = rb::SiftTable{};
+    if (!e->tri_filter || rb::kernel_of(e->opt) != RB_KERNEL_STREAM || rb::node_count(e->sc) != 1u || !e->nodes.ptr || !e->ptris.ptr) return RB_OK;
+    rb_bvh_node node{};
+    HIP_TRY(e, hipMemcpyAsync(&node, e->nodes.ptr, sizeof node, hipMemcpyDeviceToHost, e->stream));
+    HIP_TRY(e, hipStreamSynchronize(e->stream));
+    const uint32_t len = e->sc.n_indices, first = node.first_primitive, count = node.primitive_count;
+    const uint32_t end = (static_cast<uint64_t>(first) + count < len) ? first + count : len;
+    if (first >= end || end - first > rb::kSiftMaxSlots) return RB_OK;
+    std::vector<rb::PrepTri> list(end);
+    HIP_TRY(e, hipMemcpyAsync(list.data() + first, e->ptris.ptr + first, (end - first) * sizeof(rb::PrepTri), hipMemcpyDeviceToHost, e->stream));
+    HIP_TRY(e, hipStreamSynchronize(e->stream));
+    rb::SiftTable tb;
+    rb::build_sift_table(list.data(), first, end, tb);
+    if (!rb::sift_pays(tb)) return RB_OK;
+    HIP_TRY(e, e->sift_groups.resize(tb.groups.size()));
+    HIP_TRY(e, hipMemcpyAsync(e->sift_groups.ptr, tb.groups.data(), tb.groups.size() * sizeof(rb::SiftGroup), hipMemcpyHostToDevice, e->stream));
+    HIP_TRY(e, hipStreamSynchronize(e->stream));
+    e->sift_table = std::move(tb);
+    return RB_OK;
+}
+
+void keep_sphere_box(rb_engine* e, const rb_sphere* s, size_t n) {
+    e->sph_box_any = false;
+    for (size_t i = 0; s && i < n; ++i) {
+        const float r = std::fabs(s[i].radius) * 1.0001f;
+        for (int k = 0; k < 3; ++k) {
+            const float lo = s[i].center[k] - r, hi = s[i].center[k] + r;
+            e->sph_box[k] = e->sph_box_any ? std::min(e->sph_box[k], lo) : lo;
+            e->sph_box[3 + k] = e->sph_box_any ? std::max(e->sph_box[3 + k], hi) : hi;
+        }
+        e->sph_box_any = true;
+    }
 }
 
 int prep_materials(rb_engine* e, rb_material* first, size_t stride, size_t n) {
@@ -122,6 +157,7 @@
         case kSpheres:
             rc = prep_materials(e, &e->spheres.ptr->material, sizeof(rb_sphere), n);
             if (!rc) rc = prep_sphere_scan(e);
+            keep_sphere_box(e, static_cast<const rb_sphere*>(src), n);
             if (!rc) rc = build_sphere_bvh(e, static_cast<const rb_sphere*>(src), n);
             break;
         case kMeshes: rc = prep_materials(e, &e->meshes.ptr->material, sizeof(rb_mesh), n); break;
@@ -157,7 +193,8 @@
     e->prep_tri_count = tri_count;
     e->chunk.rec = e->own.rec = {};
     rc = rb::build_chunk_tree(e, tri_count);
-    return (rc || e->chunk.rec.built()) ? rc : rb::build_own_tree(e, tri_count);
+    if (!rc && !e->chunk.rec.built()) rc = rb::build_own_tree(e, tri_count);
+    return rc ? rc : prep_tri_filter(e);
 }
 
 rb::KParams rb::make_params(rb_engine* e, uint32_t first_pass, uint32_t n_passes, int src, int dst) {
@@ -206,6 +243,22 @@
     p.lds_mode = e->opt._reserved[4];
     const bool single = p.u.bvh_node_count <= 1u && p.sph_nodes == nullptr && !e->trace_uv;
     p.no_uv = (single && e->sc.no_uv && (e->sc.untex_lights || p.u.ground_enabled == 0u)) ? 1u : 0u;
+    if (single && p.u.bvh_node_count == 1u && !e->sift_table.groups.empty() && e->sift_groups.ptr) {
+        float extra[2][6];
+        uint32_t n_extra = 0;
+        for (int k = 0; k < 3; ++k) extra[0][k] = extra[0][3 + k] = p.u.camera.pos[k];
+        n_extra++;
+        if (e->sph_box_any && p.u.spheres_count > 0u) std::memcpy(extra[n_extra++], e->sph_box, sizeof e->sph_box);
+        const rb::SiftRegion r = rb::sift_region(e->sift_table, extra, n_extra);
+        if (r.on) {
+            p.sift = 1u;
+            p.sift_groups = reinterpret_cast<const float*>(e->sift_groups.ptr);
+            p.sift_block_ends = e->sift_table.block_ends;
+            for (int k = 0; k < 3; ++k) p.sift_lo[k] = r.lo[k], p.sift_hi[k] = r.hi[k];
+            p.sift_kp = r.kp, p.sift_ks = r.ks, p.sift_kt = r.kt, p.sift_kd = r.kd;
+            p.sift_rmax = r.rmax;
+        }
+    }
     return p;
 }
 
@@ -543,6 +596,7 @@
         e->opt.flags = (e->opt.flags & ~(rb::kOwnTreeFlags | RB_FLAG_DEVICE_LBVH | RB_FLAG_CHUNK_WALK | RB_FLAG_SKIP_NEAR_DEGENERATE)) |
                        RB_FLAG_REFERENCE_WALK;
     if (const char* uv = std::getenv("RB_TRACE_UV"); uv && uv[0] == '1') e->trace_uv = true;
+    if (const char* tf = std::getenv("RB_TRI_FILTER"); tf && tf[0] == '0') e->tri_filter = false;
     auto bail = [&](const char* what, hipError_t st) -> rb_engine* {
         rb::fail(nullptr, RB_ERR_DEVICE, "%s failed: %s", what, hipGetErrorString(st));
         rb_destroy(e);
@@ -1141,4 +1195,19 @@
     return rb::debug_walk_profile(reinterpret_cast<unsigned long long*>(out64), reset) == 0 ? RB_OK : RB_ERR_DEVICE;
 }
 
-}
+int rb_debug_tri_filter(rb_engine* e, const float* rays, uint32_t n, uint32_t* out, uint32_t* list2) {
+    if (!e || !rays || !out || !list2) return RB_ERR_NULL_ARGUMENT;
+    std::lock_guard<std::mutex> g(e->mu);
+    rb::set_device(e);
+    if (int rc = require_ready(e)) return rc;
+    if (int rc = ensure_prepared(e)) return rc;
+    const rb::KParams p = make_params(e, 0, 0, e->cur, e->cur);
+    if (p.sift == 0u) return rb::fail(e, RB_ERR_INVALID_OPTIONS, "this engine's scene does not sift its triangle list");
+    if (n == 0u) return RB_OK;
+    if (n > (1u << 22)) return rb::fail(e, RB_ERR_INVALID_OPTIONS, "at most 2^22 rays");
+    HIP_TRY(e, hipStreamSynchronize(e->stream));
+    list2[0] = e->sift_table.first, list2[1] = e->sift_table.end;
+    return rb::debug_tri_filter(p, rays, n, list2[0], list2[1], out);
+}
+
+}
diff --git a/renderbaby_amd/csrc/rb_tri_filter.hpp b/renderbaby_amd/csrc/rb_tri_filter.hpp
--- /dev/null
+++ b/renderbaby_amd/csrc/rb_tri_filter.hpp
@@ -0,0 +1,216 @@
+#pragma once
+#include <algorithm>
+#include <cmath>
+#include <cstdint>
+#include <vector>
+
+#include "rb_chunk_math.hpp"
+
+namespace rb {
+
+constexpr uint32_t kSiftMaxSlots = 128;
+constexpr uint32_t kSiftGroupMax = 4;
+constexpr uint32_t kSiftMinLive = 4;
+constexpr double kSiftAlphaMax = 1e-3;
+constexpr double kSiftBoxGrow = 1.05;
+constexpr float kSiftKS = 24.0f * 5.9604645e-8f * 1.01f, kSiftKP = 12.0f * 5.9604645e-8f * 1.01f, kSiftKT = 11.0f * 5.9604645e-8f * 1.01f,
+                kSiftKD = 16.0f * 5.9604645e-8f * 1.01f;
+constexpr double kSiftEdgeMax = 1e9, kSiftSpMax = 1e12;
+constexpr double kSiftSlabUlps = 8.0;
+
+struct alignas(16) SiftGroup {
+    float c[3];
+    float fk;
+    float h[3];
+    float cap;
+    float n[3];
+    float s;
+    uint32_t first, count;
+    uint32_t closed, _pad;
+};
+static_assert(sizeof(SiftGroup) == 64, "one s_load_dwordx16");
+
+struct SiftTable {
+    std::vector<SiftGroup> groups;
+    uint32_t first = 0, end = 0;
+    uint32_t block_ends = 0;
+    uint32_t live = 0, closed = 0;
+    float tmn[3] = {0, 0, 0}, tmx[3] = {0, 0, 0};
+    double lhalf = 0.0;
+};
+
+struct SiftRegion {
+    float lo[3], hi[3];
+    float kp, ks, kt, kd;
+    float rmax;
+    bool on = false;
+};
+
+namespace sift {
+
+inline bool finite3(const float v[3]) { return std::isfinite(v[0]) && std::isfinite(v[1]) && std::isfinite(v[2]); }
+
+struct Item {
+    bool closed = false, live = false;
+    chunkmath::ChunkItem it{};
+    double lo[3], hi[3];
+};
+
+inline Item make_item(const PrepTri& t, uint32_t slot) {
+    Item m;
+    m.live = t.valid != 0u;
+    if (!m.live || !finite3(t.v0) || !finite3(t.e1) || !finite3(t.e2)) return m;
+    rb_gpu_triangle g{};
+    for (int a = 0; a < 3; ++a) g.v1[a] = t.e1[a], g.v2[a] = t.e2[a];
+    chunkmath::make_item(g, slot, 0u, m.it);
+    for (int a = 0; a < 3; ++a) {
+        const double p0 = t.v0[a], p1 = double(t.v0[a]) + double(t.e1[a]), p2 = double(t.v0[a]) + double(t.e2[a]);
+        m.lo[a] = chunkmath::dmin(p0, chunkmath::dmin(p1, p2));
+        m.hi[a] = chunkmath::dmax(p0, chunkmath::dmax(p1, p2));
+    }
+    m.closed = m.it.has_normal && std::isfinite(m.it.fa_l) && std::isfinite(m.it.fa) && m.it.fa_l > 0.0;
+    return m;
+}
+
+inline SiftGroup open_group(uint32_t first, uint32_t count) {
+    SiftGroup g{};
+    g.fk = g.cap = chunkmath::f_inf();
+    g.first = first;
+    g.count = count;
+    return g;
+}
+
+inline double ext_sum(const double lo[3], const double hi[3]) { return (hi[0] - lo[0]) + (hi[1] - lo[1]) + (hi[2] - lo[2]); }
+
+inline bool close_group(const std::vector<Item>& items, uint32_t a, uint32_t b, uint32_t first_slot, SiftGroup& out) {
+    double lo[3], hi[3], largest = 0.0;
+    for (int k = 0; k < 3; ++k) lo[k] = items[a].lo[k], hi[k] = items[a].hi[k];
+    double cap = 0, fa = 0, cap_l = 0, fa_l = 0;
+    for (uint32_t i = a; i < b; ++i) {
+        const Item& m = items[i];
+        for (int k = 0; k < 3; ++k) lo[k] = chunkmath::dmin(lo[k], m.lo[k]), hi[k] = chunkmath::dmax(hi[k], m.hi[k]);
+        largest = chunkmath::dmax(largest, ext_sum(m.lo, m.hi));
+        cap = chunkmath::dmax(cap, m.it.cap), fa = chunkmath::dmax(fa, m.it.fa);
+        cap_l = chunkmath::dmax(cap_l, m.it.cap_l), fa_l = chunkmath::dmax(fa_l, m.it.fa_l);
+    }
+    if (b - a > 1u && !(ext_sum(lo, hi) <= kSiftBoxGrow * largest)) return false;
+    if (!(cap_l <= kSiftEdgeMax * kSiftEdgeMax * 1e6 * (1.0 + 1e-5))) return false;
+    const chunkmath::DCone cone = chunkmath::cone_of([&](uint32_t i) -> const chunkmath::ChunkItem& { return items[a + i].it; }, b - a);
+    if (!cone.valid || !(cone.alpha <= kSiftAlphaMax)) return false;
+    const bool beyond = !(cap_l * (1.0 + 1e-6) <= 1.5e5);
+    const double capv = beyond ? HUGE_VAL : cap * (1.0 + 1e-6), fav = beyond ? fa_l : fa;
+    const double fk = fav * double(kFastGrazeCos) * 1.00001 * (1.0 + 2e-6);
+    if (!(fk <= 1.5e5)) return false;
+    SiftGroup g{};
+    for (int k = 0; k < 3; ++k) {
+        const double mid = 0.5 * (lo[k] + hi[k]);
+        g.c[k] = static_cast<float>(mid);
+        const double half = chunkmath::dmax(hi[k] - double(g.c[k]), double(g.c[k]) - lo[k]);
+        const double pad = half * (1.0 + 1e-6) + 1e-12 * std::fabs(mid) + 1e-37;
+        g.h[k] = chunkmath::f32_not_below(pad, half);
+        if (!std::isfinite(g.c[k]) || !std::isfinite(g.h[k])) return false;
+    }
+    g.fk = chunkmath::f32_not_below(fk, fk);
+    g.cap = std::isfinite(capv) ? chunkmath::f32_not_below(capv, capv) : chunkmath::f_inf();
+    const double cos_a = std::cos(cone.alpha) * (1.0 - 1e-6) - 1e-7;
+    for (int k = 0; k < 3; ++k) g.n[k] = static_cast<float>(cone.c[k] * cos_a);
+    const double sin_a = std::sin(cone.alpha) * (1.0 + 1e-5) + 2e-6;
+    g.s = chunkmath::f32_not_below(sin_a, sin_a);
+    g.first = first_slot + a;
+    g.count = b - a;
+    g.closed = 1u;
+    out = g;
+    return true;
+}
+
+}
+
+inline void build_sift_table(const PrepTri* ptris, uint32_t first, uint32_t end, SiftTable& tb) {
+    tb = SiftTable{};
+    tb.first = first, tb.end = end;
+    if (end <= first || end - first > kSiftMaxSlots) return;
+    const uint32_t n = end - first;
+    std::vector<sift::Item> items(n);
+    for (uint32_t i = 0; i < n; ++i) {
+        items[i] = sift::make_item(ptris[first + i], first + i);
+        tb.live += items[i].live ? 1u : 0u;
+    }
+    for (uint32_t i = 0; i < n; ++i) {
+        SiftGroup alone;
+        items[i].closed = items[i].closed && sift::close_group(items, i, i + 1u, first, alone);
+    }
+    bool any = false;
+    uint32_t a = 0;
+    while (a < n) {
+        const uint32_t block_end = std::min(n, (a / 32u + 1u) * 32u);
+        SiftGroup g = sift::open_group(first + a, 1u);
+        uint32_t b = a + 1u;
+        if (items[a].closed && sift::close_group(items, a, b, first, g)) {
+            SiftGroup wider;
+            while (b < block_end && b - a < kSiftGroupMax && items[b].closed && sift::close_group(items, a, b + 1u, first, wider)) g = wider, ++b;
+        } else {
+            g = sift::open_group(first + a, 1u);
+            while (b < block_end && b - a < kSiftGroupMax && !items[b].closed) ++b;
+            g.count = b - a;
+        }
+        if (g.closed) {
+            tb.closed++;
+            double sum = 0.0;
+            for (int k = 0; k < 3; ++k) {
+                const float lo = g.c[k] - g.h[k], hi = g.c[k] + g.h[k];
+                const float lo_ = std::nextafter(lo, -chunkmath::f_inf()), hi_ = std::nextafter(hi, chunkmath::f_inf());
+                tb.tmn[k] = any ? std::min(tb.tmn[k], lo_) : lo_;
+                tb.tmx[k] = any ? std::max(tb.tmx[k], hi_) : hi_;
+                sum += 2.0 * double(g.h[k]);
+            }
+            tb.lhalf = chunkmath::dmax(tb.lhalf, 0.5 * sum);
+            any = true;
+        }
+        tb.groups.push_back(g);
+        a = b;
+    }
+    uint32_t gi = 0;
+    for (uint32_t blk = 0; blk < 4u; ++blk) {
+        while (gi < tb.groups.size() && tb.groups[gi].first - first < (blk + 1u) * 32u) ++gi;
+        tb.block_ends |= gi << (8u * blk);
+    }
+}
+
+inline bool sift_pays(const SiftTable& tb) { return !tb.groups.empty() && tb.live >= kSiftMinLive && tb.closed >= 1u; }
+
+inline SiftRegion sift_region(const SiftTable& tb, const float (*extra)[6], uint32_t n_extra, float KP = kSiftKP, float KS = kSiftKS,
+                              float KT = kSiftKT, float KD = kSiftKD) {
+    SiftRegion r{};
+    if (!sift_pays(tb)) return r;
+    double lo[3], hi[3];
+    for (int k = 0; k < 3; ++k) lo[k] = tb.tmn[k], hi[k] = tb.tmx[k];
+    for (uint32_t i = 0; i < n_extra; ++i)
+        for (int k = 0; k < 3; ++k) {
+            if (!std::isfinite(extra[i][k]) || !std::isfinite(extra[i][3 + k])) return r;
+            lo[k] = chunkmath::dmin(lo[k], extra[i][k]), hi[k] = chunkmath::dmax(hi[k], extra[i][3 + k]);
+        }
+    double m = 0.0, diag2 = 0.0;
+    for (int k = 0; k < 3; ++k) m = chunkmath::dmax(m, chunkmath::dmax(std::fabs(lo[k]), std::fabs(hi[k])));
+    const double pad = 1e-3 * chunkmath::dmax(m, chunkmath::dmax(hi[0] - lo[0], chunkmath::dmax(hi[1] - lo[1], hi[2] - lo[2]))) + 1e-30;
+    for (int k = 0; k < 3; ++k) {
+        const double l = lo[k] - pad, h = hi[k] + pad;
+        r.lo[k] = std::nextafter(static_cast<float>(l), -chunkmath::f_inf());
+        r.hi[k] = std::nextafter(static_cast<float>(h), chunkmath::f_inf());
+        diag2 += (double(r.hi[k]) - double(r.lo[k])) * (double(r.hi[k]) - double(r.lo[k]));
+        m = chunkmath::dmax(m, chunkmath::dmax(std::fabs(double(r.lo[k])), std::fabs(double(r.hi[k]))));
+    }
+    const double u = 5.9604645e-8;
+    const double sp = 1.001 * (std::sqrt(diag2) + tb.lhalf);
+    const double kp = sp * double(KP) * (1.0 + 1e-6), ks = (sp * double(KS) + kSiftSlabUlps * u * (m + sp)) * (1.0 + 1e-6);
+    const double kt = sp * double(KT) * (1.0 + 1e-6), kd = sp * double(KD) * (1.0 + 1e-6);
+    r.kp = chunkmath::f32_not_below(kp, kp), r.ks = chunkmath::f32_not_below(ks, ks);
+    r.kt = chunkmath::f32_not_below(kt, kt), r.kd = chunkmath::f32_not_below(kd, kd);
+    const double reach = 2.0 * m + sp + (kp * 1.5e5 + ks);
+    r.rmax = static_cast<float>(1e38 / reach);
+    if (double(r.rmax) * reach > 1e38) r.rmax = std::nextafter(r.rmax, 0.0f);
+    r.on = sp <= kSiftSpMax && std::isfinite(r.rmax) && r.rmax > 0.0f && std::isfinite(r.kp) && std::isfinite(r.ks) && std::isfinite(r.kt) && std::isfinite(r.kd) && std::isfinite(r.lo[0]) &&
+           std::isfinite(r.lo[1]) && std::isfinite(r.lo[2]) && std::isfinite(r.hi[0]) && std::isfinite(r.hi[1]) && std::isfinite(r.hi[2]);
+    return r;
+}
+
+}
diff --git a/renderbaby_amd/engine.py b/renderbaby_amd/engine.py
--- a/renderbaby_amd/engine.py
+++ b/renderbaby_amd/engine.py
@@ -394,6 +394,13 @@
     def trace_form(self):
         return int(self._lib.rb_debug_trace_form(self._h))
 
+    def tri_filter_masks(self, origins, directions):
+        rays = np.ascontiguousarray(np.concatenate([np.asarray(origins, np.float32), np.asarray(directions, np.float32)], axis=1))
+        out, lst = np.zeros((len(rays), 4), np.uint32), np.zeros(2, np.uint32)
+        self._check(self._lib.rb_debug_tri_filter(self._h, rays.ctypes.data, len(rays), out.ctypes.data, lst.ctypes.data))
+        bits = (out[:, :, None] >> np.arange(32, dtype=np.uint32)) & 1
+        return bits.reshape(len(rays), 128)[:, :int(lst[1] - lst[0])].T.astype(bool), int(lst[0])
+
     _ray_records = staticmethod(ray_records)
 
     def _device_call(self, fn, *args):
diff --git a/renderbaby_amd/tri_filter_model.py b/renderbaby_amd/tri_filter_model.py
--- /dev/null
+++ b/renderbaby_amd/tri_filter_model.py
@@ -0,0 +1,177 @@
+import numpy as np
+
+F32 = np.float32
+U = 2.0 ** -24
+C0 = 0.03
+FMAX = F32(1.5e5)
+KS, KP, KT, KD = (F32(24.0) * F32(5.9604645e-8) * F32(1.01), F32(12.0) * F32(5.9604645e-8) * F32(1.01),
+                  F32(11.0) * F32(5.9604645e-8) * F32(1.01), F32(16.0) * F32(5.9604645e-8) * F32(1.01))
+SLAB_ULPS = 8.0
+EDGE_MAX, SP_MAX = 1e9, 1e12
+GROUP_MAX, ALPHA_MAX, BOX_GROW, MIN_LIVE, MAX_SLOTS = 4, 1e-3, 1.05, 4, 128
+INF = F32(np.inf)
+
+
+def f32_not_below(v, floor):
+    v, floor = np.asarray(v, np.float64), np.asarray(floor, np.float64)
+    with np.errstate(over="ignore"):
+        f = v.astype(F32)
+    up = np.nextafter(f, INF)
+    return np.where(f.astype(np.float64) < floor, up, f).astype(F32)
+
+
+def _fma(a, b, c):
+    with np.errstate(invalid="ignore", over="ignore"):
+        return (np.asarray(a, np.float64) * np.asarray(b, np.float64) + np.asarray(c, np.float64)).astype(F32)
+
+
+def make_group(v0, e1, e2):
+    v0, e1, e2 = (np.asarray(a, F32) for a in (v0, e1, e2))
+    m, _, n = v0.shape
+    d0, d1, d2 = v0.astype(np.float64), e1.astype(np.float64), e2.astype(np.float64)
+    finite = np.isfinite(d0).all((0, 1)) & np.isfinite(d1).all((0, 1)) & np.isfinite(d2).all((0, 1))
+    with np.errstate(all="ignore"):
+        l1, l2 = (d1 * d1).sum(1), (d2 * d2).sum(1)
+        nx = np.stack([d1[:, 1] * d2[:, 2] - d1[:, 2] * d2[:, 1], d1[:, 2] * d2[:, 0] - d1[:, 0] * d2[:, 2],
+                       d1[:, 0] * d2[:, 1] - d1[:, 1] * d2[:, 0]], 1)
+        nn = np.sqrt((nx * nx).sum(1))
+        ll = np.maximum(l1, l2)
+        has_normal = (nn > 0.0) & np.isfinite(nn)
+        unit = nx / np.where(has_normal, nn, 1.0)[:, None]
+        graze = ll / nn / (0.95 * float(F32(C0)))
+        bf = np.where(ll * 1e6 * (1.0 + 1e-5) <= 0.0, 0.0, f32_not_below(graze * (1.0 + 1e-5), graze * (1.0 + 1e-6)).astype(np.float64))
+        g = np.sqrt(l1) * np.sqrt(l2) * (1.0 + 1e-12)
+        cap = g * 1e6 * (1.0 + 1e-5)
+        fa = np.where(ll > 0.0, bf * (g / np.where(ll > 0.0, ll, 1.0)) * (1.0 + 1e-9), bf)
+        cap_l, fa_l = ll * 1e6 * (1.0 + 1e-5), bf
+        ok = finite & (has_normal & np.isfinite(fa_l) & np.isfinite(fa) & (fa_l > 0.0)).all(0)
+        p1, p2 = d0 + d1, d0 + d2
+        tlo, thi = np.minimum(d0, np.minimum(p1, p2)), np.maximum(d0, np.maximum(p1, p2))
+        lo, hi = tlo.min(0), thi.max(0)
+        largest = (thi - tlo).sum(1).max(0)
+        if m > 1:
+            ok &= (hi - lo).sum(0) <= BOX_GROW * largest
+        sg = np.where((unit * unit[0:1]).sum(1) < 0.0, -1.0, 1.0)
+        axis = (unit * sg[:, None]).sum(0)
+        ln = np.sqrt((axis * axis).sum(0))
+        ok &= ln > 1e-9
+        axis = axis / np.where(ln > 1e-9, ln, 1.0)
+        cmin = np.minimum(1.0, np.abs((unit * axis[None]).sum(1)).min(0))
+        alpha = np.arccos(cmin) + 1e-9
+        ok &= alpha <= ALPHA_MAX
+        ok &= cap_l.max(0) <= EDGE_MAX * EDGE_MAX * 1e6 * (1.0 + 1e-5)
+        beyond = ~(cap_l.max(0) * (1.0 + 1e-6) <= 1.5e5)
+        capv = np.where(beyond, np.inf, cap.max(0) * (1.0 + 1e-6))
+        fav = np.where(beyond, fa_l.max(0), fa.max(0))
+        fk = fav * float(F32(C0)) * 1.00001 * (1.0 + 2e-6)
+        ok &= fk <= 1.5e5
+        mid = 0.5 * (lo + hi)
+        c = mid.astype(F32)
+        half = np.maximum(hi - c.astype(np.float64), c.astype(np.float64) - lo)
+        h = f32_not_below(half * (1.0 + 1e-6) + 1e-12 * np.abs(mid) + 1e-37, half)
+        ok &= np.isfinite(c).all(0) & np.isfinite(h).all(0)
+        cos_a = np.cos(alpha) * (1.0 - 1e-6) - 1e-7
+        sin_a = np.sin(alpha) * (1.0 + 1e-5) + 2e-6
+        grp = dict(c=np.where(ok, c, F32(0)), h=np.where(ok, h, F32(0)), nrm=np.where(ok, (axis * cos_a).astype(F32), F32(0)),
+                   fk=np.where(ok, f32_not_below(fk, fk), INF), cap=np.where(ok, np.where(np.isfinite(capv), f32_not_below(capv, capv), INF), INF),
+                   s=np.where(ok, f32_not_below(sin_a, sin_a), F32(0)), closed=ok)
+    return grp
+
+
+def make_region(grp, extra_lo, extra_hi):
+    c, h = grp["c"], grp["h"]
+    tlo = np.nextafter((c - h).astype(F32), -INF).astype(np.float64)
+    thi = np.nextafter((c + h).astype(F32), INF).astype(np.float64)
+    lhalf = 0.5 * (2.0 * h.astype(np.float64)).sum(0)
+    return region_of(tlo, thi, lhalf, extra_lo, extra_hi)
+
+
+def region_of(tlo, thi, lhalf, extra_lo, extra_hi):
+    lo, hi = np.minimum(tlo, extra_lo), np.maximum(thi, extra_hi)
+    m = np.maximum(np.abs(lo), np.abs(hi)).max(0)
+    pad = 1e-3 * np.maximum(m, (hi - lo).max(0)) + 1e-30
+    rlo = np.nextafter((lo - pad).astype(F32), -INF)
+    rhi = np.nextafter((hi + pad).astype(F32), INF)
+    ext = rhi.astype(np.float64) - rlo.astype(np.float64)
+    m = np.maximum(m, np.maximum(np.abs(rlo), np.abs(rhi)).max(0).astype(np.float64))
+    sp = 1.001 * (np.sqrt((ext * ext).sum(0)) + lhalf)
+    k = lambda v: f32_not_below(v * (1.0 + 1e-6), v * (1.0 + 1e-6))
+    kp, ks = sp * float(KP) * (1.0 + 1e-6), (sp * float(KS) + SLAB_ULPS * U * (m + sp)) * (1.0 + 1e-6)
+    reach = 2.0 * m + sp + (kp * 1.5e5 + ks)
+    with np.errstate(over="ignore"):
+        rmax = (1e38 / reach).astype(F32)
+        rmax = np.where(rmax.astype(np.float64) * reach > 1e38, np.nextafter(rmax, F32(0)), rmax).astype(F32)
+    return dict(on=(sp <= SP_MAX) & np.isfinite(rmax) & (rmax > 0), lo=rlo, hi=rhi, kp=k(sp * float(KP)), ks=k(sp * float(KS) + SLAB_ULPS * U * (m + sp)),
+                kt=k(sp * float(KT)), kd=k(sp * float(KD)), rmax=rmax)
+
+
+def pass1(grp, reg, o, d, detail=False):
+    o, d = [np.asarray(x, F32) for x in o], [np.asarray(x, F32) for x in d]
+    with np.errstate(all="ignore"):
+        inv = [F32(1.0) / d[i] for i in range(3)]
+        oi = [o[i] * inv[i] for i in range(3)]
+        inside = np.ones(o[0].shape, bool)
+        for i in range(3):
+            inside &= (o[i] > reg["lo"][i]) & (o[i] < reg["hi"][i]) & (np.abs(inv[i]) <= reg["rmax"])
+        nrm, c, h = grp["nrm"], grp["c"], grp["h"]
+        y = _fma(d[2], nrm[2], _fma(d[1], nrm[1], d[0] * nrm[0]))
+        lb = np.abs(y) - grp["s"]
+        fl = grp["fk"] * (F32(1.0) / lb)
+        f = np.where((lb > F32(1e-6)) & (fl < grp["cap"]), fl, grp["cap"]).astype(F32)
+        mm = _fma(reg["kp"], f, reg["ks"])
+        thr = F32(0.001) - _fma(reg["kt"], f, reg["kd"])
+        tn, tf = None, None
+        for i in range(3):
+            tc = _fma(c[i], inv[i], -oi[i])
+            hm = h[i] + mm
+            a, b = _fma(-hm, np.abs(inv[i]), tc), _fma(hm, np.abs(inv[i]), tc)
+            tn = a if tn is None else np.fmax(tn, a)
+            tf = b if tf is None else np.fmin(tf, b)
+        keep = (~(tf < tn) & ~(tf < thr)) | ~(f <= FMAX) | ~inside | ~reg["on"]
+    if detail:
+        return keep, dict(tn=tn, tf=tf, thr=thr, f=f, inside=inside)
+    return keep
+
+
+def build_table(v0, e1, e2, valid):
+    v0, e1, e2 = (np.asarray(a, F32) for a in (v0, e1, e2))
+    n = len(v0)
+    assert n <= MAX_SLOTS
+    rec = lambda a, b: make_group(v0[a:b].reshape(b - a, 3, 1), e1[a:b].reshape(b - a, 3, 1), e2[a:b].reshape(b - a, 3, 1))
+    single = [rec(i, i + 1) if valid[i] else None for i in range(n)]
+    is_closed = [g is not None and bool(g["closed"][0]) for g in single]
+    groups, a = [], 0
+    while a < n:
+        block_end = min(n, (a // 32 + 1) * 32)
+        b = a + 1
+        if is_closed[a]:
+            g = single[a]
+            while b < block_end and b - a < GROUP_MAX and is_closed[b]:
+                wider = rec(a, b + 1)
+                if not wider["closed"][0]:
+                    break
+                g, b = wider, b + 1
+        else:
+            g = make_group(np.full((1, 3, 1), np.nan, F32), np.zeros((1, 3, 1), F32), np.zeros((1, 3, 1), F32))
+            while b < block_end and b - a < GROUP_MAX and not is_closed[b]:
+                b += 1
+        groups.append((a, b - a, g))
+        a = b
+    return groups, int(np.count_nonzero(valid)), sum(1 for g in groups if g[2]["closed"][0])
+
+
+def table_region(groups, extra_lo, extra_hi):
+    closed = [g for _, _, g in groups if g["closed"][0]]
+    tlo = np.min([np.nextafter((g["c"] - g["h"]).astype(F32), -INF) for g in closed], 0).astype(np.float64)
+    thi = np.max([np.nextafter((g["c"] + g["h"]).astype(F32), INF) for g in closed], 0).astype(np.float64)
+    lhalf = max(0.5 * float((2.0 * g["h"].astype(np.float64)).sum()) for g in closed)
+    return region_of(tlo, thi, lhalf, np.asarray(extra_lo, np.float64).reshape(3, 1), np.asarray(extra_hi, np.float64).reshape(3, 1))
+
+
+def candidate_mask(groups, reg, o, d):
+    o, d = np.asarray(o, F32), np.asarray(d, F32)
+    n = sum(c for _, c, _ in groups)
+    out = np.zeros((n, o.shape[1]), bool)
+    for first, count, g in groups:
+        out[first:first + count] = pass1(g, reg, o, d)[None]
+    return out
```

Result: faster. 45050 Msamples/s (median of 6 runs) (+12.1%).
